# felixendres/rgbdslam_v2

Measured on AMD Instinct MI355X. Metric: frame-pairs matched+RANSAC/sec, 640x480 ORB-1000, higher is better.
Workload: dtype fp4 MFMA, exact (match) + f32/f64 (RANSAC); 1 GPU; configs[1]: synthetic 640x480 RGB-D, ORB 1000 kp, 20 candidate pairs/frame, 200 frames; max_matches=300, parallelism=pair-sharded x1, graph_capture=True

## Files before the change

### include/rgbdfe.h

```cpp
#ifndef RGBDFE_H
#define RGBDFE_H

#include <stddef.h>
#include <stdint.h>

#ifdef __cplusplus
extern "C" {
#endif

#define RGBDFE_MAX_MATCHES 320
#define RGBDFE_MASK_WORDS 5
#define RGBDFE_MAX_KEYPOINTS 65535

typedef enum {
  RGBDFE_OK = 0,
  RGBDFE_ERR_INVALID_ARG = -1,
  RGBDFE_ERR_NO_DEVICE = -2,
  RGBDFE_ERR_HIP = -3,
  RGBDFE_ERR_UNKNOWN_NODE = -4,
  RGBDFE_ERR_CAPACITY = -5,
  RGBDFE_ERR_OUT_OF_MEMORY = -6,
  RGBDFE_ERR_INTERNAL = -7
} rgbdfe_status;

// ... 71 lines not shown
int  rgbdfe_match_pair_list_allgather_inliers(rgbdfe_ctx* ctx, const int32_t* query_ids, const int32_t* train_ids,
                                              int32_t n_pairs, void* const* d_out, int32_t* records_per_device,
                                              int32_t* list_entries, int64_t* stride_bytes);
int  rgbdfe_pack_compact(rgbdfe_ctx* ctx, const void* d_records, int32_t n, void* d_compact, void* stream);
int  rgbdfe_sizeof_compact_result(void);
int  rgbdfe_pack_inliers(rgbdfe_ctx* ctx, const void* d_records, int32_t n, int32_t n_headers, void* d_stream,
                         int32_t* d_total, void* stream);
int  rgbdfe_sizeof_inlier_header(void);
int  rgbdfe_set_params(rgbdfe_ctx* ctx, const rgbdfe_params* p);
const char* rgbdfe_status_string(int status);
const char* rgbdfe_last_error(rgbdfe_ctx* ctx);

int rgbdfe_upload_node(rgbdfe_ctx* ctx, int32_t node_id, const uint8_t* desc,
                       const float* xyz1, int32_t n);
int rgbdfe_upload_nodes(rgbdfe_ctx* ctx, int32_t n_nodes, const int32_t* node_ids, const uint8_t* const* desc,
                        const float* const* xyz1, const int32_t* counts);
int rgbdfe_upload_node_device(rgbdfe_ctx* ctx, int32_t node_id, const void* d_desc,
                              const void* d_xyz1, int32_t n, void* stream);
int rgbdfe_upload_node_keypoints(rgbdfe_ctx* ctx, int32_t node_id, const float* kp_xy, int32_t n);
int rgbdfe_release_node(rgbdfe_ctx* ctx, int32_t node_id);
int rgbdfe_node_count(rgbdfe_ctx* ctx, int32_t node_id);

int rgbdfe_match_node_pairs(rgbdfe_ctx* ctx, int32_t new_node_id, const int32_t* candidate_ids,
                            int32_t n_pairs, rgbdfe_match_result* out);
int rgbdfe_match_pair_list(rgbdfe_ctx* ctx, const int32_t* query_ids, const int32_t* train_ids,
                           int32_t n_pairs, rgbdfe_match_result* out);
int rgbdfe_match_pair_list_device(rgbdfe_ctx* ctx, const int32_t* query_ids,
                                  const int32_t* train_ids, int32_t n_pairs, void* d_out,
                                  void* stream);
int rgbdfe_submit_pair_list(rgbdfe_ctx* ctx, const int32_t* query_ids, const int32_t* train_ids,
                            int32_t n_pairs, void* d_out, int64_t* ticket);
int rgbdfe_wait_ticket(rgbdfe_ctx* ctx, int64_t ticket, void* stream);
#define RGBDFE_HOST_RECORDS 0
#define RGBDFE_HOST_INLIERS 1
int rgbdfe_submit_pair_list_host(rgbdfe_ctx* ctx, const int32_t* query_ids, const int32_t* train_ids, int32_t n_pairs,
                                 void* out, size_t out_bytes, int payload, int64_t* ticket);
int rgbdfe_wait_host(rgbdfe_ctx* ctx, int64_t ticket, int64_t* bytes_written);
int rgbdfe_wait_host_into(rgbdfe_ctx* ctx, int64_t ticket, void* out, size_t out_bytes, int64_t* bytes_written);
int rgbdfe_synchronize(rgbdfe_ctx* ctx);

int rgbdfe_upload_sift_node(rgbdfe_ctx* ctx, int32_t node_id, const float* desc128,
                            const float* xyz1, int32_t n);
int rgbdfe_match_sift_pair_list(rgbdfe_ctx* ctx, const int32_t* query_ids, const int32_t* train_ids,
                                int32_t n_pairs, rgbdfe_match_result* out, float* out_dist);
int rgbdfe_submit_sift_pair_list(rgbdfe_ctx* ctx, const int32_t* query_ids, const int32_t* train_ids,
                                 int32_t n_pairs, void* d_out, void* d_out_dist, int64_t* ticket);
int rgbdfe_sift_match_nodes(rgbdfe_ctx* ctx, int32_t query_id, int32_t train_id, int32_t* match_q,
                            int32_t* match_t, float* match_dist, int32_t* n_matches);

int rgbdfe_upload_float_node(rgbdfe_ctx* ctx, int32_t node_id, const float* desc, int32_t dim, const float* xyz1,
                             int32_t n);
int rgbdfe_match_flann_pair_list(rgbdfe_ctx* ctx, const int32_t* query_ids, const int32_t* train_ids, int32_t n_pairs,
                                 double nn_distance_ratio, rgbdfe_match_result* out, float* out_dist);

int rgbdfe_hamming_nn_nodes(rgbdfe_ctx* ctx, int32_t query_id, int32_t train_id,
                            int32_t* out_hd, int32_t* out_idx);
int rgbdfe_hamming_nn_host(rgbdfe_ctx* ctx, const uint8_t* qdesc, int32_t nq,
                           const uint8_t* tdesc, int32_t nt, int32_t* out_hd, int32_t* out_idx);

int rgbdfe_project_to_3d(rgbdfe_ctx* ctx, const float* kp_xy, int32_t n_kp, const float* depth,
                         int32_t rows, int32_t cols, double fx, double fy, double cx, double cy,
                         double depth_scaling, int32_t max_keypoints, int32_t* kept_idx,
                         float* xyz1, int32_t* n_out);

int rgbdfe_project_to_3d_cloud(rgbdfe_ctx* ctx, const float* kp_xy, int32_t n_kp, const float* cloud, int32_t rows,
                               int32_t cols, double maximum_depth, int32_t max_keypoints, int32_t* kept_idx, float* xyz1,
                               int32_t* n_out);

int rgbdfe_sift_node_features(rgbdfe_ctx* ctx, const float* kp_xy, int32_t n_kp, const float* desc_in,
                              const float* depth, int32_t rows, int32_t cols, double fx, double fy,
                              double cx, double cy, double depth_scaling, int32_t max_keypoints,
                              int32_t use_root_sift, int32_t* kept_idx, float* xyz1,
                              float* siftgpu_descriptors, float* feature_descriptors, int32_t* n_out);
int rgbdfe_sift_node_features_min_depth(rgbdfe_ctx* ctx, const float* kp_xy, const float* kp_size, int32_t n_kp,
                                        const float* desc_in, const float* depth, int32_t rows, int32_t cols, double fx,
                                        double fy, double cx, double cy, double depth_scaling, int32_t max_keypoints,
                                        int32_t use_root_sift, int32_t* kept_idx, float* xyz1, float* siftgpu_descriptors,
                                        float* feature_descriptors, int32_t* n_out);

int rgbdfe_set_latency_mode(rgbdfe_ctx* ctx, int32_t max_pairs, int32_t chunk_iterations);

#define RGBDFE_HAMMING_MODE_DEFAULT 3
int rgbdfe_set_hamming_mode(rgbdfe_ctx* ctx, int32_t mode);

typedef struct rgbdfe_emm_counts {
  uint32_t inliers, outliers, occluded, all;
} rgbdfe_emm_counts;
int rgbdfe_depth_to_mono8(rgbdfe_ctx* ctx, const void* depth, int32_t depth_is_u16, int32_t rows, int32_t cols,
                          uint8_t* mono8, float* depth_m);
int rgbdfe_upload_node_cloud(rgbdfe_ctx* ctx, int32_t node_id, const float* depth, int32_t rows, int32_t cols,
                             const uint8_t* rgb, int32_t rgb_channels, int32_t encoding_bgr, double fx,
                             double fy, double cx, double cy, double depth_scaling, double min_depth,
                             int32_t cloud_skip, float* cloud_out);
int rgbdfe_release_node_cloud(rgbdfe_ctx* ctx, int32_t node_id);
int rgbdfe_observation_likelihood(rgbdfe_ctx* ctx, int32_t n, const int32_t* new_ids, const int32_t* old_ids,
                                  const float* transforms, int32_t emm_skip_step, rgbdfe_emm_counts* out);
int rgbdfe_observation_criterion_met(uint32_t inliers, uint32_t outliers, uint32_t all,
                                     double observability_threshold, double* quality);

int rgbdfe_assemble_map(rgbdfe_ctx* ctx, int32_t n_nodes, const int32_t* node_ids, const float* transforms,
                        double maximum_depth, int32_t preserve_raster, float* out, int64_t capacity, int64_t* n_out,
                        int64_t* node_offsets);
int rgbdfe_assemble_map_device(rgbdfe_ctx* ctx, int32_t n_nodes, const int32_t* node_ids, const float* transforms,
                               double maximum_depth, int32_t preserve_raster, void* d_out, int64_t capacity,
                               int64_t* n_out, int64_t* node_offsets, void* stream);
int rgbdfe_download_node_cloud(rgbdfe_ctx* ctx, int32_t node_id, float* cloud_out, int64_t capacity_points,
                               int32_t* rows, int32_t* cols);

#define RGBDFE_VOXEL_LEAF_TOO_SMALL 1
int rgbdfe_voxel_filter(rgbdfe_ctx* ctx, const float* points, int64_t n_in, double voxelfilter_size, float* out,
                        int64_t capacity, int64_t* n_out, int32_t* flags);
int rgbdfe_voxel_filter_device(rgbdfe_ctx* ctx, const void* d_points, int64_t n_in, double voxelfilter_size,
                               void* d_out, int64_t capacity, int64_t* n_out, int32_t* flags, void* stream);
int rgbdfe_reduce_node_cloud(rgbdfe_ctx* ctx, int32_t node_id, double voxelfilter_size, int64_t* n_out,
                             int32_t* flags);

typedef struct rgbdfe_octomap rgbdfe_octomap;
typedef struct rgbdfe_octomap_params {
  double resolution;
  double prob_hit;
  double prob_miss;
  double clamping_min;
  double clamping_max;
  double occupancy_threshold;
} rgbdfe_octomap_params;
typedef struct rgbdfe_octomap_leaf {
  uint16_t key[3];
  uint16_t zero0;
  float log_odds;
  uint8_t rgb[3];
  uint8_t zero1;
} rgbdfe_octomap_leaf;
void rgbdfe_octomap_default_params(rgbdfe_octomap_params* params);
int rgbdfe_octomap_create(rgbdfe_ctx* ctx, const rgbdfe_octomap_params* params, int64_t capacity_cells,
                          rgbdfe_octomap** map);
void rgbdfe_octomap_destroy(rgbdfe_octomap* map);
int rgbdfe_octomap_reset(rgbdfe_octomap* map);
int rgbdfe_octomap_reserve(rgbdfe_octomap* map, int64_t capacity_cells);
int rgbdfe_octomap_insert_nodes(rgbdfe_octomap* map, int32_t n_nodes, const int32_t* node_ids, const float* transforms,
                                double max_range, int32_t* n_done);
int rgbdfe_octomap_insert_cloud(rgbdfe_octomap* map, const float* points, int64_t n, const float* transform,
                                double max_range);
int rgbdfe_octomap_size(rgbdfe_octomap* map, int64_t* n_leaves);
int rgbdfe_octomap_leaves(rgbdfe_octomap* map, rgbdfe_octomap_leaf* out, int64_t capacity, int64_t* n_out);
int rgbdfe_octomap_stats(rgbdfe_octomap* map, int64_t* out, int32_t n_out);

typedef struct rgbdfe_octomap_node {
  float log_odds;
  uint8_t rgb[3];
  uint8_t children;
} rgbdfe_octomap_node;
int rgbdfe_octomap_tree(rgbdfe_octomap* map, rgbdfe_octomap_node* out, int64_t capacity, int64_t* n_nodes);
int rgbdfe_octomap_tree_device(rgbdfe_octomap* map, void* d_out, int64_t capacity, int64_t* n_nodes, void* stream);
int rgbdfe_octomap_nodes_at_depth(rgbdfe_octomap* map, int32_t depth, float min_log_odds, rgbdfe_octomap_leaf* out,
                                  int64_t capacity, int64_t* n_out);
int rgbdfe_octomap_write(rgbdfe_octomap* map, const char* path);
int rgbdfe_octomap_set_leaves(rgbdfe_octomap* map, const rgbdfe_octomap_leaf* leaves, int64_t n);
int rgbdfe_octomap_read(rgbdfe_octomap* map, const char* path);

typedef struct rgbdfe_pose_graph rgbdfe_pose_graph;
typedef int (*rgbdfe_rand_fn)(void* state);
rgbdfe_pose_graph* rgbdfe_pose_graph_create(void);
void rgbdfe_pose_graph_destroy(rgbdfe_pose_graph* g);
int rgbdfe_pose_graph_add_node(rgbdfe_pose_graph* g, int32_t node_id, int32_t vertex_id, int32_t matchable,
                               int32_t keyframe);
int rgbdfe_pose_graph_add_edge(rgbdfe_pose_graph* g, int32_t node_id1, int32_t node_id2);
// ... 169 lines not shown
```

### rgbdslam_v2_amd/_lib.py

```python
import ctypes as C
import os

import numpy as np

_HERE = os.path.dirname(os.path.abspath(__file__))
LIB_PATH = os.environ.get("RGBDFE_LIB", os.path.join(_HERE, "librgbdfe.so"))

RGBDFE_MAX_MATCHES = 320
RGBDFE_MASK_WORDS = 5

DEFAULT_HAMMING_MODE = 3
KERNEL_HAMMING = 0
KERNEL_RANSAC = 1
KERNEL_SIFT_DOT = 2
KERNEL_SIFT_FINISH = 3
KERNEL_EMM = 4


class RgbdfeParams(C.Structure):
    _fields_ = [
        ("max_matches", C.c_int32),
        ("min_matches", C.c_int32),
        ("ransac_iterations", C.c_int32),
        ("max_dist_for_inliers", C.c_float),
# ... 278 lines not shown
    L.rgbdfe_release_node_cloud.argtypes = [ctx, i32]
    L.rgbdfe_observation_likelihood.restype = C.c_int
    L.rgbdfe_observation_likelihood.argtypes = [ctx, i32, vp, vp, vp, i32, vp]
    L.rgbdfe_assemble_map.restype = C.c_int
    L.rgbdfe_assemble_map.argtypes = [ctx, i32, vp, vp, C.c_double, i32, vp, C.c_int64, C.POINTER(C.c_int64), vp]
    L.rgbdfe_assemble_map_device.restype = C.c_int
    L.rgbdfe_assemble_map_device.argtypes = [ctx, i32, vp, vp, C.c_double, i32, vp, C.c_int64, C.POINTER(C.c_int64), vp, vp]
    L.rgbdfe_download_node_cloud.restype = C.c_int
    L.rgbdfe_download_node_cloud.argtypes = [ctx, i32, vp, C.c_int64, C.POINTER(i32), C.POINTER(i32)]
    L.rgbdfe_voxel_filter.restype = C.c_int
    L.rgbdfe_voxel_filter.argtypes = [ctx, vp, C.c_int64, C.c_double, vp, C.c_int64, C.POINTER(C.c_int64), C.POINTER(i32)]
    L.rgbdfe_voxel_filter_device.restype = C.c_int
    L.rgbdfe_voxel_filter_device.argtypes = [ctx, vp, C.c_int64, C.c_double, vp, C.c_int64, C.POINTER(C.c_int64),
                                             C.POINTER(i32), vp]
    L.rgbdfe_reduce_node_cloud.restype = C.c_int
    L.rgbdfe_reduce_node_cloud.argtypes = [ctx, i32, C.c_double, C.POINTER(C.c_int64), C.POINTER(i32)]
    omap = vp
    L.rgbdfe_octomap_default_params.restype = None
    L.rgbdfe_octomap_default_params.argtypes = [C.POINTER(OctomapParams)]
    L.rgbdfe_octomap_create.restype = C.c_int
    L.rgbdfe_octomap_create.argtypes = [ctx, C.POINTER(OctomapParams), C.c_int64, C.POINTER(vp)]
    L.rgbdfe_octomap_destroy.restype = None
    L.rgbdfe_octomap_destroy.argtypes = [omap]
    L.rgbdfe_octomap_reset.restype = C.c_int
    L.rgbdfe_octomap_reset.argtypes = [omap]
    L.rgbdfe_octomap_reserve.restype = C.c_int
    L.rgbdfe_octomap_reserve.argtypes = [omap, C.c_int64]
    L.rgbdfe_octomap_insert_nodes.restype = C.c_int
    L.rgbdfe_octomap_insert_nodes.argtypes = [omap, i32, vp, vp, C.c_double, C.POINTER(i32)]
    L.rgbdfe_octomap_insert_cloud.restype = C.c_int
    L.rgbdfe_octomap_insert_cloud.argtypes = [omap, vp, C.c_int64, vp, C.c_double]
    L.rgbdfe_octomap_size.restype = C.c_int
    L.rgbdfe_octomap_size.argtypes = [omap, C.POINTER(C.c_int64)]
    L.rgbdfe_octomap_leaves.restype = C.c_int
    L.rgbdfe_octomap_leaves.argtypes = [omap, vp, C.c_int64, C.POINTER(C.c_int64)]
    L.rgbdfe_octomap_stats.restype = C.c_int
    L.rgbdfe_octomap_stats.argtypes = [omap, vp, i32]
    L.rgbdfe_octomap_tree.restype = C.c_int
    L.rgbdfe_octomap_tree.argtypes = [omap, vp, C.c_int64, C.POINTER(C.c_int64)]
    L.rgbdfe_octomap_tree_device.restype = C.c_int
    L.rgbdfe_octomap_tree_device.argtypes = [omap, vp, C.c_int64, C.POINTER(C.c_int64), vp]
    L.rgbdfe_octomap_nodes_at_depth.restype = C.c_int
    L.rgbdfe_octomap_nodes_at_depth.argtypes = [omap, i32, C.c_float, vp, C.c_int64, C.POINTER(C.c_int64)]
    L.rgbdfe_octomap_write.restype = C.c_int
    L.rgbdfe_octomap_write.argtypes = [omap, C.c_char_p]
    L.rgbdfe_octomap_set_leaves.restype = C.c_int
    L.rgbdfe_octomap_set_leaves.argtypes = [omap, vp, C.c_int64]
    L.rgbdfe_octomap_read.restype = C.c_int
    L.rgbdfe_octomap_read.argtypes = [omap, C.c_char_p]
    L.rgbdfe_observation_criterion_met.restype = C.c_int
    L.rgbdfe_observation_criterion_met.argtypes = [C.c_uint32, C.c_uint32, C.c_uint32, C.c_double,
                                                   C.POINTER(C.c_double)]
    L.rgbdfe_set_latency_mode.restype = C.c_int
    L.rgbdfe_set_latency_mode.argtypes = [ctx, i32, i32]
    L.rgbdfe_set_profiling.restype = C.c_int
    L.rgbdfe_set_profiling.argtypes = [ctx, C.c_int]
    L.rgbdfe_get_kernel_time.restype = C.c_int
    L.rgbdfe_get_kernel_time.argtypes = [ctx, C.c_int, C.POINTER(C.c_double),
                                         C.POINTER(C.c_int64), C.POINTER(C.c_int64)]
    L.rgbdfe_reset_kernel_time.restype = C.c_int
    L.rgbdfe_reset_kernel_time.argtypes = [ctx]
    L.rgbdfe_set_graph_capture.restype = C.c_int
    L.rgbdfe_set_graph_capture.argtypes = [ctx, C.c_int]
    L.rgbdfe_graph_stats.restype = C.c_int
    L.rgbdfe_graph_stats.argtypes = [ctx, C.POINTER(C.c_int64), C.c_int32]
    L.rgbdfe_create_multi.restype = C.c_int
    L.rgbdfe_create_multi.argtypes = [C.POINTER(RgbdfeConfig), vp, i32, C.POINTER(vp)]
    L.rgbdfe_device_count.restype = C.c_int
    L.rgbdfe_device_count.argtypes = [ctx]
    L.rgbdfe_device_context.restype = vp
    L.rgbdfe_device_context.argtypes = [ctx, i32]
    L.rgbdfe_match_pair_list_allgather.restype = C.c_int
    L.rgbdfe_match_pair_list_allgather.argtypes = [ctx, vp, vp, i32, vp, C.POINTER(i32)]
    L.rgbdfe_match_pair_list_allgather_edges.restype = C.c_int
    L.rgbdfe_match_pair_list_allgather_edges.argtypes = [ctx, vp, vp, i32, vp, vp, vp, C.POINTER(i32)]
    L.rgbdfe_group_submit_us.restype = C.c_int
    L.rgbdfe_group_submit_us.argtypes = [ctx, C.POINTER(C.c_double)]
    L.rgbdfe_gather_transport.restype = C.c_char_p
    L.rgbdfe_gather_transport.argtypes = [ctx]
    L.rgbdfe_gather_exchanges.restype = C.c_int
    L.rgbdfe_gather_exchanges.argtypes = [ctx]
    L.rgbdfe_set_hamming_mode.restype = C.c_int
    L.rgbdfe_set_hamming_mode.argtypes = [ctx, i32]
    L.rgbdfe_match_pair_list_allgather_compact.restype = C.c_int
    L.rgbdfe_match_pair_list_allgather_compact.argtypes = [ctx, vp, vp, i32, vp, C.POINTER(i32)]
    L.rgbdfe_pack_compact.restype = C.c_int
    L.rgbdfe_pack_compact.argtypes = [ctx, vp, i32, vp, vp]
    L.rgbdfe_sizeof_compact_result.restype = C.c_int
    L.rgbdfe_match_pair_list_allgather_inliers.restype = C.c_int
    L.rgbdfe_match_pair_list_allgather_inliers.argtypes = [ctx, vp, vp, i32, vp, C.POINTER(i32), vp, C.POINTER(C.c_int64)]
    L.rgbdfe_pack_inliers.restype = C.c_int
    L.rgbdfe_pack_inliers.argtypes = [ctx, vp, i32, i32, vp, vp, vp]
    L.rgbdfe_sizeof_inlier_header.restype = C.c_int
    if L.rgbdfe_sizeof_inlier_header() != INLIER_HEADER_DTYPE.itemsize:
        raise RgbdfeError("rgbdfe_inlier_header layout mismatch between librgbdfe.so and the binding")
    if L.rgbdfe_sizeof_compact_result() != COMPACT_DTYPE.itemsize:
        raise RgbdfeError("rgbdfe_compact_result layout mismatch between librgbdfe.so and the binding")
    L.rgbdfe_sift_detect.restype = C.c_int
    L.rgbdfe_sift_detect.argtypes = [ctx, vp, vp, i32, i32, i32, vp, vp, i32, C.POINTER(i32)]
    L.rgbdfe_sift_describe.restype = C.c_int
    L.rgbdfe_sift_describe.argtypes = [ctx, vp, i32, i32, vp, i32, vp]
    L.rgbdfe_sift_detect_batch.restype = C.c_int
    L.rgbdfe_sift_detect_batch.argtypes = [ctx, i32, vp, i32, i32, i32, i32, vp, vp, vp]
    L.rgbdfe_sift_detect_batch_nodes.restype = C.c_int
    L.rgbdfe_sift_detect_batch_nodes.argtypes = [ctx, i32, vp, vp, i32, i32, C.c_double, C.c_double, C.c_double, C.c_double,
                                                 C.c_double, i32, i32, vp, i32, vp, vp, vp, vp]
    L.rgbdfe_detect.restype = C.c_int
    L.rgbdfe_detect.argtypes = [ctx, vp, vp, i32, i32, vp, i32, C.POINTER(i32)]
    L.rgbdfe_detect_sift_describe.restype = C.c_int
    L.rgbdfe_detect_sift_describe.argtypes = [ctx, vp, vp, vp, i32, i32, C.c_double, C.c_double, C.c_double, C.c_double,
                                              C.c_double, i32, vp, vp, vp, vp, C.POINTER(i32)]
    L.rgbdfe_detect_sift_describe_batch_nodes.restype = C.c_int
    L.rgbdfe_detect_sift_describe_batch_nodes.argtypes = [ctx, i32, vp, vp, vp, i32, i32, C.c_double, C.c_double, C.c_double,
                                                          C.c_double, C.c_double, i32, vp, i32, vp, vp, vp, vp]
    L.rgbdfe_sift_detect_orb_describe.restype = C.c_int
    L.rgbdfe_sift_detect_orb_describe.argtypes = [ctx, vp, vp, i32, i32, C.c_double, C.c_double, C.c_double, C.c_double,
                                                  C.c_double, i32, vp, vp, vp, C.POINTER(i32)]
    L.rgbdfe_sift_detect_orb_describe_batch_nodes.restype = C.c_int
    L.rgbdfe_sift_detect_orb_describe_batch_nodes.argtypes = [ctx, i32, vp, vp, i32, i32, C.c_double, C.c_double, C.c_double,
                                                              C.c_double, C.c_double, i32, vp, i32, vp, vp, vp, vp]
    L.rgbdfe_sizeof_sensor_frame.restype = C.c_int
    if L.rgbdfe_sizeof_sensor_frame() != C.sizeof(RgbdfeSensorFrame):
        raise RgbdfeError("rgbdfe_sensor_frame layout mismatch between librgbdfe.so and the binding")
    L.rgbdfe_ingest_frame.restype = C.c_int
    L.rgbdfe_ingest_frame.argtypes = [ctx, C.POINTER(RgbdfeSensorFrame), vp, vp, vp]
    L.rgbdfe_sensor_detect_describe.restype = C.c_int
    L.rgbdfe_sensor_detect_describe.argtypes = [ctx, C.POINTER(RgbdfeSensorFrame), C.c_double, C.c_double, C.c_double, C.c_double,
                                                C.c_double, vp, vp, vp, C.POINTER(i32)]
    L.rgbdfe_sensor_detect_describe_batch_nodes.restype = C.c_int
    L.rgbdfe_sensor_detect_describe_batch_nodes.argtypes = [ctx, i32, C.POINTER(RgbdfeSensorFrame), C.c_double, C.c_double,
                                                            C.c_double, C.c_double, C.c_double, i32, vp, vp, vp, vp, vp,
                                                            C.POINTER(RgbdfeSensorCloud)]
    L.rgbdfe_sift_geometry.restype = C.c_int
    L.rgbdfe_sift_geometry.argtypes = [ctx] + [C.POINTER(i32)] * 4
    L.rgbdfe_sift_debug_plane.restype = C.c_int
    L.rgbdfe_sift_debug_plane.argtypes = [ctx, i32, i32, vp, i32, C.POINTER(i32), C.POINTER(i32)]
    L.rgbdfe_sift_debug_candidates.restype = C.c_int
    L.rgbdfe_sift_debug_candidates.argtypes = [ctx, i32, i32, vp, i32, C.POINTER(i32)]
    L.rgbdfe_sizeof_match_result.restype = C.c_int
    L.rgbdfe_abi_version.restype = C.c_int
    if L.rgbdfe_sizeof_match_result() != C.sizeof(RgbdfeMatchResult) or \
            RESULT_DTYPE.itemsize != C.sizeof(RgbdfeMatchResult):
        raise RgbdfeError("rgbdfe_match_result layout mismatch between librgbdfe.so and the binding")
    RAND_FN = C.CFUNCTYPE(C.c_int, C.c_void_p)
    L.rgbdfe_rand_fn = RAND_FN
    L.rgbdfe_pose_graph_create.restype = vp
    L.rgbdfe_pose_graph_create.argtypes = []
    L.rgbdfe_pose_graph_destroy.restype = None
    L.rgbdfe_pose_graph_destroy.argtypes = [vp]
    L.rgbdfe_pose_graph_add_node.restype = C.c_int
    L.rgbdfe_pose_graph_add_node.argtypes = [vp, i32, i32, i32, i32]
    L.rgbdfe_pose_graph_add_edge.restype = C.c_int
    L.rgbdfe_pose_graph_add_edge.argtypes = [vp, i32, i32]
    L.rgbdfe_pose_graph_set_matchable.restype = C.c_int
    L.rgbdfe_pose_graph_set_matchable.argtypes = [vp, i32, i32]
    L.rgbdfe_pose_graph_set_estimate.restype = C.c_int
    L.rgbdfe_pose_graph_set_estimate.argtypes = [vp, i32, vp]
    L.rgbdfe_pose_graph_get_estimate.restype = C.c_int
    L.rgbdfe_pose_graph_get_estimate.argtypes = [vp, i32, vp]
    L.rgbdfe_pose_graph_set_fixed.restype = C.c_int
    L.rgbdfe_pose_graph_set_fixed.argtypes = [vp, i32, i32]
    L.rgbdfe_pose_graph_add_edge_se3.restype = C.c_int
    L.rgbdfe_pose_graph_add_edge_se3.argtypes = [vp, i32, i32, vp, vp, i32]
    L.rgbdfe_pose_graph_chi2.restype = C.c_int
    L.rgbdfe_pose_graph_chi2.argtypes = [vp, vp, C.POINTER(C.c_double)]
    L.rgbdfe_pose_graph_linearize.restype = C.c_int
    L.rgbdfe_pose_graph_linearize.argtypes = [vp, vp, vp, vp, i32, C.POINTER(i32), vp, vp, vp, i32, C.POINTER(i32), vp, vp, vp,
                                              i32, C.POINTER(i32), C.POINTER(C.c_double)]
    L.rgbdfe_pose_graph_optimize.restype = C.c_int
    L.rgbdfe_pose_graph_optimize.argtypes = [vp, vp, i32, C.POINTER(PoseGraphReport)]
    L.rgbdfe_pose_graph_optimize_graph.restype = C.c_int
    L.rgbdfe_pose_graph_optimize_graph.argtypes = [vp, vp, C.c_double, C.POINTER(PoseGraphReport)]
    L.rgbdfe_pose_graph_transforms.restype = C.c_int
    L.rgbdfe_pose_graph_transforms.argtypes = [vp, i32, vp, vp]
    L.rgbdfe_potential_edge_targets.restype = C.c_int
    L.rgbdfe_potential_edge_targets.argtypes = [vp, i32, i32, i32, i32, i32, i32, RAND_FN, vp, C.c_uint32, vp, i32,
                                                C.POINTER(i32)]
    _lib = L
    return L


EXPORTED_SYMBOLS = [
    "rgbdfe_default_config", "rgbdfe_create", "rgbdfe_destroy", "rgbdfe_set_params",
    "rgbdfe_status_string", "rgbdfe_last_error", "rgbdfe_upload_node", "rgbdfe_upload_nodes",
    "rgbdfe_upload_node_device", "rgbdfe_release_node", "rgbdfe_node_count",
    "rgbdfe_match_node_pairs", "rgbdfe_match_pair_list", "rgbdfe_match_pair_list_device",
    "rgbdfe_detector_configure", "rgbdfe_detector_thresholds", "rgbdfe_detect_describe",
    "rgbdfe_orb_detect", "rgbdfe_orb_compute",
    "rgbdfe_submit_pair_list", "rgbdfe_wait_ticket", "rgbdfe_submit_pair_list_host", "rgbdfe_wait_host", "rgbdfe_wait_host_into", "rgbdfe_upload_sift_node",
    "rgbdfe_match_sift_pair_list", "rgbdfe_submit_sift_pair_list", "rgbdfe_sift_match_nodes",
    "rgbdfe_synchronize", "rgbdfe_hamming_nn_nodes", "rgbdfe_hamming_nn_host",
    "rgbdfe_project_to_3d", "rgbdfe_sift_node_features", "rgbdfe_sift_node_features_min_depth", "rgbdfe_depth_to_mono8",
    "rgbdfe_host_register", "rgbdfe_host_unregister",
    "rgbdfe_upload_node_cloud", "rgbdfe_release_node_cloud", "rgbdfe_observation_likelihood",
    "rgbdfe_assemble_map", "rgbdfe_assemble_map_device", "rgbdfe_download_node_cloud",
    "rgbdfe_voxel_filter", "rgbdfe_voxel_filter_device", "rgbdfe_reduce_node_cloud",
    "rgbdfe_octomap_default_params", "rgbdfe_octomap_create", "rgbdfe_octomap_destroy", "rgbdfe_octomap_reset",
    "rgbdfe_octomap_reserve", "rgbdfe_octomap_insert_nodes", "rgbdfe_octomap_insert_cloud", "rgbdfe_octomap_size",
    "rgbdfe_octomap_leaves", "rgbdfe_octomap_stats",
    "rgbdfe_octomap_tree", "rgbdfe_octomap_tree_device", "rgbdfe_octomap_nodes_at_depth", "rgbdfe_octomap_write",
    "rgbdfe_octomap_set_leaves", "rgbdfe_octomap_read",
    "rgbdfe_observation_criterion_met", "rgbdfe_set_latency_mode", "rgbdfe_set_profiling", "rgbdfe_get_kernel_time",
    "rgbdfe_reset_kernel_time", "rgbdfe_graph_stats", "rgbdfe_set_graph_capture", "rgbdfe_match_pair_list_allgather_inliers", "rgbdfe_pack_inliers", "rgbdfe_sizeof_inlier_header", "rgbdfe_sizeof_match_result", "rgbdfe_abi_version",
    "rgbdfe_pose_graph_create", "rgbdfe_pose_graph_destroy", "rgbdfe_pose_graph_add_node",
    "rgbdfe_pose_graph_add_edge", "rgbdfe_pose_graph_set_matchable", "rgbdfe_potential_edge_targets",
    "rgbdfe_pose_graph_set_estimate", "rgbdfe_pose_graph_get_estimate", "rgbdfe_pose_graph_set_fixed",
    "rgbdfe_pose_graph_add_edge_se3", "rgbdfe_pose_graph_chi2", "rgbdfe_pose_graph_linearize",
    "rgbdfe_pose_graph_optimize", "rgbdfe_pose_graph_optimize_graph", "rgbdfe_pose_graph_transforms",
    "rgbdfe_create_multi", "rgbdfe_device_count", "rgbdfe_device_context", "rgbdfe_match_pair_list_allgather",
    "rgbdfe_gather_transport", "rgbdfe_gather_exchanges", "rgbdfe_set_hamming_mode", "rgbdfe_project_to_3d_cloud", "rgbdfe_detect_describe_cloud",
    "rgbdfe_detect_describe_batch", "rgbdfe_detect_describe_batch_nodes", "rgbdfe_match_pair_list_allgather_edges",
    "rgbdfe_set_feature_min_depth", "rgbdfe_project_to_3d_min_depth",
    "rgbdfe_place_recognition", "rgbdfe_place_recognition_batch", "rgbdfe_upload_float_node",
    "rgbdfe_match_flann_pair_list", "rgbdfe_upload_node_keypoints",
    "rgbdfe_match_pair_list_allgather_compact", "rgbdfe_pack_compact", "rgbdfe_sizeof_compact_result",
    "rgbdfe_group_submit_us", "rgbdfe_sift_detect", "rgbdfe_sift_detect_batch", "rgbdfe_sift_describe", "rgbdfe_sift_geometry", "rgbdfe_sift_debug_plane", "rgbdfe_sift_debug_candidates",
    "rgbdfe_sift_detect_batch_nodes", "rgbdfe_set_detector_type", "rgbdfe_fast_detect",
    "rgbdfe_detect", "rgbdfe_detect_sift_describe", "rgbdfe_detect_sift_describe_batch_nodes",
    "rgbdfe_sift_detect_orb_describe", "rgbdfe_sift_detect_orb_describe_batch_nodes",
    "rgbdfe_sizeof_sensor_frame", "rgbdfe_ingest_frame", "rgbdfe_sensor_detect_describe",
    "rgbdfe_sensor_detect_describe_batch_nodes",
]
```

### rgbdslam_v2_amd/csrc/api_batches.hip

```cpp
#include "rgbdfe_host.h"

namespace rgbdfe_host {


int fail(rgbdfe_ctx* ctx, int code, const std::string& msg) {
  if (ctx) {
    std::lock_guard<std::mutex> g(ctx->err_mu);
    ctx->last_error = msg;
  }
  return code;
}


void fill_ransac_const(rgbdfe_ctx* ctx) {
  const rgbdfe_params& p = ctx->cfg.params;
  RansacConst& rc = ctx->rc;
  rc.max_matches = p.max_matches;
  rc.min_matches = p.min_matches;
  rc.ransac_iterations = p.ransac_iterations;
  rc.max_dist_m = (float)(double)p.max_dist_for_inliers;
  rc.sq_max_dist = (double)(rc.max_dist_m * rc.max_dist_m);
  rc.depth_cov = p.depth_cov;
  const double cam_angle_x = 58.0 / 180.0 * M_PI;
  const double cam_angle_y = 45.0 / 180.0 * M_PI;
// ... 60 lines not shown
      ctx->event_pool.push_back(p.d);
    } else {
      add(RGBDFE_KERNEL_HAMMING, p.a, p.b);
      add(RGBDFE_KERNEL_RANSAC, p.b, p.c);
    }
    ctx->event_pool.push_back(p.a);
    ctx->event_pool.push_back(p.b);
    ctx->event_pool.push_back(p.c);
  }
  ctx->pending.clear();
}

int ensure_ec_pool(rgbdfe_ctx* ctx, rgbdfe_ctx::Lane& lane, size_t regions, hipStream_t stream) {
  if (regions <= lane.ec_regions) return RGBDFE_OK;
  HIP_TRY(ctx, hipStreamSynchronize(stream));
  if (lane.d_ec) (void)hipFree(lane.d_ec);
  lane.d_ec = nullptr;
  lane.ec_regions = 0;
  HIP_TRY(ctx, hipMalloc((void**)&lane.d_ec, regions * select_ransac_ec_region_bytes()));
  lane.ec_regions = regions;
  return RGBDFE_OK;
}
int want_latency_path(rgbdfe_ctx* ctx, rgbdfe_ctx::Lane& lane, int32_t n, hipStream_t stream, bool* use, int* chunk_out,
                      PhasePlan* plan) {
  const size_t need_recs = (size_t)n * (size_t)(ctx->rc.ransac_iterations > 0 ? ctx->rc.ransac_iterations : 0);
  const bool force_phases = ctx->latency_chunk_iters < 0;
  const int chunk_cfg = force_phases ? -ctx->latency_chunk_iters : ctx->latency_chunk_iters;
  int chunk = chunk_cfg > 0 ? chunk_cfg : (n <= 64 ? 4 : (n <= 640 ? 7 : (n <= 1280 ? 14 : 28)));
  const int I_all = ctx->rc.ransac_iterations > 0 ? ctx->rc.ransac_iterations : 0;
  const bool too_many_pairs = (size_t)n > kMaxEcRegions;
  while (!too_many_pairs && chunk < I_all && (size_t)n * (size_t)((I_all + chunk - 1) / chunk) > kMaxEcRegions) ++chunk;
  bool latency = !too_many_pairs && n <= ctx->latency_pairs && ctx->rc.ransac_iterations >= 2 * chunk &&
                 need_recs <= ((size_t)1 << 24);
  *chunk_out = chunk;
  if (latency && need_recs > lane.recs_capacity) {
    HIP_TRY(ctx, hipStreamSynchronize(stream));
    if (lane.d_recs) (void)hipFree(lane.d_recs);
    lane.d_recs = nullptr;
    lane.recs_capacity = 0;
    if (hipMalloc((void**)&lane.d_recs, need_recs * (sizeof(IterRec) + sizeof(IterSum)) +
                                            ransac_split_mask_bytes(need_recs, (size_t)ctx->cfg.max_pairs_per_batch)) == hipSuccess)
      lane.recs_capacity = need_recs;
    else latency = false;
  }
  if (latency && !lane.d_walk &&
      hipMalloc((void**)&lane.d_walk, sizeof(WalkState) * ((size_t)ctx->cfg.max_pairs_per_batch + 1)) != hipSuccess) {
    lane.d_walk = nullptr;
    latency = false;
  }
  const int I = ctx->rc.ransac_iterations;
  static const int env_phases = getenv("RGBDFE_PHASES") ? atoi(getenv("RGBDFE_PHASES")) : 0;
  static const int mid_plan = getenv("RGBDFE_MID_PLAN") ? atoi(getenv("RGBDFE_MID_PLAN")) : 0;
  const bool mid = n > 256 && n <= 1280 && !force_phases && env_phases == 0;
  if ((n <= 256 && !force_phases) || env_phases == 1 || (mid && mid_plan == 1)) { plan->n_phases = 1; plan->ends[0] = I; }
  else if (mid && mid_plan == 2 && I > 14) { plan->n_phases = 2; plan->ends[0] = 14; plan->ends[1] = I; }
  else if (env_phases == 2) { plan->n_phases = 2; plan->ends[0] = ((I * 7 / 20) / 7) * 7 > 0 ? ((I * 7 / 20) / 7) * 7 : I; plan->ends[1] = I; if (plan->ends[0] >= I) plan->n_phases = 1; }
  else {
    const int cand[4] = {14, ((I * 7 / 20) / 7) * 7, ((I * 14 / 20) / 7) * 7, I};
    int k = 0, last = 0;
    for (int c : cand) { const int e = c > I ? I : c; if (e > last) { plan->ends[k++] = e; last = e; } }
    if (k == 0) plan->ends[k++] = I;
    plan->n_phases = k;
  }
  *use = latency;
  size_t regions = (size_t)n;
  if (latency) {
    int begin = 0;
    for (int p = 0; p < plan->n_phases; ++p) {
      size_t chunks = (size_t)((plan->ends[p] - begin + chunk - 1) / chunk);
      if (plan->n_phases > 2 && p == 1)
        chunks += (size_t)((I - begin + 63) / 64);
      if ((size_t)n * chunks > regions) regions = (size_t)n * chunks;
      begin = plan->ends[p];
    }
  }
  regions = regions / (size_t)(n > 0 ? n : 1) * (((size_t)n + 7) / 8 * 8);
  return ensure_ec_pool(ctx, lane, regions + 8, stream);
}

bool hamming_on_mfma(const rgbdfe_ctx* ctx) { return ctx->hamming_mode != 0 && (uint32_t)ctx->cfg.max_keypoints <= 32768u; }

HammingGeometry hamming_geometry(const rgbdfe_ctx* ctx, uint32_t n, uint32_t max_nq, uint32_t max_nt) {
  const uint32_t cap = (uint32_t)ctx->cfg.max_pairs_per_batch;
  return hamming_on_mfma(ctx) ? hamming_mfma_geometry(n, max_nq, max_nt, cap) : hamming_nn_geometry(n, max_nq, max_nt, cap);
}

uint32_t launch_hamming(rgbdfe_ctx* ctx, const PairWork* d_work, uint32_t* d_keys, uint32_t n, HammingGeometry geom,
                        hipStream_t stream) {
  const uint32_t mk = (uint32_t)ctx->cfg.max_keypoints;
  if (hamming_on_mfma(ctx))
    return launch_hamming_mfma(ctx->d_desc4, d_work, d_keys, mk, n, geom, ctx->hamming_mode, stream);
  return launch_hamming_nn(ctx->d_desc, d_work, d_keys, mk, n, geom, stream);
}

uint32_t launch_hamming(rgbdfe_ctx* ctx, const PairWork* d_work, uint32_t* d_keys, uint32_t n, uint32_t max_nq,
                        uint32_t max_nt, hipStream_t stream) {
  return launch_hamming(ctx, d_work, d_keys, n, hamming_geometry(ctx, n, max_nq, max_nt), stream);
}

bool capture_stream_ready(rgbdfe_ctx* ctx) {
  if (ctx->capture_stream) return true;
  if (hipStreamCreateWithFlags(&ctx->capture_stream, hipStreamNonBlocking) != hipSuccess) { (void)hipGetLastError(); ctx->capture_stream = nullptr; }
  return ctx->capture_stream != nullptr;
}

int enqueue_pairs(rgbdfe_ctx* ctx, const int32_t* qids, const int32_t* tids, int32_t n, rgbdfe_match_result* d_out, hipEvent_t wait_for, int64_t* ticket_out, int* lane_out, int matcher, float* d_out_dist, double flann_ratio) {


  const bool sift = matcher != 0;
  if (n > ctx->cfg.max_pairs_per_batch)
    return fail(ctx, RGBDFE_ERR_CAPACITY, "n_pairs exceeds max_pairs_per_batch");
  const int64_t ticket = ctx->next_ticket;
  rgbdfe_ctx::Slot& slot = ctx->ring[ticket % rgbdfe_ctx::kRing];
  const int li = (int)(ticket % rgbdfe_ctx::kLanes);
  rgbdfe_ctx::Lane& lane = ctx->lanes[li];
  hipStream_t stream = lane.stream;
  if (slot.pending) {
    HIP_TRY(ctx, hipEventSynchronize(slot.done));
    slot.pending = false;
  }
  uint32_t max_nq = 0, max_nt = 0, sift_kinds = 0;
  for (int32_t i = 0; i < n; ++i) {
    auto q = ctx->nodes.find(qids[i]);
    auto t = ctx->nodes.find(tids[i]);
    if (q == ctx->nodes.end() || t == ctx->nodes.end())
      return fail(ctx, RGBDFE_ERR_UNKNOWN_NODE, "pair references a node that is not resident");
    if (q->second.kind != (uint32_t)matcher || t->second.kind != (uint32_t)matcher)
      return fail(ctx, RGBDFE_ERR_INVALID_ARG, "node descriptor kind does not fit this matcher");
    PairWork& w = slot.h_work[i];
    w.q_slot = q->second.slot;
    w.t_slot = t->second.slot;
    w.nq = q->second.n;
    w.nt = t->second.n;
    w.uid = pair_uid(qids[i], tids[i]);
    w.qid = qids[i];
    w.tid = tids[i];
    w.pad = matcher == 1 ? sift_fast_keys(ctx, q->second, t->second) : 0u;
    sift_kinds |= w.pad ? 1u : 2u;
    if (ctx->rc.g2o_iterations > 0 && !(q->second.flags & t->second.flags & kNodeHasKeypoints))
      return fail(ctx, RGBDFE_ERR_INVALID_ARG,
                  "g2o_iterations > 0: a node of the batch has no keypoints (rgbdfe_upload_node_keypoints after every upload of it)");
    if (w.nq > max_nq) max_nq = w.nq;
    if (w.nt > max_nt) max_nt = w.nt;
  }
  if (ctx->rc.g2o_iterations > 0 && !ctx->d_kp2d)
    return fail(ctx, RGBDFE_ERR_INVALID_ARG, "g2o_iterations > 0 needs the nodes' keypoints (rgbdfe_upload_node_keypoints)");
  int32_t piece = n;
  if (n > 0 && ctx->latency_pairs != 0) {
    const size_t I = (size_t)(ctx->rc.ransac_iterations > 0 ? ctx->rc.ransac_iterations : 1);
    size_t fit = (((size_t)1 << 24) / I) < kMaxEcRegions ? (((size_t)1 << 24) / I) : kMaxEcRegions;
    if (fit > 65535) fit = 65535;
    if (fit < 1) fit = 1;
    if ((size_t)n > fit && (size_t)n <= (size_t)ctx->latency_pairs) piece = (int32_t)fit;
  }
  if (sift && piece > 65535) return fail(ctx, RGBDFE_ERR_CAPACITY, "a one-wave SIFT batch holds at most 65535 pairs");
  bool latency = false;
  int chunk = 7;
  PhasePlan pp{};
  if (n > 0) {
    int rcl = want_latency_path(ctx, lane, piece, stream, &latency, &chunk, &pp);
    if (rcl != RGBDFE_OK) return rcl;
  }
  if (wait_for) HIP_TRY(ctx, hipStreamWaitEvent(stream, wait_for, 0));
  if (ctx->nodes_ready) HIP_TRY(ctx, hipStreamWaitEvent(stream, ctx->nodes_ready, 0));
  hipError_t launch_err = hipSuccess;
  if (n > 0) {
    if (!d_out) d_out = lane.d_results;
    const bool graphable = ctx->use_graphs && !sift && !ctx->profiling && piece >= n && ctx->rc.g2o_iterations == 0;
    const HammingGeometry geom = sift ? HammingGeometry{0, 1}
                                      : hamming_geometry(ctx, (uint32_t)(piece < n ? piece : n), max_nq, max_nt);
    rgbdfe_ctx::GraphEntry* ge = nullptr;
    bool capturing = false;
    if (graphable) {
      rgbdfe_ctx::GraphKey key;
      memset(&key, 0, sizeof(key));
      key.n = n; key.qblocks = geom.qblocks; key.tsplit = geom.tsplit; key.slot = (int32_t)(ticket % rgbdfe_ctx::kRing);
      key.latency = latency ? 1 : 0; key.chunk = chunk; key.hamming_mode = ctx->hamming_mode; key.n_phases = pp.n_phases;
      for (int i = 0; i < 4; ++i) key.ends[i] = i < pp.n_phases ? pp.ends[i] : 0;
      memcpy(&key.rc, &ctx->rc, sizeof(RansacConst));
      key.d_out = d_out; key.d_recs = lane.d_recs; key.d_ec = lane.d_ec; key.d_walk = lane.d_walk; key.d_keys = lane.d_keys;
      size_t gi = 0;
      for (; gi < ctx->graphs.size(); ++gi)
        if (memcmp(&ctx->graphs[gi].key, &key, sizeof(key)) == 0) { ge = &ctx->graphs[gi]; break; }
      if (ge) {
        ge->used = ++ctx->graph_clock;
        const hipError_t le = hipGraphLaunch(ge->exec, stream);
        if (le == hipSuccess) {
          ctx->graph_launches++;
          ctx->graph_miss_run = 0;
        } else {
          (void)hipGetLastError();
          (void)hipGraphExecDestroy(ge->exec); (void)hipGraphDestroy(ge->graph);
          ctx->graphs.erase(ctx->graphs.begin() + (long)gi);
          ctx->graph_launch_failures++;
          ge = nullptr;
        }
      } else {
        ctx->graph_misses++;
        const bool try_capture = ctx->graph_miss_run < rgbdfe_ctx::kGraphMissRun ||
                                 ctx->graph_miss_run % rgbdfe_ctx::kGraphRetry == 0;
        ctx->graph_miss_run++;
        if (try_capture && capture_stream_ready(ctx) &&
            hipStreamBeginCapture(ctx->capture_stream, hipStreamCaptureModeRelaxed) == hipSuccess) {
          capturing = true;
          if (ctx->graphs.size() >= 48) {
            size_t lru = 0;
            for (size_t i = 1; i < ctx->graphs.size(); ++i) if (ctx->graphs[i].used < ctx->graphs[lru].used) lru = i;
            (void)hipGraphExecDestroy(ctx->graphs[lru].exec); (void)hipGraphDestroy(ctx->graphs[lru].graph);
            ctx->graphs.erase(ctx->graphs.begin() + (long)lru);
          }
          ctx->graphs.push_back(rgbdfe_ctx::GraphEntry{key, nullptr, nullptr, ++ctx->graph_clock});
        } else {
          (void)hipGetLastError();
          ctx->graph_plain_batches++;
        }
      }
    }
    rgbdfe_ctx::Pending pend{};
    pend.sift = sift;
    for (int attempt = 0; attempt < 2; ++attempt) {
      hipStream_t const ls = capturing ? ctx->capture_stream : stream;
      if (!ge) {
        const hipError_t me = hipMemcpyAsync(slot.d_work, slot.h_work, sizeof(PairWork) * (size_t)n, hipMemcpyHostToDevice, ls);
        if (me != hipSuccess && launch_err == hipSuccess) launch_err = me;
      }
      if (ctx->profiling) {
        pend.a = get_event(ctx);
        pend.b = get_event(ctx);
        pend.c = get_event(ctx);
        if (sift) pend.d = get_event(ctx);
        pend.pairs = n;
        (void)hipEventRecord(pend.a, ls);
      }
      const uint32_t mk = (uint32_t)ctx->cfg.max_keypoints;
      for (int32_t off = 0; off < n && !ge; off += piece) {
        const int32_t m = (n - off) < piece ? (n - off) : piece;
        const bool first = off == 0, last = off + m >= n;
        if (!first) {
          int rcl = want_latency_path(ctx, lane, m, ls, &latency, &chunk, &pp);
          if (rcl != RGBDFE_OK) { launch_err = hipErrorOutOfMemory; break; }
        }
        const PairWork* d_work = slot.d_work + off;
        rgbdfe_match_result* d_res = d_out + off;
        if (!sift) {
          const uint32_t planes = launch_hamming(ctx, d_work, lane.d_keys, (uint32_t)m, first ? geom : hamming_geometry(ctx, (uint32_t)m, max_nq, max_nt), ls);
          if (ctx->profiling && first) (void)hipEventRecord(pend.b, ls);
          if (latency)
            launch_select_ransac_latency(ctx->d_xyz, d_work, lane.d_keys, planes, d_res, mk, (uint32_t)m, ctx->rc,
                                         lane.d_prep, lane.d_recs, lane.d_walk, lane.d_ec, chunk, pp.ends, pp.n_phases, ls);
          else
            launch_select_ransac(ctx->d_xyz, d_work, lane.d_keys, planes, d_res, mk, (uint32_t)m, ctx->rc, lane.d_prep,
                                 lane.d_ec, ls);
          if (ctx->rc.g2o_iterations > 0)
            launch_g2o_refine(d_work, d_res, (uint32_t)m, ctx->rc, lane.d_prep, ctx->d_kp2d, mk, lane.d_ec, ls);
          if (ctx->profiling && last) (void)hipEventRecord(pend.c, ls);
        } else {
          float* d_dist = (d_out_dist ? d_out_dist : lane.d_all_dist) + (size_t)off * RGBDFE_MAX_MATCHES;
          if (matcher == 2) {
            launch_l2_knn2(ctx->d_sift_f32, d_work, mk, (uint32_t)m, max_nq, lane.d_row_part, ls);
            if (ctx->profiling && first) (void)hipEventRecord(pend.b, ls);
// ... 83 lines not shown
```

### rgbdslam_v2_amd/csrc/api_context.hip

```cpp
#include "rgbdfe_host.h"

namespace impl {


void rgbdfe_default_config(rgbdfe_config* cfg) {
  if (!cfg) return;
  memset(cfg, 0, sizeof(*cfg));
  cfg->device_id = 0;
  cfg->max_nodes = 256;
  cfg->max_keypoints = 1024;
  cfg->max_pairs_per_batch = 4096;
  cfg->params.max_matches = 300;
  cfg->params.min_matches = 20;
  cfg->params.ransac_iterations = 200;
  cfg->params.max_dist_for_inliers = 3.0f;
  cfg->params.depth_cov = 1e-4;
  cfg->params.seed = 20260923u;
}

int rgbdfe_create(const rgbdfe_config* cfg, rgbdfe_ctx** out) {
  if (!cfg || !out) return RGBDFE_ERR_INVALID_ARG;
  *out = nullptr;
  if (cfg->max_nodes < 1 || cfg->max_keypoints < 1 || cfg->max_keypoints > RGBDFE_MAX_KEYPOINTS ||
      cfg->max_pairs_per_batch < 1)
    return RGBDFE_ERR_INVALID_ARG;
  int ndev = 0;
  if (hipGetDeviceCount(&ndev) != hipSuccess || ndev <= 0) return RGBDFE_ERR_NO_DEVICE;
  if (cfg->device_id < 0 || cfg->device_id >= ndev) return RGBDFE_ERR_NO_DEVICE;
  rgbdfe_ctx* ctx = new rgbdfe_ctx();
  ctx->cfg = *cfg;
  int rc = validate_params(ctx, cfg->params);
  if (rc != RGBDFE_OK) { delete ctx; return rc; }
  fill_ransac_const(ctx);
  if (const char* sf = getenv("RGBDFE_SIFT_FAST_KEYS")) ctx->sift_fast = atoi(sf) != 0;
  if (const char* hm = getenv("RGBDFE_HAMMING_MODE")) ctx->hamming_mode = atoi(hm) < 0 || atoi(hm) > 3 ? RGBDFE_HAMMING_MODE_DEFAULT : atoi(hm);
  if (const char* gr = getenv("RGBDFE_GRAPHS")) ctx->use_graphs = atoi(gr) != 0;
  auto bail = [&](int code) { ::rgbdfe_destroy(ctx); return code; };
  if (hipSetDevice(cfg->device_id) != hipSuccess) return bail(RGBDFE_ERR_NO_DEVICE);
  (void)ransac_split_init();
  if (hipStreamCreateWithFlags(&ctx->stream, hipStreamNonBlocking) != hipSuccess)
    return bail(RGBDFE_ERR_HIP);
  if (hipEventCreateWithFlags(&ctx->ev_in, hipEventDisableTiming) != hipSuccess) return bail(RGBDFE_ERR_HIP);
  const size_t rows = (size_t)cfg->max_nodes * (size_t)cfg->max_keypoints + 16;
  if (hipMalloc((void**)&ctx->d_desc, rows * 32) != hipSuccess) return bail(RGBDFE_ERR_OUT_OF_MEMORY);
  if (hipMalloc((void**)&ctx->d_xyz, rows * 16) != hipSuccess) return bail(RGBDFE_ERR_OUT_OF_MEMORY);
  if (hipMalloc((void**)&ctx->d_desc4, hamming_mfma_slab_bytes((uint32_t)cfg->max_nodes, (uint32_t)cfg->max_keypoints)) != hipSuccess)
    return bail(RGBDFE_ERR_OUT_OF_MEMORY);
  if (hipMemsetAsync(ctx->d_desc, 0, rows * 32, ctx->stream) != hipSuccess) return bail(RGBDFE_ERR_HIP);
  if (hipMemsetAsync(ctx->d_xyz, 0, rows * 16, ctx->stream) != hipSuccess) return bail(RGBDFE_ERR_HIP);
  if (hipMemsetAsync(ctx->d_desc4, 0, hamming_mfma_slab_bytes((uint32_t)cfg->max_nodes, (uint32_t)cfg->max_keypoints), ctx->stream) != hipSuccess)
    return bail(RGBDFE_ERR_HIP);
  if (hipStreamSynchronize(ctx->stream) != hipSuccess) return bail(RGBDFE_ERR_HIP);
  const size_t np = (size_t)cfg->max_pairs_per_batch;
  for (auto& sl : ctx->ring) {
    if (hipMalloc((void**)&sl.d_work, np * sizeof(PairWork)) != hipSuccess) return bail(RGBDFE_ERR_OUT_OF_MEMORY);
    if (hipHostMalloc((void**)&sl.h_work, np * sizeof(PairWork), hipHostMallocDefault) != hipSuccess)
      return bail(RGBDFE_ERR_OUT_OF_MEMORY);
    if (hipEventCreateWithFlags(&sl.done, hipEventDisableTiming) != hipSuccess) return bail(RGBDFE_ERR_HIP);
  }
  for (auto& ln : ctx->lanes) {
    if (hipStreamCreateWithFlags(&ln.stream, hipStreamNonBlocking) != hipSuccess) return bail(RGBDFE_ERR_HIP);
    if (hipMalloc((void**)&ln.d_keys, np * (size_t)cfg->max_keypoints * 4) != hipSuccess)
      return bail(RGBDFE_ERR_OUT_OF_MEMORY);
    if (hipMalloc((void**)&ln.d_results, np * sizeof(rgbdfe_match_result)) != hipSuccess)
      return bail(RGBDFE_ERR_OUT_OF_MEMORY);
    if (hipMalloc((void**)&ln.d_prep, np * sizeof(PairPrep)) != hipSuccess) return bail(RGBDFE_ERR_OUT_OF_MEMORY);
  }
  ctx->emm_q_lo = erf_boundary(0.001);
  ctx->emm_q_hi = erf_boundary(0.999);
  ctx->free_slots.reserve(cfg->max_nodes);
  for (int32_t s = cfg->max_nodes - 1; s >= 0; --s) ctx->free_slots.push_back((uint32_t)s);
  *out = ctx;
  return RGBDFE_OK;
}

void rgbdfe_destroy(rgbdfe_ctx* ctx) {
  if (!ctx) return;
  if (ctx->stream) (void)hipStreamSynchronize(ctx->stream);
  for (auto& ln : ctx->lanes) if (ln.stream) (void)hipStreamSynchronize(ln.stream);
  for (hipStream_t st : {ctx->orb_upload_stream, ctx->orb_compute_stream, ctx->sift_stream1, ctx->sift_stream2, ctx->sift_stream3,
                        ctx->sn.depth_stream, ctx->fast.st, ctx->fast.up})
    if (st) (void)hipStreamSynchronize(st);
  sift_nodes_release(ctx);
  sift_behind_release(ctx);
  sift_orb_release(ctx);
  sensor_release(ctx);
  drain_pending(ctx);
  for (hipEvent_t e : ctx->event_pool) (void)hipEventDestroy(e);
  for (auto& ge : ctx->graphs) { (void)hipGraphExecDestroy(ge.exec); (void)hipGraphDestroy(ge.graph); }
  if (ctx->capture_stream) (void)hipStreamDestroy(ctx->capture_stream);
  if (ctx->upload_stage) (void)hipHostFree(ctx->upload_stage);
  if (ctx->sift_stream1) (void)hipStreamDestroy(ctx->sift_stream1);
  if (ctx->sift_stream2) (void)hipStreamDestroy(ctx->sift_stream2);
  if (ctx->sift_stream3) (void)hipStreamDestroy(ctx->sift_stream3);
  ctx->graphs.clear();
  if (ctx->d_desc) (void)hipFree(ctx->d_desc);
  if (ctx->d_xyz) (void)hipFree(ctx->d_xyz);
  for (auto& sl : ctx->ring) {
    if (sl.d_work) (void)hipFree(sl.d_work);
    if (sl.h_work) (void)hipHostFree(sl.h_work);
    if (sl.done) (void)hipEventDestroy(sl.done);
  }
  for (auto& kv : ctx->clouds) {
    if (kv.second.d) (void)hipFree(kv.second.d);
    if (kv.second.d_samples) (void)hipFree(kv.second.d_samples);
  }
  if (ctx->d_sift_bf16) (void)hipFree(ctx->d_sift_bf16);
  if (ctx->d_sift_f32) (void)hipFree(ctx->d_sift_f32);
  for (auto& ln : ctx->lanes) {
    if (ln.d_row_part) (void)hipFree(ln.d_row_part);
    if (ln.d_col_part) (void)hipFree(ln.d_col_part);
    if (ln.d_col_blocks) (void)hipFree(ln.d_col_blocks);
    if (ln.d_sm_q) (void)hipFree(ln.d_sm_q);
    if (ln.d_sm_t) (void)hipFree(ln.d_sm_t);
    if (ln.d_sm_d) (void)hipFree(ln.d_sm_d);
    if (ln.d_sm_n) (void)hipFree(ln.d_sm_n);
    if (ln.d_all_dist) (void)hipFree(ln.d_all_dist);
    if (ln.d_recs) (void)hipFree(ln.d_recs);
// ... 264 lines not shown
```

### rgbdslam_v2_amd/csrc/api_frame.hip

```cpp
#include "rgbdfe_host.h"

namespace impl {

static int hamming_keys_to_host(rgbdfe_ctx* ctx, uint32_t nq, uint32_t planes, int32_t* out_hd, int32_t* out_idx) {
  const size_t mk = (size_t)ctx->cfg.max_keypoints;
  std::vector<uint32_t> all((size_t)planes * mk), keys(nq);
  hipStream_t st = ctx->lanes[0].stream;
  HIP_TRY(ctx, hipMemcpyAsync(all.data(), ctx->lanes[0].d_keys, all.size() * 4, hipMemcpyDeviceToHost, st));
  HIP_TRY(ctx, hipStreamSynchronize(st));
  for (uint32_t i = 0; i < nq; ++i) {
    uint32_t k = all[i];
    for (uint32_t pl = 1; pl < planes; ++pl) k = std::min(k, all[(size_t)pl * mk + i]);
    keys[i] = k;
  }
  for (uint32_t i = 0; i < nq; ++i) {
    const uint32_t hd = keys[i] >> 16;
    if (hd > 256u) {
      out_hd[i] = 257;
      out_idx[i] = -1;
    } else {
      out_hd[i] = (int32_t)hd;
      out_idx[i] = (int32_t)(keys[i] & 0xFFFFu);
    }
  }
// ... 509 lines not shown
    const CloudEntry& co = b->second;
    const bool flat = co.ch <= 1 || co.cw <= 1;
    if (i == 0) { ch = co.ch; cw = co.cw; cloud_skip = co.cloud_skip; }
    if (ch <= 1 || cw <= 1) {
      if (!flat) return fail(ctx, RGBDFE_ERR_INVALID_ARG, "clouds of one batch must share their dimensions");
      continue;
    }
    if (cn.ch != ch || cn.cw != cw || co.ch != ch || co.cw != cw || co.cloud_skip != cloud_skip)
      return fail(ctx, RGBDFE_ERR_INVALID_ARG, "clouds of one batch must share their dimensions");
    if (cn.samples_skip != emm_skip_step) {
      CloudEntry& w = a->second;
      if (w.d_samples) { (void)hipFree(w.d_samples); w.d_samples = nullptr; }
      const size_t ns = (size_t)((ch + emm_skip_step - 1) / emm_skip_step) * (size_t)((cw + emm_skip_step - 1) / emm_skip_step);
      if (hipMalloc((void**)&w.d_samples, ns * sizeof(float4)) != hipSuccess)
        return fail(ctx, RGBDFE_ERR_OUT_OF_MEMORY, "sample array allocation failed");
      launch_decimate_cloud(w.d, ch, cw, emm_skip_step, w.d_samples, ctx->stream);
      w.samples_skip = emm_skip_step;
    }
    EmmJob& jb = jobs[(size_t)i];
    jb.new_samples = cn.d_samples;
    jb.old_z = reinterpret_cast<const float*>(co.d + (size_t)co.ch * co.cw);
    const float* T = transforms + (size_t)i * 16;
    for (int r = 0; r < 3; ++r)
      for (int c = 0; c < 4; ++c) jb.T[r * 4 + c] = T[c * 4 + r];
    jb.fx = co.fx / cloud_skip; jb.fy = co.fy / cloud_skip;
    jb.cx = co.cx / cloud_skip; jb.cy = co.cy / cloud_skip;
  }
  if (ch <= 1 || cw <= 1) {
    for (int32_t i = 0; i < n; ++i) { out[i].inliers = out[i].all = 1; out[i].outliers = out[i].occluded = 0; }
    return RGBDFE_OK;
  }
  const size_t b_jobs = (sizeof(EmmJob) * (size_t)n + 255) & ~(size_t)255;
  int rc = ensure_scratch(ctx, b_jobs + (size_t)n * 16 + 256);
  if (rc != RGBDFE_OK) return rc;
  EmmJob* d_jobs = (EmmJob*)ctx->d_scratch;
  uint32_t* d_counts = (uint32_t*)((char*)ctx->d_scratch + b_jobs);
  HIP_TRY(ctx, hipMemcpyAsync(d_jobs, jobs.data(), sizeof(EmmJob) * (size_t)n, hipMemcpyHostToDevice, ctx->stream));
  const double s1 = cloud_skip * ctx->cfg.params.depth_cov;
  const double denom = std::sqrt(s1 + s1) * 1.41421;
  hipEvent_t e0 = nullptr, e1 = nullptr;
  if (ctx->profiling) {
    e0 = get_event(ctx); e1 = get_event(ctx);
    (void)hipEventRecord(e0, ctx->stream);
  }
  if (!(denom > 0.0) || !std::isfinite(denom))
    return fail(ctx, RGBDFE_ERR_INVALID_ARG, "depth_cov must be positive and finite for the measurement model");
  const double d_lo = division_boundary(ctx->emm_q_lo, denom), d_hi = division_boundary(ctx->emm_q_hi, denom);
  launch_emm(d_jobs, n, ch, cw, emm_skip_step, d_lo, d_hi, d_counts, ctx->stream);
  if (ctx->profiling) (void)hipEventRecord(e1, ctx->stream);
  HIP_TRY(ctx, hipGetLastError());
  HIP_TRY(ctx, hipMemcpyAsync(out, d_counts, (size_t)n * 16, hipMemcpyDeviceToHost, ctx->stream));
  HIP_TRY(ctx, hipStreamSynchronize(ctx->stream));
  if (ctx->profiling) {
    float ms = 0.f;
    if (hipEventElapsedTime(&ms, e0, e1) == hipSuccess) {
      ctx->k_ms[RGBDFE_KERNEL_EMM] += ms;
      ctx->k_launches[RGBDFE_KERNEL_EMM]++;
      ctx->k_pairs[RGBDFE_KERNEL_EMM] += n;
    }
    ctx->event_pool.push_back(e0);
    ctx->event_pool.push_back(e1);
  }
  return RGBDFE_OK;
}

int rgbdfe_observation_criterion_met(uint32_t inliers, uint32_t outliers, uint32_t all, double observability_threshold,
                                     double* quality) {
  if (observability_threshold < 0) return 1;
  const double q = inliers / static_cast<double>(inliers + outliers);
  if (quality) *quality = q;
  const double certainty = inliers / static_cast<double>(all);
  return (q > observability_threshold) && (certainty > 0.25) ? 1 : 0;
}

int rgbdfe_set_latency_mode(rgbdfe_ctx* ctx, int32_t max_pairs, int32_t chunk_iterations) {
  if (!ctx || max_pairs < 0) return fail(ctx, RGBDFE_ERR_INVALID_ARG, "bad arguments");
  std::lock_guard<std::mutex> g(ctx->mu);
  ctx->latency_pairs = max_pairs;
  ctx->latency_chunk_iters = chunk_iterations;
  return RGBDFE_OK;
}

int rgbdfe_set_hamming_mode(rgbdfe_ctx* ctx, int32_t mode) {
  if (!ctx || mode < 0 || mode > 3) return fail(ctx, RGBDFE_ERR_INVALID_ARG, "hamming mode must be 0, 1, 2 or 3");
  std::lock_guard<std::mutex> g(ctx->mu);
  ctx->hamming_mode = mode;
  return RGBDFE_OK;
}

int rgbdfe_set_profiling(rgbdfe_ctx* ctx, int enable) {
  if (!ctx) return RGBDFE_ERR_INVALID_ARG;
  std::lock_guard<std::mutex> g(ctx->mu);
  ctx->profiling = enable != 0;
  return RGBDFE_OK;
}

int rgbdfe_get_kernel_time(rgbdfe_ctx* ctx, int which, double* total_ms, int64_t* launches,
                           int64_t* pairs) {
  if (!ctx || which < 0 || which >= RGBDFE_KERNEL_COUNT) return RGBDFE_ERR_INVALID_ARG;
  std::lock_guard<std::mutex> g(ctx->mu);
  drain_pending(ctx);
  if (total_ms) *total_ms = ctx->k_ms[which];
  if (launches) *launches = ctx->k_launches[which];
  if (pairs) *pairs = ctx->k_pairs[which];
  return RGBDFE_OK;
}

int rgbdfe_reset_kernel_time(rgbdfe_ctx* ctx) {
  if (!ctx) return RGBDFE_ERR_INVALID_ARG;
  std::lock_guard<std::mutex> g(ctx->mu);
  for (int i = 0; i < RGBDFE_KERNEL_COUNT; ++i) {
    ctx->k_ms[i] = 0;
    ctx->k_launches[i] = 0;
    ctx->k_pairs[i] = 0;
  }
  return RGBDFE_OK;
}

int rgbdfe_sizeof_match_result(void) { return (int)sizeof(rgbdfe_match_result); }
int rgbdfe_sizeof_compact_result(void) { return (int)sizeof(rgbdfe_compact_result); }
int rgbdfe_pack_compact(rgbdfe_ctx* ctx, const void* d_records, int32_t n, void* d_compact, void* stream) {
  if (!ctx || n < 0 || (n > 0 && (!d_records || !d_compact))) return fail(ctx, RGBDFE_ERR_INVALID_ARG, "bad pack arguments");
  std::lock_guard<std::mutex> g(ctx->mu);
  HIP_TRY(ctx, hipSetDevice(ctx->cfg.device_id));
  launch_compact_pack((const rgbdfe_match_result*)d_records, (uint32_t)n, (rgbdfe_compact_result*)d_compact,
                      stream ? (hipStream_t)stream : ctx->stream);
  HIP_TRY(ctx, hipGetLastError());
  return RGBDFE_OK;
}
int rgbdfe_set_graph_capture(rgbdfe_ctx* ctx, int enable) {
  if (!ctx) return RGBDFE_ERR_INVALID_ARG;
  std::lock_guard<std::mutex> g(ctx->mu);
  ctx->use_graphs = enable != 0;
  return RGBDFE_OK;
}

int rgbdfe_pack_inliers(rgbdfe_ctx* ctx, const void* d_records, int32_t n, int32_t n_headers, void* d_stream, int32_t* d_total,
                        void* stream) {
  if (!ctx || n < 0 || n_headers < n || !d_stream || !d_total || (n > 0 && !d_records))
    return fail(ctx, RGBDFE_ERR_INVALID_ARG, "bad pack arguments");
  std::lock_guard<std::mutex> g(ctx->mu);
  HIP_TRY(ctx, hipSetDevice(ctx->cfg.device_id));
  launch_pack_inliers((const rgbdfe_match_result*)d_records, (uint32_t)n, (uint32_t)n_headers, d_stream, d_total,
                      stream ? (hipStream_t)stream : ctx->stream);
  HIP_TRY(ctx, hipGetLastError());
  return RGBDFE_OK;
}
int rgbdfe_sizeof_inlier_header(void) { return (int)sizeof(rgbdfe_inlier_header); }
int rgbdfe_graph_stats(rgbdfe_ctx* ctx, int64_t* out, int32_t n_out) {
  if (!ctx || !out || n_out < 0) return RGBDFE_ERR_INVALID_ARG;
  std::lock_guard<std::mutex> g(ctx->mu);
  const int64_t v[RGBDFE_GRAPH_STATS] = {ctx->graph_captures, ctx->graph_launches, ctx->graph_misses, ctx->graph_plain_batches,
                                         (int64_t)ctx->graph_capture_failures, ctx->graph_launch_failures,
                                         (int64_t)ctx->graphs.size(), ctx->use_graphs ? 1 : 0};
  for (int32_t i = 0; i < n_out && i < RGBDFE_GRAPH_STATS; ++i) out[i] += v[i];
  return RGBDFE_OK;
}

int rgbdfe_abi_version(void) { return 6; }


}
```

### rgbdslam_v2_amd/csrc/hamming_mfma.hip

```cpp
#include "rgbdfe_internal.h"

namespace rgbdfe {

constexpr uint32_t kHammingPhantomTile = 0x7FFFFFFFu;
struct HammingSlots {
  uint32_t nt_search, n_ttiles, tile0, tile1, n_full, n_stages, last_slot;
  bool has_ragged;
  __host__ __device__ static HammingSlots make(uint32_t nt, uint32_t tsplit, uint32_t split, uint32_t tiles_per_stage) {
    HammingSlots s;
    s.nt_search = nt > 0 ? nt - 1u : 0u;
    s.n_ttiles = (s.nt_search + 31u) >> 5;
    s.tile0 = 0; s.tile1 = s.n_ttiles;
    if (tsplit > 1u) {
      const uint32_t chunk = (s.n_ttiles + tsplit - 1u) / tsplit;
      s.tile0 = split * chunk < s.n_ttiles ? split * chunk : s.n_ttiles;
      s.tile1 = s.tile0 + chunk < s.n_ttiles ? s.tile0 + chunk : s.n_ttiles;
    }
    const uint32_t full_tiles = s.nt_search >> 5;
    const uint32_t fend = s.tile1 < full_tiles ? s.tile1 : full_tiles;
    s.n_full = fend > s.tile0 ? fend - s.tile0 : 0u;
    s.has_ragged = (s.nt_search & 31u) != 0u && s.tile1 == s.n_ttiles && s.tile1 > s.tile0;
    s.n_stages = (s.n_full + (s.has_ragged ? 1u : 0u) + tiles_per_stage - 1u) / tiles_per_stage;
    s.last_slot = s.n_stages * tiles_per_stage - 1u;
    return s;
  }
  __host__ __device__ uint32_t tile(uint32_t slot) const {
    const uint32_t behind = (has_ragged & (slot == last_slot)) ? n_ttiles - 1u : kHammingPhantomTile;
    return slot < n_full ? tile0 + slot : behind;
  }
};

namespace {

typedef int v8i __attribute__((ext_vector_type(8)));
typedef float v16f __attribute__((ext_vector_type(16)));

constexpr int kThreads = 256;
#ifndef RGBDFE_HAMMING_QT
#define RGBDFE_HAMMING_QT 2
#endif
#ifndef RGBDFE_HAMMING_STAGE
#define RGBDFE_HAMMING_STAGE 4
#endif
constexpr int kQT = RGBDFE_HAMMING_QT;
constexpr int kQueriesPerBlock = 4 * kQT * 32;
constexpr int kStage = RGBDFE_HAMMING_STAGE;
constexpr float kNone = 3.0e38f;
constexpr float kRowUnit = 1.0f / 16384.0f;
constexpr float kBias = 256.0f;

__device__ __forceinline__ uint32_t spread8(uint32_t x) {
  uint32_t t = (x | (x << 12)) & 0x000F000Fu;
  t = (t | (t << 6)) & 0x03030303u;
  t = (t | (t << 3)) & 0x11111111u;
  return 0x22222222u | (t << 3);
}

__global__ __launch_bounds__(256) void hamming_expand_kernel(const uint32_t* __restrict__ rows, uint4* __restrict__ tiles,
                                                             uint32_t n) {
  const uint32_t gid = blockIdx.x * 256u + threadIdx.x;
  const uint32_t tile = gid >> 8, s = (gid >> 6) & 3u, half = (gid >> 5) & 1u, r = gid & 31u;
  const uint32_t row = tile * 32u + r;
  if (tile * 32u >= n) return;
  uint4 o = make_uint4(0u, 0u, 0u, 0u);
  if (row < n) {
    const uint32_t w = rows[(size_t)row * 8u + 2u * s + half];
    o.x = spread8(w & 0xFFu);
    o.y = spread8((w >> 8) & 0xFFu);
    o.z = spread8((w >> 16) & 0xFFu);
    o.w = spread8(w >> 24);
  }
  tiles[gid] = o;
}

__device__ __forceinline__ v8i as_operand(uint4 v) {
  v8i o;
  o[0] = (int)v.x; o[1] = (int)v.y; o[2] = (int)v.z; o[3] = (int)v.w;
  o[4] = 0; o[5] = 0; o[6] = 0; o[7] = 0;
  return o;
}

__device__ __forceinline__ uint32_t min16(const v16f& a) {
  uint32_t x[16];
#pragma unroll
  for (int r = 0; r < 16; ++r) x[r] = __float_as_uint(a[r]);
  const uint32_t m0 = min(min(x[0], x[1]), x[2]);
  const uint32_t m1 = min(min(x[3], x[4]), x[5]);
  const uint32_t m2 = min(min(x[6], x[7]), x[8]);
  const uint32_t m3 = min(min(x[9], x[10]), x[11]);
  const uint32_t m4 = min(min(x[12], x[13]), x[14]);
  const uint32_t m5 = min(min(m0, m1), x[15]);
  const uint32_t m6 = min(min(m2, m3), m4);
  return min(m5, m6);
}

template <int MODE, bool SPLIT>
__global__ __launch_bounds__(kThreads) void hamming_mfma_kernel(const uint4* __restrict__ slab,
                                                                const PairWork* __restrict__ work,
                                                                uint32_t* __restrict__ keys, uint32_t max_kp,
                                                                uint32_t tiles_per_slot, uint32_t n_pairs,
                                                                uint32_t qblocks, uint32_t tsplit) {
  __shared__ uint4 lds[2][kStage * 256];
  const uint32_t L = blockIdx.x;
  const uint32_t xcd = L & 7u;
  const uint32_t j = L >> 3;
  const uint32_t subs = qblocks * tsplit;
  const uint32_t pair = (j / subs) * 8u + xcd;
  if (pair >= n_pairs) return;
  const uint32_t sub = j % subs;
  const uint32_t qblock = sub / tsplit;
  const uint32_t split = sub % tsplit;

  const PairWork w = work[pair];
  const uint32_t nq = w.nq;
  if (qblock * kQueriesPerBlock >= nq) return;
  const uint32_t nt_search = w.nt > 0 ? w.nt - 1u : 0u;
  const uint32_t n_ttiles = (nt_search + 31u) >> 5;
  uint32_t tile0 = 0, tile1 = n_ttiles;
  if (SPLIT) {
    const uint32_t chunk = (n_ttiles + tsplit - 1u) / tsplit;
    tile0 = min(split * chunk, n_ttiles);
    tile1 = min(tile0 + chunk, n_ttiles);
  }

  const uint32_t lane = threadIdx.x & 63u;
  const uint32_t wave = threadIdx.x >> 6;
  const uint32_t half = lane >> 5;

  v8i bq[kQT][4];
#pragma unroll
  for (int t = 0; t < kQT; ++t) {
    uint32_t qt = qblock * (kQueriesPerBlock / 32) + wave * kQT + t;
    qt = min(qt, tiles_per_slot - 1u);
    const uint4* __restrict__ qs = slab + ((size_t)w.q_slot * tiles_per_slot + qt) * 256u;
#pragma unroll
    for (int s = 0; s < 4; ++s) {
      uint4 v = qs[s * 64 + lane];
      v.x ^= 0x88888888u; v.y ^= 0x88888888u; v.z ^= 0x88888888u; v.w ^= 0x88888888u;
      bq[t][s] = as_operand(v);
    }
  }

  v16f crow;
#pragma unroll
  for (int r = 0; r < 16; ++r) crow[r] = kBias + (float)((r & 3) + 8 * (r >> 2) + 4 * (int)half) * kRowUnit;
  v16f czero;
#pragma unroll
  for (int r = 0; r < 16; ++r) czero[r] = 0.f;
  v16f crow_ragged;
  {
    const uint32_t rag0 = (nt_search >> 5) << 5;
#pragma unroll
    for (int r = 0; r < 16; ++r) {
      const uint32_t row = rag0 + (uint32_t)((r & 3) + 8 * (r >> 2)) + 4u * half;
      crow_ragged[r] = row < nt_search ? crow[r] : kNone;
    }
  }

  uint32_t best[kQT];
#pragma unroll
// ... 2 lines not shown
  const uint4* __restrict__ ts = slab + (size_t)w.t_slot * tiles_per_slot * 256u;
  const uint32_t n_tiles = tile1 - tile0;
  const uint32_t n_stages = (n_tiles + kStage - 1u) / kStage;
  const uint32_t last_tile = tiles_per_slot - 1u;

  {
#pragma unroll
    for (int i = 0; i < kStage; ++i) {
      const uint32_t tl = min(tile0 + (uint32_t)i, last_tile);
      lds[0][i * 256 + threadIdx.x] = ts[(size_t)tl * 256u + threadIdx.x];
    }
  }
  __syncthreads();

  for (uint32_t st = 0; st < n_stages; ++st) {
    uint4 nxt[kStage];
#pragma unroll
    for (int i = 0; i < kStage; ++i) {
      const uint32_t tl = min(tile0 + (st + 1u) * kStage + (uint32_t)i, last_tile);
      nxt[i] = ts[(size_t)tl * 256u + threadIdx.x];
    }
    const uint4* __restrict__ buf = lds[st & 1u];
    auto do_tile = [&](int i, uint32_t tile, const v16f& CROW) {
      v8i a[4];
#pragma unroll
      for (int s = 0; s < 4; ++s) a[s] = as_operand(buf[i * 256 + s * 64 + lane]);
      const float base = (float)(tile * 32u) * kRowUnit;
      v16f acc[kQT];
#pragma unroll
      for (int t = 0; t < kQT; ++t) {
        acc[t] = __builtin_amdgcn_mfma_scale_f32_32x32x64_f8f6f4(a[0], bq[t][0], MODE == 1 ? CROW : czero, 4, 4, 0, 0, 0, 0);
        acc[t] = __builtin_amdgcn_mfma_scale_f32_32x32x64_f8f6f4(a[1], bq[t][1], acc[t], 4, 4, 0, 0, 0, 0);
        acc[t] = __builtin_amdgcn_mfma_scale_f32_32x32x64_f8f6f4(a[2], bq[t][2], acc[t], 4, 4, 0, 0, 0, 0);
        acc[t] = __builtin_amdgcn_mfma_scale_f32_32x32x64_f8f6f4(a[3], bq[t][3], acc[t], 4, 4, 0, 0, 0, 0);
      }
#pragma unroll
      for (int t = 0; t < kQT; ++t) {
        if (MODE != 1) {
#pragma unroll
          for (int r = 0; r < 16; ++r) acc[t][r] += CROW[r];
        }
        const float m = __uint_as_float(min16(acc[t]));
        best[t] = min(best[t], __float_as_uint(m + base));
      }
    };
    const uint32_t stage_tile0 = tile0 + st * kStage;
    if (stage_tile0 + kStage <= tile1 && (stage_tile0 + kStage) * 32u <= nt_search) {
#pragma unroll
      for (int i = 0; i < kStage; ++i) do_tile(i, stage_tile0 + (uint32_t)i, crow);
    } else {
#pragma unroll
      for (int i = 0; i < kStage; ++i) {
        const uint32_t tile = stage_tile0 + (uint32_t)i;
        if (tile < tile1) {
          if (tile * 32u + 32u > nt_search) do_tile(i, tile, crow_ragged);
          else do_tile(i, tile, crow);
        }
      }
    }
#pragma unroll
    for (int i = 0; i < kStage; ++i) lds[(st + 1u) & 1u][i * 256 + threadIdx.x] = nxt[i];
    __syncthreads();
  }

  uint32_t* kout = keys + ((size_t)pair * tsplit + split) * max_kp;
#pragma unroll
  for (int t = 0; t < kQT; ++t) {
    uint32_t bb = best[t];
    bb = min(bb, (uint32_t)__shfl_xor((int)bb, 32));
    const float b = __uint_as_float(bb);
    const uint32_t qi = qblock * kQueriesPerBlock + (wave * kQT + (uint32_t)t) * 32u + (lane & 31u);
    if (half == 0 && qi < nq) {
      uint32_t key = kNoMatchKey;
      if (b < 1.0e30f) {
        const uint32_t k = (uint32_t)(b * 16384.0f);
        key = ((k >> 15) << 16) | (k & 32767u);
      }
      kout[qi] = key;
    }
  }
}


#ifndef RGBDFE_HAMMING_PIPE_BURST
#define RGBDFE_HAMMING_PIPE_BURST 0
#endif
#ifndef RGBDFE_HAMMING_PIPE_ALT4
#define RGBDFE_HAMMING_PIPE_ALT4 0
#endif
#ifndef RGBDFE_HAMMING_PIPE_WAVES
#define RGBDFE_HAMMING_PIPE_WAVES 3
#endif
#ifndef RGBDFE_HAMMING_PIPE_VALU_GROUPS
#define RGBDFE_HAMMING_PIPE_VALU_GROUPS 334
#endif
#ifndef RGBDFE_HAMMING_PIPE_DIAG
#define RGBDFE_HAMMING_PIPE_DIAG 0
#endif
constexpr int kPipeStage = 4;
constexpr float kRowUnitPerTile = 32.0f / 16384.0f;

#define HP_MFMA(ACC, A, B, C) ACC = __builtin_amdgcn_mfma_scale_f32_32x32x64_f8f6f4(A, B, C, 4, 4, 0, 0, 0, 0);
#define HP_SGB(MASK, N) __builtin_amdgcn_sched_group_barrier(MASK, N, 0);
#define HP_FENCE() __builtin_amdgcn_sched_barrier(0);

template <bool SPLIT>
__global__ __launch_bounds__(kThreads) __attribute__((amdgpu_waves_per_eu(RGBDFE_HAMMING_PIPE_WAVES, RGBDFE_HAMMING_PIPE_WAVES)))
void hamming_mfma_pipe_kernel(const uint4* __restrict__ slab,
                                                                     const PairWork* __restrict__ work,
                                                                     uint32_t* __restrict__ keys, uint32_t max_kp,
                                                                     uint32_t tiles_per_slot, uint32_t n_pairs,
                                                                     uint32_t qblocks, uint32_t tsplit) {
  __shared__ uint4 lds0[kPipeStage][256], lds1[kPipeStage][256], lds2[kPipeStage][256];
  const uint32_t L = blockIdx.x;
  const uint32_t xcd = L & 7u;
  const uint32_t j = L >> 3;
  const uint32_t subs = qblocks * tsplit;
  const uint32_t pair = (j / subs) * 8u + xcd;
  if (pair >= n_pairs) return;
  const uint32_t sub = j % subs;
  const uint32_t qblock = sub / tsplit;
  const uint32_t split = sub % tsplit;

  const PairWork w = work[pair];
  const uint32_t nq = w.nq;
  if (qblock * kQueriesPerBlock >= nq) return;
  const HammingSlots slots = HammingSlots::make(w.nt, SPLIT ? tsplit : 1u, SPLIT ? split : 0u, kPipeStage);
  const uint32_t nt_search = slots.nt_search, n_stages = slots.n_stages;
  const bool has_ragged = slots.has_ragged;
  auto slot_tile = [&](uint32_t s) -> uint32_t { return slots.tile(s); };

  const uint32_t lane = threadIdx.x & 63u;
  const uint32_t wave = __builtin_amdgcn_readfirstlane(threadIdx.x >> 6);
  const uint32_t half = lane >> 5;

  v8i bq[kQT][4];
#pragma unroll
  for (int t = 0; t < kQT; ++t) {
    uint32_t qt = qblock * (kQueriesPerBlock / 32) + wave * kQT + t;
    qt = min(qt, tiles_per_slot - 1u);
    const uint4* __restrict__ qs = slab + ((size_t)w.q_slot * tiles_per_slot + qt) * 256u;
#pragma unroll
    for (int s = 0; s < 4; ++s) {
      uint4 v = qs[s * 64 + lane];
      v.x ^= 0x88888888u; v.y ^= 0x88888888u; v.z ^= 0x88888888u; v.w ^= 0x88888888u;
      bq[t][s] = as_operand(v);
    }
  }

  v16f crow, c3;
#pragma unroll
  for (int r = 0; r < 16; ++r) crow[r] = kBias + (float)((r & 3) + 8 * (r >> 2) + 4 * (int)half) * kRowUnit;
  c3 = crow;
  auto set_c3_ragged = [&]() {
    uint32_t nts = nt_search;
    asm volatile("" : "+v"(nts));
    const uint32_t rag0 = (nts >> 5) << 5;
#pragma unroll
    for (int r = 0; r < 16; ++r) {
      const uint32_t row = rag0 + (uint32_t)((r & 3) + 8 * (r >> 2)) + 4u * half;
      c3[r] = row < nts ? crow[r] : kNone;
    }
  };

  uint32_t best0 = __float_as_uint(kNone), best1 = __float_as_uint(kNone);

  const uint32_t last_tile = tiles_per_slot - 1u;
  const char* __restrict__ ts = reinterpret_cast<const char*>(slab + (size_t)w.t_slot * tiles_per_slot * 256u);
  const uint64_t ts_u = reinterpret_cast<uint64_t>(ts);
  const uint32_t ts_lo = __builtin_amdgcn_readfirstlane((uint32_t)ts_u);
  const uint32_t ts_hi = __builtin_amdgcn_readfirstlane((uint32_t)(ts_u >> 32));
  const uint32_t vo16 = threadIdx.x * 16u;

  auto load_stage = [&](uint32_t st, uint4 (*buf)[256]) {
#pragma unroll
    for (int i = 0; i < kPipeStage; ++i) {
      const uint32_t tl = min(slot_tile(st * kPipeStage + (uint32_t)i), last_tile);
      const char* tb = reinterpret_cast<const char*>((((uint64_t)ts_hi << 32) | ts_lo) + (uint64_t)tl * 4096u);
      uint32_t vo = vo16;
      asm volatile("" : "+v"(vo));
      __builtin_amdgcn_global_load_lds((const __attribute__((address_space(1))) void*)(tb + vo),
                                       (__attribute__((address_space(3))) void*)&buf[i][wave * 64],
                                       16, 0, 0);
    }
  };

  if (n_stages > 0) {
    static_assert(kQT == 2 && kPipeStage == 4, "the unrolled stream is written for two query tiles and four-tile stages");
    load_stage(0, lds0);
    if (n_stages > 1) load_stage(1, lds1);
    __builtin_amdgcn_s_waitcnt(0x0F70);
    __syncthreads();

    v8i aA[4], aB[4];
#if RGBDFE_HAMMING_PIPE_DIAG & 2
#define HP_READ(DST, BUF, SLOT, S) asm volatile("" : "+v"(DST[S]));
#else
#define HP_READ(DST, BUF, SLOT, S) DST[S] = as_operand(lds##BUF[SLOT][(S) * 64 + lane]);
#endif
#define HP_BASE(SLOT) ((float)slot_tile(st * kPipeStage + (SLOT)) * kRowUnitPerTile)
#if RGBDFE_HAMMING_PIPE_DIAG & 1
#define HP_EPI(ACC, BEST, BASE) asm volatile("" : : "v"(ACC));
#else
#define HP_EPI(ACC, BEST, BASE)                                                 \
    BEST = min(BEST, __float_as_uint(__uint_as_float(min16(ACC)) + (BASE))); \
    asm volatile("" : "+v"(BEST));
#endif
#if RGBDFE_HAMMING_PIPE_BURST
#define HP_UNIT_SCHED() HP_SGB(0x008, 4) HP_SGB(0x100, 2) HP_SGB(0x002, 12)
#else
#define HP_UNIT_SCHED()                                                                             \
    HP_SGB(0x008, 1) HP_SGB(0x100, 2)                                                               \
    HP_SGB(0x008, 1) HP_SGB(0x002, RGBDFE_HAMMING_PIPE_VALU_GROUPS / 100)                            \
    HP_SGB(0x008, 1) HP_SGB(0x002, RGBDFE_HAMMING_PIPE_VALU_GROUPS / 10 % 10)                        \
    HP_SGB(0x008, 1) HP_SGB(0x002, RGBDFE_HAMMING_PIPE_VALU_GROUPS % 10)
#endif
#define HP_UNIT(ACC, A, Q, C, PACC, PBEST, PBASE, R0, R1)                                           \
    HP_MFMA(ACC, A[0], bq[Q][0], C)                                                                 \
    R0 R1                                                                                           \
    HP_MFMA(ACC, A[1], bq[Q][1], ACC)                                                               \
    HP_EPI(PACC, PBEST, PBASE)                                                                      \
    HP_MFMA(ACC, A[2], bq[Q][2], ACC)                                                               \
    HP_MFMA(ACC, A[3], bq[Q][3], ACC)                                                               \
    HP_UNIT_SCHED()                                                                                 \
    HP_FENCE()
#if RGBDFE_HAMMING_PIPE_DIAG & 4
#define HP_TURN()
#define HP_LOADS false
#else
#define HP_TURN() __builtin_amdgcn_s_waitcnt(0x0F70); __syncthreads();
#define HP_LOADS true
#endif
#if RGBDFE_HAMMING_PIPE_ALT4
#define HP_TILE(X0, X1, A, C, P0, P1, PBASE, R0, R1, R2, R3)                                         \
    HP_MFMA(X0, A[0], bq[0][0], C) HP_MFMA(X1, A[0], bq[1][0], C)                                    \
    R0 R1 R2 R3                                                                                      \
    HP_MFMA(X0, A[1], bq[0][1], X0) HP_MFMA(X1, A[1], bq[1][1], X1)                                  \
    HP_EPI(P0, best0, PBASE)                                                                         \
    HP_MFMA(X0, A[2], bq[0][2], X0) HP_MFMA(X1, A[2], bq[1][2], X1)                                  \
    HP_EPI(P1, best1, PBASE)                                                                         \
    HP_MFMA(X0, A[3], bq[0][3], X0) HP_MFMA(X1, A[3], bq[1][3], X1)                                  \
    HP_SGB(0x008, 1) HP_SGB(0x100, 1) HP_SGB(0x008, 1) HP_SGB(0x100, 1)                              \
    HP_SGB(0x008, 1) HP_SGB(0x100, 1) HP_SGB(0x002, 2) HP_SGB(0x008, 1) HP_SGB(0x100, 1) HP_SGB(0x002, 3) \
    HP_SGB(0x008, 1) HP_SGB(0x002, 4) HP_SGB(0x008, 1) HP_SGB(0x002, 4)                              \
    HP_SGB(0x008, 1) HP_SGB(0x002, 4) HP_SGB(0x008, 1) HP_SGB(0x002, 4)                              \
    HP_FENCE()
#define HP_HALF_A(CUR)                                                                                               \
    {                                                                                                                \
      b0 = HP_BASE(0); b1 = HP_BASE(1);                                                                              \
      HP_FENCE()                                                                                                     \
      HP_TILE(acc0, acc1, aA, crow, acc2, acc3, pend, HP_READ(aB, CUR, 1, 0), HP_READ(aB, CUR, 1, 1),                \
              HP_READ(aB, CUR, 1, 2), HP_READ(aB, CUR, 1, 3))                                                        \
      HP_TILE(acc2, acc3, aB, crow, acc0, acc1, b0, HP_READ(aA, CUR, 2, 0), HP_READ(aA, CUR, 2, 1),                  \
              HP_READ(aA, CUR, 2, 2), HP_READ(aA, CUR, 2, 3))                                                        \
      HP_TURN()                                                                                                      \
    }
#define HP_HALF_B(CUR, NXT, NN)                                                                                      \
    {                                                                                                                \
      if (HP_LOADS && st + 2u < n_stages) load_stage(st + 2u, lds##NN);                                              \
      const float b2 = HP_BASE(2), b3 = HP_BASE(3);                                                                  \
      if (has_ragged && st + 1u == n_stages) {                                                                       \
        set_c3_ragged();                                                                                             \
        asm volatile("" : "+v"(c3));                                                                                 \
      }                                                                                                              \
      HP_FENCE()                                                                                                     \
      HP_TILE(acc0, acc1, aA, crow, acc2, acc3, b1, HP_READ(aB, CUR, 3, 0), HP_READ(aB, CUR, 3, 1),                  \
              HP_READ(aB, CUR, 3, 2), HP_READ(aB, CUR, 3, 3))                                                        \
      HP_TILE(acc2, acc3, aB, c3, acc0, acc1, b2, HP_READ(aA, NXT, 0, 0), HP_READ(aA, NXT, 0, 1),                    \
              HP_READ(aA, NXT, 0, 2), HP_READ(aA, NXT, 0, 3))                                                        \
      pend = b3;                                                                                                     \
    }
#else
#define HP_HALF_A(CUR)                                                                                               \
    {                                                                                                                \
      b0 = HP_BASE(0); b1 = HP_BASE(1);                                                                              \
      HP_FENCE()                                                                                                     \
      HP_UNIT(acc0, aA, 0, crow, acc1, best1, pend, HP_READ(aB, CUR, 1, 0), HP_READ(aB, CUR, 1, 1))                  \
      HP_UNIT(acc1, aA, 1, crow, acc0, best0, b0, HP_READ(aB, CUR, 1, 2), HP_READ(aB, CUR, 1, 3))                    \
      HP_UNIT(acc0, aB, 0, crow, acc1, best1, b0, HP_READ(aA, CUR, 2, 0), HP_READ(aA, CUR, 2, 1))                    \
      HP_UNIT(acc1, aB, 1, crow, acc0, best0, b1, HP_READ(aA, CUR, 2, 2), HP_READ(aA, CUR, 2, 3))                    \
      HP_TURN()                                                                                                      \
    }
#define HP_HALF_B(CUR, NXT, NN)                                                                                      \
    {                                                                                                                \
      if (HP_LOADS && st + 2u < n_stages) load_stage(st + 2u, lds##NN);    \
      const float b2 = HP_BASE(2), b3 = HP_BASE(3);                                                                  \
      if (has_ragged && st + 1u == n_stages) {                                                                       \
        set_c3_ragged();                                                                                             \
        asm volatile("" : "+v"(c3));         \
      }                                                                                                              \
      HP_FENCE()                                                                                                     \
      HP_UNIT(acc0, aA, 0, crow, acc1, best1, b1, HP_READ(aB, CUR, 3, 0), HP_READ(aB, CUR, 3, 1))                    \
      HP_UNIT(acc1, aA, 1, crow, acc0, best0, b2, HP_READ(aB, CUR, 3, 2), HP_READ(aB, CUR, 3, 3))                    \
      HP_UNIT(acc0, aB, 0, c3, acc1, best1, b2, HP_READ(aA, NXT, 0, 0), HP_READ(aA, NXT, 0, 1))                      \
      HP_UNIT(acc1, aB, 1, c3, acc0, best0, b3, HP_READ(aA, NXT, 0, 2), HP_READ(aA, NXT, 0, 3))                      \
      pend = b3;                                                                                                     \
    }

#endif
    HP_READ(aA, 0, 0, 0) HP_READ(aA, 0, 0, 1) HP_READ(aA, 0, 0, 2) HP_READ(aA, 0, 0, 3)
#if RGBDFE_HAMMING_PIPE_ALT4
    v16f acc0, acc1, acc2 = crow, acc3 = crow;
#else
    v16f acc0, acc1 = crow;
#endif
    float pend = 4.0e6f;
    float b0, b1;
    uint32_t st = 0;
    HP_HALF_A(0)
    for (;;) {
      HP_HALF_B(0, 1, 2)
      if (++st == n_stages) break;
      HP_HALF_A(1)
      HP_HALF_B(1, 2, 0)
      if (++st == n_stages) break;
      HP_HALF_A(2)
      HP_HALF_B(2, 0, 1)
      if (++st == n_stages) break;
      HP_HALF_A(0)
    }
#if RGBDFE_HAMMING_PIPE_ALT4
    HP_EPI(acc2, best0, pend)
    HP_EPI(acc3, best1, pend)
#else
    HP_EPI(acc1, best1, pend)
#endif
#undef HP_HALF_A
#undef HP_HALF_B
#undef HP_TURN
#undef HP_LOADS
#undef HP_UNIT
#undef HP_EPI
#undef HP_BASE
#undef HP_READ
  }

  uint32_t* kout = keys + ((size_t)pair * tsplit + split) * max_kp;
  const uint32_t bests[2] = {best0, best1};
#pragma unroll
  for (int t = 0; t < kQT; ++t) {
    uint32_t bb = bests[t];
    bb = min(bb, (uint32_t)__shfl_xor((int)bb, 32));
    const float b = __uint_as_float(bb);
    const uint32_t qi = qblock * kQueriesPerBlock + (wave * kQT + (uint32_t)t) * 32u + (lane & 31u);
    if (half == 0 && qi < nq) {
      uint32_t key = kNoMatchKey;
      if (RGBDFE_HAMMING_PIPE_DIAG ? b < -1.0f : b < 1024.0f) {
        const uint32_t k = (uint32_t)(b * 16384.0f);
        key = ((k >> 15) << 16) | (k & 32767u);
      }
      kout[qi] = key;
    }
  }
}
#undef HP_MFMA
#undef HP_SGB
#undef HP_FENCE

}

}

extern "C" int rgbdfe_debug_hamming_slots(uint32_t nt, uint32_t tsplit, uint32_t split, uint32_t* tiles_out, int capacity,
                                          int* has_ragged, uint32_t* n_ttiles) {
  const rgbdfe::HammingSlots s = rgbdfe::HammingSlots::make(nt, tsplit, split, 4u);
  if (has_ragged) *has_ragged = s.has_ragged ? 1 : 0;
  if (n_ttiles) *n_ttiles = s.n_ttiles;
  const int n = (int)(s.n_stages * 4u);
  if (n > capacity) return -1;
  for (int i = 0; i < n; ++i) tiles_out[i] = s.tile((uint32_t)i);
  return n;
}

namespace rgbdfe {

uint32_t hamming_mfma_tiles_per_slot(uint32_t max_kp) { return (max_kp + 31u) / 32u; }

size_t hamming_mfma_slab_bytes(uint32_t max_nodes, uint32_t max_kp) {
  return ((size_t)max_nodes * hamming_mfma_tiles_per_slot(max_kp) + 1u) * 4096u;
}

void launch_hamming_expand(const uint32_t* node_rows, uint32_t* slab, uint32_t slot, uint32_t max_kp, uint32_t n,
                           hipStream_t stream) {
  if (n == 0) return;
  const uint32_t tiles = (n + 31u) / 32u;
  uint4* dst = reinterpret_cast<uint4*>(slab) + (size_t)slot * hamming_mfma_tiles_per_slot(max_kp) * 256u;
  hipLaunchKernelGGL(hamming_expand_kernel, dim3(tiles), dim3(256), 0, stream, node_rows, dst, n);
}

HammingGeometry hamming_mfma_geometry(uint32_t n_pairs, uint32_t max_nq, uint32_t max_nt, uint32_t key_planes_capacity) {
  HammingGeometry g{0, 1};
  if (n_pairs == 0 || max_nq == 0) return g;
  g.qblocks = (max_nq + kQueriesPerBlock - 1) / kQueriesPerBlock;
  const uint32_t blocks1 = n_pairs * g.qblocks;
  const uint32_t ttiles = (max_nt + 31u) / 32u;
  if (blocks1 < 1024 && ttiles > kStage) {
    uint32_t tsplit = (1024 + blocks1 - 1) / blocks1;
    const uint32_t max_split = (ttiles + kStage - 1) / kStage;
    if (tsplit > max_split) tsplit = max_split;
    if (tsplit > 32) tsplit = 32;
    const uint32_t fit = key_planes_capacity / n_pairs;
    if (tsplit > fit) tsplit = fit;
    if (tsplit < 1) tsplit = 1;
    g.tsplit = tsplit;
  }
  return g;
}

uint32_t launch_hamming_mfma(const uint32_t* slab, const PairWork* work, uint32_t* keys, uint32_t max_kp,
                             uint32_t n_pairs, HammingGeometry geom, int mode, hipStream_t stream) {
  if (n_pairs == 0 || geom.qblocks == 0) return 1;
  const uint32_t qblocks = geom.qblocks, tsplit = geom.tsplit;
  const uint32_t tiles_per_slot = hamming_mfma_tiles_per_slot(max_kp);
  const uint32_t pairs8 = (n_pairs + 7u) / 8u * 8u;
  const uint32_t grid = pairs8 * qblocks * tsplit;
  const uint4* s4 = reinterpret_cast<const uint4*>(slab);
#define RGBDFE_LAUNCH_HM(M, S)                                                                                   \
  hipLaunchKernelGGL((hamming_mfma_kernel<M, S>), dim3(grid), dim3(kThreads), 0, stream, s4, work, keys, max_kp, \
                     tiles_per_slot, n_pairs, qblocks, tsplit)
  if (mode == 3) {
    if (tsplit > 1)
      hipLaunchKernelGGL((hamming_mfma_pipe_kernel<true>), dim3(grid), dim3(kThreads), 0, stream, s4, work, keys, max_kp,
                         tiles_per_slot, n_pairs, qblocks, tsplit);
    else
      hipLaunchKernelGGL((hamming_mfma_pipe_kernel<false>), dim3(grid), dim3(kThreads), 0, stream, s4, work, keys, max_kp,
                         tiles_per_slot, n_pairs, qblocks, tsplit);
  } else if (mode == 2) {
    if (tsplit > 1) RGBDFE_LAUNCH_HM(2, true); else RGBDFE_LAUNCH_HM(2, false);
  } else {
    if (tsplit > 1) RGBDFE_LAUNCH_HM(1, true); else RGBDFE_LAUNCH_HM(1, false);
  }
#undef RGBDFE_LAUNCH_HM
  return tsplit;
}

}
```

### rgbdslam_v2_amd/csrc/hamming_nn.hip

```cpp
#include "rgbdfe_internal.h"

namespace rgbdfe {

constexpr int kHamThreads = 256;
constexpr int kQPL = 2;
constexpr int kQueriesPerBlock = kHamThreads * kQPL;

template <bool SPLIT>
__global__ __launch_bounds__(kHamThreads) void hamming_nn_kernel(
    const uint32_t* __restrict__ desc_pool, const PairWork* __restrict__ work,
    uint32_t* __restrict__ keys, uint32_t max_kp, uint32_t n_pairs, uint32_t tiles,
    uint32_t tsplit) {
  const uint32_t L = blockIdx.x;
  const uint32_t xcd = L & 7u;
  const uint32_t j = L >> 3;
  const uint32_t subs = tiles * tsplit;
  const uint32_t pair = (j / subs) * 8u + xcd;
  if (pair >= n_pairs) return;
  const uint32_t sub = j % subs;
  const uint32_t tile = sub / tsplit;
  const uint32_t split = sub % tsplit;

  const PairWork w = work[pair];
  const uint32_t nq = w.nq;
  const uint32_t nt_search = w.nt > 0 ? w.nt - 1u : 0u;

  uint32_t t0 = 0, t1 = nt_search;
  if (SPLIT) {
    uint32_t chunk = (nt_search + tsplit - 1u) / tsplit;
    t0 = min(split * chunk, nt_search);
    t1 = min(t0 + chunk, nt_search);
  }

  const uint32_t qbase = tile * kQueriesPerBlock + threadIdx.x;
  if (tile * kQueriesPerBlock >= nq) return;

  uint32_t q[kQPL][8];
  const uint4* qpool = reinterpret_cast<const uint4*>(desc_pool + (size_t)w.q_slot * max_kp * 8u);
#pragma unroll
  for (int k = 0; k < kQPL; ++k) {
    uint32_t qi = qbase + k * kHamThreads;
    qi = qi < nq ? qi : nq - 1u;
    uint4 a = qpool[2u * qi], b = qpool[2u * qi + 1u];
    q[k][0] = a.x; q[k][1] = a.y; q[k][2] = a.z; q[k][3] = a.w;
    q[k][4] = b.x; q[k][5] = b.y; q[k][6] = b.z; q[k][7] = b.w;
  }

  uint32_t best[kQPL];
#pragma unroll
  for (int k = 0; k < kQPL; ++k) best[k] = 0xFFFFFFFFu;

  const uint32_t* __restrict__ tpool = desc_pool + (size_t)w.t_slot * max_kp * 8u;
  uint32_t t = t0;
  uint32_t cur[32];
  {
    const uint32_t* __restrict__ row = tpool + (size_t)t * 8u;
#pragma unroll
    for (int i = 0; i < 32; ++i) cur[i] = row[i];
  }
#pragma unroll 2
  for (; t + 4u <= t1; t += 4u) {
    uint32_t nxt[32];
    const uint32_t* __restrict__ row = tpool + (size_t)(t + 4u) * 8u;
#pragma unroll
    for (int i = 0; i < 32; ++i) nxt[i] = row[i];
#pragma unroll
    for (int g = 0; g < 4; ++g) {
#pragma unroll
      for (int k = 0; k < kQPL; ++k) {
        uint32_t hd = 0;
#pragma unroll
        for (int i = 0; i < 8; ++i) hd += __builtin_popcount(q[k][i] ^ cur[g * 8 + i]);
        uint32_t key = (hd << 16) | (t + g);
        best[k] = min(best[k], key);
      }
    }
#pragma unroll
    for (int i = 0; i < 32; ++i) cur[i] = nxt[i];
  }
#pragma unroll
  for (int g = 0; g < 3; ++g) {
    if (t + g < t1) {
#pragma unroll
      for (int k = 0; k < kQPL; ++k) {
        uint32_t hd = 0;
#pragma unroll
        for (int i = 0; i < 8; ++i) hd += __builtin_popcount(q[k][i] ^ cur[g * 8 + i]);
        uint32_t key = (hd << 16) | (t + g);
        best[k] = min(best[k], key);
      }
    }
  }

  uint32_t* kout = keys + ((size_t)pair * tsplit + split) * max_kp;
#pragma unroll
  for (int k = 0; k < kQPL; ++k) {
    uint32_t qi = qbase + k * kHamThreads;
    if (qi < nq) kout[qi] = best[k] == 0xFFFFFFFFu ? kNoMatchKey : best[k];
  }
}

HammingGeometry hamming_nn_geometry(uint32_t n_pairs, uint32_t max_nq, uint32_t max_nt, uint32_t key_planes_capacity) {
  HammingGeometry g{0, 1};
  if (n_pairs == 0 || max_nq == 0) return g;
  g.qblocks = (max_nq + kQueriesPerBlock - 1) / kQueriesPerBlock;
  const uint32_t blocks1 = n_pairs * g.qblocks;
  if (blocks1 < 2048 && max_nt > 64) {
    uint32_t tsplit = (2048 + blocks1 - 1) / blocks1;
    const uint32_t max_split = (max_nt + 63) / 64;
    if (tsplit > max_split) tsplit = max_split;
    if (tsplit > 32) tsplit = 32;
    const uint32_t fit = key_planes_capacity / n_pairs;
    if (tsplit > fit) tsplit = fit;
    if (tsplit < 1) tsplit = 1;
    g.tsplit = tsplit;
  }
  return g;
}

uint32_t launch_hamming_nn(const uint32_t* desc_pool, const PairWork* work, uint32_t* keys,
                           uint32_t max_kp, uint32_t n_pairs, HammingGeometry geom, hipStream_t stream) {
  if (n_pairs == 0 || geom.qblocks == 0) return 1;
  const uint32_t tiles = geom.qblocks, tsplit = geom.tsplit;
  const uint32_t pairs8 = (n_pairs + 7u) / 8u * 8u;
  const uint32_t grid = pairs8 * tiles * tsplit;
  if (tsplit > 1)
    hipLaunchKernelGGL(hamming_nn_kernel<true>, dim3(grid), dim3(kHamThreads), 0, stream,
                       desc_pool, work, keys, max_kp, n_pairs, tiles, tsplit);
  else
    hipLaunchKernelGGL(hamming_nn_kernel<false>, dim3(grid), dim3(kHamThreads), 0, stream,
                       desc_pool, work, keys, max_kp, n_pairs, tiles, tsplit);
  return tsplit;
}

}
```

### rgbdslam_v2_amd/csrc/rgbdfe_api.hip

```cpp
#include "rgbdfe_host.h"

extern "C" {

void rgbdfe_default_config(rgbdfe_config* cfg) { impl::rgbdfe_default_config(cfg); }

int rgbdfe_create(const rgbdfe_config* cfg, rgbdfe_ctx** out) {
  return guarded(nullptr, [&]() -> int { return impl::rgbdfe_create(cfg, out); });
}

int rgbdfe_create_multi(const rgbdfe_config* cfg, const int32_t* device_ids, int32_t n_devices, rgbdfe_ctx** out) {
  return guarded(nullptr, [&]() -> int { return group_create(cfg, device_ids, n_devices, out); });
}

void rgbdfe_destroy(rgbdfe_ctx* ctx) {
  if (!ctx) return;
  try {
    if (ctx->group) group_destroy(ctx);
    else impl::rgbdfe_destroy(ctx);
  } catch (...) {
  }
}

int rgbdfe_device_count(rgbdfe_ctx* ctx) {
  if (!ctx) return RGBDFE_ERR_INVALID_ARG;
// ... 884 lines not shown
int rgbdfe_octomap_nodes_at_depth(rgbdfe_octomap* map, int32_t depth, float min_log_odds, rgbdfe_octomap_leaf* out,
                                  int64_t capacity, int64_t* n_out) {
  RGBDFE_ON_MAP(map, impl::rgbdfe_octomap_nodes_at_depth(map, depth, min_log_odds, out, capacity, n_out));
}

int rgbdfe_octomap_write(rgbdfe_octomap* map, const char* path) { RGBDFE_ON_MAP(map, impl::rgbdfe_octomap_write(map, path)); }

int rgbdfe_octomap_set_leaves(rgbdfe_octomap* map, const rgbdfe_octomap_leaf* leaves, int64_t n) {
  RGBDFE_ON_MAP(map, impl::rgbdfe_octomap_set_leaves(map, leaves, n));
}

int rgbdfe_octomap_read(rgbdfe_octomap* map, const char* path) { RGBDFE_ON_MAP(map, impl::rgbdfe_octomap_read(map, path)); }
#undef RGBDFE_ON_MAP

int rgbdfe_pose_graph_chi2(rgbdfe_ctx* ctx, rgbdfe_pose_graph* g, double* chi2) {
  if (!ctx) return RGBDFE_ERR_INVALID_ARG;
  return RGBDFE_FIRST(ctx, impl::rgbdfe_pose_graph_chi2(c, g, chi2));
}

int rgbdfe_pose_graph_linearize(rgbdfe_ctx* ctx, rgbdfe_pose_graph* g, double* errors, double* weights, int32_t edge_capacity,
                                int32_t* n_edges, int32_t* free_ids, double* h_diag, double* b, int32_t vertex_capacity,
                                int32_t* n_free, int32_t* off_rows, int32_t* off_cols, double* h_off, int32_t block_capacity,
                                int32_t* n_blocks, double* chi2) {
  if (!ctx) return RGBDFE_ERR_INVALID_ARG;
  return RGBDFE_FIRST(ctx, impl::rgbdfe_pose_graph_linearize(c, g, errors, weights, edge_capacity, n_edges, free_ids, h_diag, b,
                                                             vertex_capacity, n_free, off_rows, off_cols, h_off, block_capacity,
                                                             n_blocks, chi2));
}

int rgbdfe_pose_graph_optimize(rgbdfe_ctx* ctx, rgbdfe_pose_graph* g, int32_t iterations, rgbdfe_pose_graph_report* report) {
  if (!ctx) return RGBDFE_ERR_INVALID_ARG;
  return RGBDFE_FIRST(ctx, impl::rgbdfe_pose_graph_optimize(c, g, iterations, report));
}

int rgbdfe_pose_graph_optimize_graph(rgbdfe_ctx* ctx, rgbdfe_pose_graph* g, double break_criterion,
                                     rgbdfe_pose_graph_report* report) {
  if (!ctx) return RGBDFE_ERR_INVALID_ARG;
  return RGBDFE_FIRST(ctx, impl::rgbdfe_pose_graph_optimize_graph(c, g, break_criterion, report));
}

int rgbdfe_observation_likelihood(rgbdfe_ctx* ctx, int32_t n, const int32_t* new_ids, const int32_t* old_ids,
                                  const float* transforms, int32_t emm_skip_step, rgbdfe_emm_counts* out) {
  if (!ctx) return RGBDFE_ERR_INVALID_ARG;
  return guarded(ctx, [&]() -> int {
    if (!RGBDFE_IS_GROUP(ctx))
      return impl::rgbdfe_observation_likelihood(ctx, n, new_ids, old_ids, transforms, emm_skip_step, out);
    if (n < 0 || (n > 0 && (!new_ids || !old_ids || !transforms || !out)))
      return fail(ctx, RGBDFE_ERR_INVALID_ARG, "bad arguments");
    Group& g = *ctx->group;
    const int G = (int)g.children.size();
    return group_run(ctx, [&](int i) -> int {
      std::vector<int32_t> a, b;
      std::vector<float> T;
      for (int32_t k = i; k < n; k += G) {
        a.push_back(new_ids[k]); b.push_back(old_ids[k]);
        T.insert(T.end(), transforms + (size_t)k * 16, transforms + (size_t)k * 16 + 16);
      }
      if (a.empty()) return RGBDFE_OK;
      std::vector<rgbdfe_emm_counts> o(a.size());
      const int rc = impl::rgbdfe_observation_likelihood(g.children[(size_t)i], (int32_t)a.size(), a.data(), b.data(),
                                                         T.data(), emm_skip_step, o.data());
      if (rc != RGBDFE_OK) return rc;
      for (size_t m = 0; m < o.size(); ++m) out[(size_t)i + m * (size_t)G] = o[m];
      return RGBDFE_OK;
    });
  });
}

int rgbdfe_observation_criterion_met(uint32_t inliers, uint32_t outliers, uint32_t all, double observability_threshold,
                                     double* quality) {
  return impl::rgbdfe_observation_criterion_met(inliers, outliers, all, observability_threshold, quality);
}

int rgbdfe_set_latency_mode(rgbdfe_ctx* ctx, int32_t max_pairs, int32_t chunk_iterations) {
  if (!ctx) return RGBDFE_ERR_INVALID_ARG;
  return RGBDFE_ALL(ctx, impl::rgbdfe_set_latency_mode(c, max_pairs, chunk_iterations));
}

int rgbdfe_set_hamming_mode(rgbdfe_ctx* ctx, int32_t mode) {
  if (!ctx) return RGBDFE_ERR_INVALID_ARG;
  return RGBDFE_ALL(ctx, impl::rgbdfe_set_hamming_mode(c, mode));
}

int rgbdfe_set_profiling(rgbdfe_ctx* ctx, int enable) {
  if (!ctx) return RGBDFE_ERR_INVALID_ARG;
  return RGBDFE_ALL(ctx, impl::rgbdfe_set_profiling(c, enable));
}

int rgbdfe_get_kernel_time(rgbdfe_ctx* ctx, int which, double* total_ms, int64_t* launches, int64_t* pairs) {
  if (!ctx) return RGBDFE_ERR_INVALID_ARG;
  return guarded(ctx, [&]() -> int {
    if (!RGBDFE_IS_GROUP(ctx)) return impl::rgbdfe_get_kernel_time(ctx, which, total_ms, launches, pairs);
    double ms = 0; int64_t nl = 0, np = 0;
    for (rgbdfe_ctx* c : ctx->group->children) {
      double a = 0; int64_t b = 0, d = 0;
      const int rc = impl::rgbdfe_get_kernel_time(c, which, &a, &b, &d);
      if (rc != RGBDFE_OK) return rc;
      ms += a; nl += b; np += d;
    }
    if (total_ms) *total_ms = ms;
    if (launches) *launches = nl;
    if (pairs) *pairs = np;
    return RGBDFE_OK;
  });
}

int rgbdfe_reset_kernel_time(rgbdfe_ctx* ctx) {
  if (!ctx) return RGBDFE_ERR_INVALID_ARG;
  return RGBDFE_ALL(ctx, impl::rgbdfe_reset_kernel_time(c));
}

int rgbdfe_graph_stats(rgbdfe_ctx* ctx, int64_t* out, int32_t n_out) {
  if (!ctx || !out || n_out < 0) return RGBDFE_ERR_INVALID_ARG;
  return guarded(ctx, [&]() -> int {
    for (int32_t i = 0; i < n_out; ++i) out[i] = 0;
    if (!RGBDFE_IS_GROUP(ctx)) return impl::rgbdfe_graph_stats(ctx, out, n_out);
    for (rgbdfe_ctx* c : ctx->group->children) {
      const int rc = impl::rgbdfe_graph_stats(c, out, n_out);
      if (rc != RGBDFE_OK) return rc;
    }
    return RGBDFE_OK;
  });
}

int rgbdfe_sizeof_match_result(void) { return impl::rgbdfe_sizeof_match_result(); }
int rgbdfe_sizeof_compact_result(void) { return impl::rgbdfe_sizeof_compact_result(); }
int rgbdfe_abi_version(void) { return impl::rgbdfe_abi_version(); }

}
```

### rgbdslam_v2_amd/csrc/rgbdfe_host.h

```cpp
#pragma once
#include <hip/hip_runtime.h>

#include <algorithm>
#include <atomic>
#include <climits>
#include <cmath>
#include <cstdint>
#include <cstdio>
#include <cstdlib>
#include <cstring>
#include <condition_variable>
#include <functional>
#include <memory>
#include <mutex>
#include <thread>
#include <string>
#include <unordered_map>
#include <unordered_set>
#include <vector>

#include "fast_host.h"
#include "orb_host.h"
#include "sift_extract.h"
#include "rgbdfe_internal.h"
// ... 52 lines not shown

namespace rgbdfe_host {

class TaskPool {
 public:
  explicit TaskPool(int n) {
    for (int i = 0; i < n; ++i) th_.emplace_back([this] { run(); });
  }
  ~TaskPool() {
    { std::lock_guard<std::mutex> l(m_); stop_ = true; }
    cv_.notify_all();
    for (auto& t : th_) if (t.joinable()) t.join();
  }
  void submit(std::function<void()> f) {
    { std::lock_guard<std::mutex> l(m_); q_.push_back(std::move(f)); ++pending_; }
    cv_.notify_one();
  }
  void wait_all() {
    std::unique_lock<std::mutex> l(m_);
    done_.wait(l, [&] { return pending_ == 0; });
  }
  int size() const { return (int)th_.size(); }
  void parallel_for(int n, const std::function<void(int)>& fn) {
    std::atomic<int> next{0};
    auto body = [&next, &fn, n] { for (;;) { const int i = next.fetch_add(1); if (i >= n) break; fn(i); } };
    const int helpers = std::min(n - 1, size());
    for (int h = 0; h < helpers; ++h) submit(body);
    body();
    wait_all();
  }
 private:
  void run() {
    for (;;) {
      std::function<void()> f;
      {
        std::unique_lock<std::mutex> l(m_);
        cv_.wait(l, [&] { return stop_ || !q_.empty(); });
        if (stop_ && q_.empty()) return;
        f = std::move(q_.front());
        q_.erase(q_.begin());
      }
      try { f(); } catch (...) { failed_ = true; }
      { std::lock_guard<std::mutex> l(m_); --pending_; }
      done_.notify_all();
    }
  }
  std::vector<std::thread> th_;
  std::vector<std::function<void()>> q_;
  std::mutex m_;
  std::condition_variable cv_, done_;
  int pending_ = 0;
  bool stop_ = false;
 public:
  bool failed_ = false;
};

}
using namespace rgbdfe_host;

inline hipError_t create_side_stream(hipStream_t* s, int which) {
  int lo = 0, hi = 0;
  if (hipDeviceGetStreamPriorityRange(&lo, &hi) != hipSuccess || lo == hi) { (void)hipGetLastError(); return hipStreamCreateWithFlags(s, hipStreamNonBlocking); }
  return hipStreamCreateWithPriority(s, hipStreamNonBlocking, which > 0 ? hi : lo);
}

struct rgbdfe_ctx {
  rgbdfe_config cfg{};
  std::mutex mu;
  std::mutex err_mu;
  std::string last_error;
  struct Group* group = nullptr;
  hipStream_t stream = nullptr;
  uint32_t* d_desc = nullptr;
  float4* d_xyz = nullptr;
  uint32_t* d_desc4 = nullptr;
  float* d_kp2d = nullptr;
  hipStream_t orb_upload_stream = nullptr;
  hipStream_t orb_compute_stream = nullptr;
  hipEvent_t orb_upload_done[OrbWorkspace::kSets] = {};
  hipEvent_t orb_describe_done[OrbWorkspace::kSets] = {};
  bool feature_min_depth = false;
  bool sift_fast = true;
  int hamming_mode = RGBDFE_HAMMING_MODE_DEFAULT;
#ifndef RGBDFE_LANES
#define RGBDFE_LANES 2
#endif
  static constexpr int kLanes = RGBDFE_LANES;
  static constexpr int kRing = 2 * RGBDFE_LANES;
  struct Lane {
    hipStream_t stream = nullptr;
    IterRec* d_recs = nullptr;
    size_t recs_capacity = 0;
    WalkState* d_walk = nullptr;
    PairPrep* d_prep = nullptr;
    double* d_ec = nullptr;
    size_t ec_regions = 0;
    uint32_t* d_keys = nullptr;
    rgbdfe_match_result* d_results = nullptr;
    uint32_t* d_row_part = nullptr;
    uint32_t* d_col_part = nullptr;
    uint2* d_col_blocks = nullptr;
    uint16_t* d_sm_q = nullptr;
    uint16_t* d_sm_t = nullptr;
    float* d_sm_d = nullptr;
    int32_t* d_sm_n = nullptr;
    float* d_all_dist = nullptr;
  };
  uint16_t* d_sift_bf16 = nullptr;
  float* d_sift_f32 = nullptr;
  bool sift_ready = false;
  struct Slot {
    PairWork* h_work = nullptr;
    PairWork* d_work = nullptr;
    hipEvent_t done = nullptr;
    bool pending = false;
    bool failed = false;
    int64_t ticket = 0;
  };
  Lane lanes[kLanes];
  Slot ring[kRing];
  int32_t latency_pairs = INT32_MAX;
  int32_t latency_chunk_iters = 0;
  int64_t next_ticket = 1;
  struct GraphKey {
    int32_t n; uint32_t qblocks, tsplit; int32_t slot, latency, chunk, hamming_mode, n_phases; int32_t ends[4];
    RansacConst rc;
    void* d_out; void* d_recs; void* d_ec; void* d_walk; void* d_keys;
  };
  struct GraphEntry { GraphKey key; hipGraph_t graph; hipGraphExec_t exec; uint64_t used; };
  std::vector<GraphEntry> graphs;
  uint64_t graph_clock = 0;
  int64_t graph_launches = 0, graph_captures = 0;
  int64_t graph_misses = 0;
  int64_t graph_plain_batches = 0;
  int64_t graph_launch_failures = 0;
  int32_t graph_miss_run = 0;
  static constexpr int32_t kGraphMissRun = 8, kGraphRetry = 16;
  bool use_graphs = false;
  hipStream_t capture_stream = nullptr;
  long graph_capture_failures = 0;
  uint8_t* upload_stage = nullptr; size_t upload_stage_bytes = 0;
  hipEvent_t ev_in = nullptr;
  hipEvent_t nodes_ready = nullptr;
  hipEvent_t nodes_ready_ev = nullptr;
  rgbdfe_match_result* h_results = nullptr;
  struct HostJob {
    bool pending = false;
    bool waiting = false;
    bool direct = false;
    int payload = 0;
    int64_t ticket = 0;
    int32_t n = 0;
    void* out = nullptr;
    size_t out_bytes = 0;
    hipEvent_t copied = nullptr;
  };
  HostJob host_jobs[kLanes];
  uint8_t* h_stage[kLanes] = {};
  uint8_t* d_inl_stream[kLanes] = {};
  int32_t* d_inl_total[kLanes] = {};
  int32_t* h_inl_total[kLanes] = {};
  void* d_scratch = nullptr;
  size_t scratch_bytes = 0;
  OrbWorkspace orb;
  OrbWorkspace orb_super;
  std::unique_ptr<TaskPool> detect_pool, stage_pool;
// ... 182 lines not shown
int rgbdfe_upload_nodes(rgbdfe_ctx* ctx, int32_t n_nodes, const int32_t* node_ids, const uint8_t* const* desc, const float* const* xyz1, const int32_t* counts);
int rgbdfe_upload_node_device(rgbdfe_ctx* ctx, int32_t node_id, const void* d_desc, const void* d_xyz1, int32_t n, void* stream);
int rgbdfe_upload_node_keypoints(rgbdfe_ctx* ctx, int32_t node_id, const float* kp_xy, int32_t n);
int rgbdfe_release_node(rgbdfe_ctx* ctx, int32_t node_id);
int rgbdfe_node_count(rgbdfe_ctx* ctx, int32_t node_id);
int rgbdfe_match_pair_list(rgbdfe_ctx* ctx, const int32_t* query_ids, const int32_t* train_ids, int32_t n_pairs, rgbdfe_match_result* out, int64_t out_stride = 1);
int rgbdfe_match_node_pairs(rgbdfe_ctx* ctx, int32_t new_node_id, const int32_t* candidate_ids, int32_t n_pairs, rgbdfe_match_result* out);
int rgbdfe_match_pair_list_device(rgbdfe_ctx* ctx, const int32_t* query_ids, const int32_t* train_ids, int32_t n_pairs, void* d_out, void* stream);
int rgbdfe_submit_pair_list(rgbdfe_ctx* ctx, const int32_t* query_ids, const int32_t* train_ids, int32_t n_pairs, void* d_out, int64_t* ticket);
int rgbdfe_wait_ticket(rgbdfe_ctx* ctx, int64_t ticket, void* stream);
int rgbdfe_submit_pair_list_host(rgbdfe_ctx* ctx, const int32_t* query_ids, const int32_t* train_ids, int32_t n_pairs, void* out, size_t out_bytes, int payload, int64_t* ticket);
int rgbdfe_wait_host(rgbdfe_ctx* ctx, int64_t ticket, int64_t* bytes_written);
int rgbdfe_wait_host_into(rgbdfe_ctx* ctx, int64_t ticket, void* out, size_t out_bytes, int64_t* bytes_written);
int rgbdfe_synchronize(rgbdfe_ctx* ctx);
int rgbdfe_upload_sift_node(rgbdfe_ctx* ctx, int32_t node_id, const float* desc128, const float* xyz1, int32_t n);
int rgbdfe_upload_float_node(rgbdfe_ctx* ctx, int32_t node_id, const float* desc, int32_t dim, const float* xyz1, int32_t n);
int rgbdfe_match_sift_pair_list(rgbdfe_ctx* ctx, const int32_t* query_ids, const int32_t* train_ids, int32_t n_pairs, rgbdfe_match_result* out, float* out_dist, int64_t out_stride = 1, int matcher = 1, double flann_ratio = 0.95);
int rgbdfe_submit_sift_pair_list(rgbdfe_ctx* ctx, const int32_t* query_ids, const int32_t* train_ids, int32_t n_pairs, void* d_out, void* d_out_dist, int64_t* ticket);
int rgbdfe_sift_match_nodes(rgbdfe_ctx* ctx, int32_t query_id, int32_t train_id, int32_t* match_q, int32_t* match_t, float* match_dist, int32_t* n_matches);
int rgbdfe_detector_configure(rgbdfe_ctx* ctx, int32_t max_keypoints, int32_t grid_resolution, int32_t adjuster_max_iterations);
int rgbdfe_set_detector_type(rgbdfe_ctx* ctx, int32_t type);
int rgbdfe_fast_detect(rgbdfe_ctx* ctx, const uint8_t* gray, const uint8_t* mask, int32_t rows, int32_t cols, int32_t threshold, rgbdfe_keypoint* keypoints, int32_t capacity, int32_t* n_out);
int rgbdfe_detector_thresholds(rgbdfe_ctx* ctx, double* thresholds, int32_t* n_cells);
int rgbdfe_orb_detect(rgbdfe_ctx* ctx, const uint8_t* gray, const uint8_t* mask, int32_t rows, int32_t cols, int32_t fast_threshold, rgbdfe_keypoint* keypoints, int32_t capacity, int32_t* n_out);
int rgbdfe_orb_compute(rgbdfe_ctx* ctx, const uint8_t* gray, int32_t rows, int32_t cols, rgbdfe_keypoint* keypoints, int32_t n, uint8_t* descriptors, int32_t* n_out);
int rgbdfe_sift_detect(rgbdfe_ctx* ctx, const uint8_t* gray, const uint8_t* , int32_t rows, int32_t cols, int32_t max_keypoints, rgbdfe_keypoint* keypoints, float* desc128, int32_t capacity, int32_t* n_out);
int rgbdfe_sift_describe(rgbdfe_ctx* ctx, const uint8_t* gray, int32_t rows, int32_t cols, rgbdfe_keypoint* keypoints, int32_t n, float* desc128);
int rgbdfe_sift_detect_batch(rgbdfe_ctx* ctx, int32_t n_frames, const uint8_t* const* gray, int32_t rows, int32_t cols, int32_t max_keypoints, int32_t out_stride, rgbdfe_keypoint* keypoints, float* desc128, int32_t* n_out);
int rgbdfe_sift_detect_batch_nodes(rgbdfe_ctx* ctx, int32_t n_frames, const uint8_t* const* gray, const float* const* depth, int32_t rows, int32_t cols, double fx, double fy, double cx, double cy, double depth_scaling, int32_t max_keypoints, int32_t use_root_sift, const int32_t* node_ids, int32_t out_stride, rgbdfe_keypoint* keypoints, float* xyz1, float* feature_descriptors, int32_t* n_out);
int rgbdfe_sift_debug_plane(rgbdfe_ctx* ctx, int32_t octave, int32_t level, float* out, int32_t capacity_floats, int32_t* w, int32_t* h);
int rgbdfe_sift_debug_candidates(rgbdfe_ctx* ctx, int32_t octave, int32_t dog_level, float* out, int32_t capacity_rows, int32_t* n);
int rgbdfe_sift_geometry(rgbdfe_ctx* ctx, int32_t* octave_min, int32_t* octave_num, int32_t* levels, int32_t* dog_levels);
int rgbdfe_detect_describe(rgbdfe_ctx* ctx, const uint8_t* gray, const uint8_t* mask, const float* depth, int32_t rows, int32_t cols, double fx, double fy, double cx, double cy, double depth_scaling, rgbdfe_keypoint* keypoints, uint8_t* descriptors, float* xyz1, int32_t* n_out);
int rgbdfe_detect_describe_batch(rgbdfe_ctx* ctx, int32_t n_frames, const uint8_t* const* gray, const uint8_t* const* mask, const float* const* depth, int32_t rows, int32_t cols, double fx, double fy, double cx, double cy, double depth_scaling, int32_t out_stride, rgbdfe_keypoint* keypoints, uint8_t* descriptors, float* xyz1, int32_t* n_out, const int32_t* node_ids = nullptr, const SensorRun* sensor = nullptr);
int rgbdfe_hamming_nn_nodes(rgbdfe_ctx* ctx, int32_t query_id, int32_t train_id, int32_t* out_hd, int32_t* out_idx);
int rgbdfe_place_recognition_batch(rgbdfe_ctx* ctx, const int32_t* query_ids, int32_t n_queries, const int32_t* candidate_offsets, const int32_t* candidate_ids, int32_t k_neighbours, int32_t max_hd, int32_t max_out, int32_t* out_ids, float* out_scores, int32_t* out_counts);
int rgbdfe_place_recognition(rgbdfe_ctx* ctx, int32_t query_id, const int32_t* candidate_ids, int32_t n_candidates, int32_t k_neighbours, int32_t max_hd, int32_t max_out, int32_t* out_ids, float* out_scores, int32_t* n_out);
int rgbdfe_hamming_nn_host(rgbdfe_ctx* ctx, const uint8_t* qdesc, int32_t nq, const uint8_t* tdesc, int32_t nt, int32_t* out_hd, int32_t* out_idx);
int rgbdfe_project_to_3d(rgbdfe_ctx* ctx, const float* kp_xy, int32_t n_kp, const float* depth, int32_t rows, int32_t cols, double fx, double fy, double cx, double cy, double depth_scaling, int32_t max_keypoints, int32_t* kept_idx, float* xyz1, int32_t* n_out);
int rgbdfe_set_feature_min_depth(rgbdfe_ctx* ctx, int32_t on);
int rgbdfe_project_to_3d_min_depth(rgbdfe_ctx* ctx, const float* kp_xy, const float* kp_size, int32_t n_kp, const float* depth, int32_t rows, int32_t cols, double fx, double fy, double cx, double cy, double depth_scaling, int32_t max_keypoints, int32_t* kept_idx, float* xyz1, int32_t* n_out);
int rgbdfe_project_to_3d_cloud(rgbdfe_ctx* ctx, const float* kp_xy, int32_t n_kp, const float* cloud, int32_t rows, int32_t cols, double maximum_depth, int32_t max_keypoints, int32_t* kept_idx, float* xyz1, int32_t* n_out);
int rgbdfe_detect_describe_cloud(rgbdfe_ctx* ctx, const uint8_t* gray, const uint8_t* mask, const float* cloud, int32_t rows, int32_t cols, double maximum_depth, rgbdfe_keypoint* keypoints, uint8_t* descriptors, float* xyz1, int32_t* n_out);
int rgbdfe_detect(rgbdfe_ctx* ctx, const uint8_t* gray, const uint8_t* mask, int32_t rows, int32_t cols, rgbdfe_keypoint* keypoints, int32_t capacity, int32_t* n_out);
int rgbdfe_detect_sift_describe(rgbdfe_ctx* ctx, const uint8_t* gray, const uint8_t* mask, const float* depth, int32_t rows, int32_t cols, double fx, double fy, double cx, double cy, double depth_scaling, int32_t use_root_sift, rgbdfe_keypoint* keypoints, float* xyz1, float* siftgpu_descriptors, float* feature_descriptors, int32_t* n_out);
int rgbdfe_detect_sift_describe_batch_nodes(rgbdfe_ctx* ctx, int32_t n_frames, const uint8_t* const* gray, const uint8_t* const* mask, const float* const* depth, int32_t rows, int32_t cols, double fx, double fy, double cx, double cy, double depth_scaling, int32_t use_root_sift, const int32_t* node_ids, int32_t out_stride, rgbdfe_keypoint* keypoints, float* xyz1, float* feature_descriptors, int32_t* n_out);
int rgbdfe_sift_detect_orb_describe(rgbdfe_ctx* ctx, const uint8_t* gray, const float* depth, int32_t rows, int32_t cols, double fx, double fy, double cx, double cy, double depth_scaling, int32_t max_keypoints, rgbdfe_keypoint* keypoints, uint8_t* descriptors, float* xyz1, int32_t* n_out);
int rgbdfe_sift_detect_orb_describe_batch_nodes(rgbdfe_ctx* ctx, int32_t n_frames, const uint8_t* const* gray, const float* const* depth, int32_t rows, int32_t cols, double fx, double fy, double cx, double cy, double depth_scaling, int32_t max_keypoints, const int32_t* node_ids, int32_t out_stride, rgbdfe_keypoint* keypoints, uint8_t* descriptors, float* xyz1, int32_t* n_out);
int rgbdfe_sift_node_features(rgbdfe_ctx* ctx, const float* kp_xy, const float* kp_size, int32_t n_kp, const float* desc_in, const float* depth, int32_t rows, int32_t cols, double fx, double fy, double cx, double cy, double depth_scaling, int32_t max_keypoints, int32_t use_root_sift, int32_t* kept_idx, float* xyz1, float* siftgpu_descriptors, float* feature_descriptors, int32_t* n_out);
int rgbdfe_depth_to_mono8(rgbdfe_ctx* ctx, const void* depth, int32_t depth_is_u16, int32_t rows, int32_t cols, uint8_t* mono8, float* depth_m);
int rgbdfe_upload_node_cloud(rgbdfe_ctx* ctx, int32_t node_id, const float* depth, int32_t rows, int32_t cols, const uint8_t* rgb, int32_t rgb_channels, int32_t encoding_bgr, double fx, double fy, double cx, double cy, double depth_scaling, double min_depth, int32_t cloud_skip, float* cloud_out);
int rgbdfe_release_node_cloud(rgbdfe_ctx* ctx, int32_t node_id);
int rgbdfe_assemble_map(rgbdfe_ctx* ctx, int32_t n_nodes, const int32_t* node_ids, const float* transforms, double maximum_depth, int32_t preserve_raster, float* out, int64_t capacity, int64_t* n_out, int64_t* node_offsets);
int rgbdfe_assemble_map_device(rgbdfe_ctx* ctx, int32_t n_nodes, const int32_t* node_ids, const float* transforms, double maximum_depth, int32_t preserve_raster, void* d_out, int64_t capacity, int64_t* n_out, int64_t* node_offsets, void* stream);
int rgbdfe_download_node_cloud(rgbdfe_ctx* ctx, int32_t node_id, float* cloud_out, int64_t capacity_points, int32_t* rows, int32_t* cols);
int rgbdfe_voxel_filter(rgbdfe_ctx* ctx, const float* points, int64_t n_in, double voxelfilter_size, float* out, int64_t capacity, int64_t* n_out, int32_t* flags);
int rgbdfe_voxel_filter_device(rgbdfe_ctx* ctx, const void* d_points, int64_t n_in, double voxelfilter_size, void* d_out, int64_t capacity, int64_t* n_out, int32_t* flags, void* stream);
int rgbdfe_reduce_node_cloud(rgbdfe_ctx* ctx, int32_t node_id, double voxelfilter_size, int64_t* n_out, int32_t* flags);
int rgbdfe_pose_graph_chi2(rgbdfe_ctx* ctx, rgbdfe_pose_graph* g, double* chi2);
int rgbdfe_pose_graph_linearize(rgbdfe_ctx* ctx, rgbdfe_pose_graph* g, double* errors, double* weights, int32_t edge_capacity, int32_t* n_edges, int32_t* free_ids, double* h_diag, double* b, int32_t vertex_capacity, int32_t* n_free, int32_t* off_rows, int32_t* off_cols, double* h_off, int32_t block_capacity, int32_t* n_blocks, double* chi2);
int rgbdfe_pose_graph_optimize(rgbdfe_ctx* ctx, rgbdfe_pose_graph* g, int32_t iterations, rgbdfe_pose_graph_report* report);
int rgbdfe_pose_graph_optimize_graph(rgbdfe_ctx* ctx, rgbdfe_pose_graph* g, double break_criterion, rgbdfe_pose_graph_report* report);
void rgbdfe_octomap_default_params(rgbdfe_octomap_params* p);
rgbdfe_ctx* octomap_owner(rgbdfe_octomap* map);
int rgbdfe_octomap_create(rgbdfe_ctx* ctx, rgbdfe_ctx* owner, const rgbdfe_octomap_params* params, int64_t capacity_cells, rgbdfe_octomap** out);
void rgbdfe_octomap_destroy(rgbdfe_octomap* map);
int rgbdfe_octomap_reset(rgbdfe_octomap* map);
int rgbdfe_octomap_reserve(rgbdfe_octomap* map, int64_t capacity_cells);
int rgbdfe_octomap_insert_nodes(rgbdfe_octomap* map, int32_t n_nodes, const int32_t* node_ids, const float* transforms, double max_range, int32_t* n_done);
int rgbdfe_octomap_insert_cloud(rgbdfe_octomap* map, const float* points, int64_t n, const float* transform, double max_range);
int rgbdfe_octomap_size(rgbdfe_octomap* map, int64_t* n_leaves);
int rgbdfe_octomap_leaves(rgbdfe_octomap* map, rgbdfe_octomap_leaf* out, int64_t capacity, int64_t* n_out);
int rgbdfe_octomap_stats(rgbdfe_octomap* map, int64_t* out, int32_t n_out);
int rgbdfe_octomap_tree(rgbdfe_octomap* map, rgbdfe_octomap_node* out, int64_t capacity, int64_t* n_nodes);
int rgbdfe_octomap_tree_device(rgbdfe_octomap* map, void* d_out, int64_t capacity, int64_t* n_nodes, void* stream);
int rgbdfe_octomap_nodes_at_depth(rgbdfe_octomap* map, int32_t depth, float min_log_odds, rgbdfe_octomap_leaf* out, int64_t capacity, int64_t* n_out);
int rgbdfe_octomap_write(rgbdfe_octomap* map, const char* path);
int rgbdfe_octomap_set_leaves(rgbdfe_octomap* map, const rgbdfe_octomap_leaf* leaves, int64_t n);
int rgbdfe_octomap_read(rgbdfe_octomap* map, const char* path);
int rgbdfe_observation_likelihood(rgbdfe_ctx* ctx, int32_t n, const int32_t* new_ids, const int32_t* old_ids, const float* transforms, int32_t emm_skip_step, rgbdfe_emm_counts* out);
int rgbdfe_observation_criterion_met(uint32_t inliers, uint32_t outliers, uint32_t all, double observability_threshold, double* quality);
int rgbdfe_set_latency_mode(rgbdfe_ctx* ctx, int32_t max_pairs, int32_t chunk_iterations);
int rgbdfe_set_hamming_mode(rgbdfe_ctx* ctx, int32_t mode);
int rgbdfe_set_profiling(rgbdfe_ctx* ctx, int enable);
int rgbdfe_get_kernel_time(rgbdfe_ctx* ctx, int which, double* total_ms, int64_t* launches, int64_t* pairs);
int rgbdfe_reset_kernel_time(rgbdfe_ctx* ctx);
int rgbdfe_sizeof_match_result(void);
int rgbdfe_sizeof_compact_result(void);
int rgbdfe_pack_compact(rgbdfe_ctx* ctx, const void* d_records, int32_t n, void* d_compact, void* stream);
int rgbdfe_set_graph_capture(rgbdfe_ctx* ctx, int enable);
int rgbdfe_pack_inliers(rgbdfe_ctx* ctx, const void* d_records, int32_t n, int32_t n_headers, void* d_stream, int32_t* d_total, void* stream);
int rgbdfe_sizeof_inlier_header(void);
int rgbdfe_graph_stats(rgbdfe_ctx* ctx, int64_t* out, int32_t n_out);
int rgbdfe_abi_version(void);
}

#include <dlfcn.h>
namespace rgbdfe_host {

struct Rccl {
  void* handle = nullptr;
  int (*CommInitAll)(void**, int, const int*) = nullptr;
  int (*CommDestroy)(void*) = nullptr;
  int (*AllGather)(const void*, void*, size_t, int, void*, hipStream_t) = nullptr;
  int (*GroupStart)() = nullptr;
  int (*GroupEnd)() = nullptr;
  const char* (*GetErrorString)(int) = nullptr;
  bool load() {
    if (handle) return true;
    for (const char* name : {"librccl.so.1", "librccl.so", "/opt/rocm/lib/librccl.so.1"}) {
      handle = dlopen(name, RTLD_NOW | RTLD_GLOBAL);
      if (handle) break;
    }
    if (!handle) return false;
    CommInitAll = (decltype(CommInitAll))dlsym(handle, "ncclCommInitAll");
    CommDestroy = (decltype(CommDestroy))dlsym(handle, "ncclCommDestroy");
    AllGather = (decltype(AllGather))dlsym(handle, "ncclAllGather");
    GroupStart = (decltype(GroupStart))dlsym(handle, "ncclGroupStart");
    GroupEnd = (decltype(GroupEnd))dlsym(handle, "ncclGroupEnd");
    GetErrorString = (decltype(GetErrorString))dlsym(handle, "ncclGetErrorString");
    return CommInitAll && CommDestroy && AllGather && GroupStart && GroupEnd;
  }
};
constexpr int kNcclChar = 0;

struct Worker {
  std::thread th;
  std::mutex m;
  std::condition_variable cv;
  std::function<int()> job;
  bool has_job = false, quit = false;
  int rc = RGBDFE_OK;
};

}

struct Group {
  std::vector<rgbdfe_ctx*> children;
  std::vector<int> device_ids;
  std::vector<std::unique_ptr<Worker>> workers;
  Rccl rccl;
  std::vector<void*> comms;
  bool rccl_tried = false, rccl_ok = false;
  std::vector<hipStream_t> gather_streams;
  std::vector<hipEvent_t> gather_events;
  std::string transport = "none";
  std::vector<rgbdfe_match_result*> edge_recs;
  std::vector<int32_t*> edge_idx, edge_dst, edge_cnt;
  std::vector<int32_t*> edge_cnt_host;
  std::vector<char*> inl_stream;
  int32_t edge_cap = 0;
  size_t inl_cap_entries = 0;
  int inl_exchanges = 0;
  double last_submit_us = 0.0;
  std::recursive_mutex mu;
};
namespace rgbdfe_host {
void worker_main(Worker* w);
int group_run(rgbdfe_ctx* gctx, const std::function<int(int)>& fn);
void group_destroy(rgbdfe_ctx* gctx);
int group_create(const rgbdfe_config* cfg, const int32_t* device_ids, int32_t n, rgbdfe_ctx** out);
int group_match(rgbdfe_ctx* gctx, const int32_t* q, const int32_t* t, int32_t n, rgbdfe_match_result* out, bool sift, float* out_dist);
int group_each(rgbdfe_ctx* gctx, const std::function<int(int)>& fn);
int group_submit(rgbdfe_ctx* gctx, const std::function<int(int)>& fn);
bool group_setup_rccl(rgbdfe_ctx* gctx);
int group_ensure_edge_scratch(rgbdfe_ctx* gctx, int32_t per);
// ... 37 lines not shown
```

### rgbdslam_v2_amd/csrc/rgbdfe_internal.h

```cpp
#pragma once
#include <hip/hip_runtime.h>
#include <stdint.h>

#include "rgbdfe.h"

namespace rgbdfe {

struct PairWork {
  uint32_t q_slot, t_slot;
  uint32_t nq, nt;
  uint32_t uid;
  int32_t qid, tid;
  uint32_t pad;
};
static_assert(sizeof(PairWork) == 32, "PairWork layout");

constexpr uint32_t kNoMatchKey = (257u << 16) | 0xFFFFu;

struct RansacConst {
  int32_t max_matches, min_matches, ransac_iterations;
  float max_dist_m;
  double sq_max_dist;
  double depth_cov;
  double raster_cov_x;
  double raster_cov_y;
  uint32_t seed;
  int32_t g2o_iterations;
};

struct HammingGeometry { uint32_t qblocks, tsplit; };
HammingGeometry hamming_nn_geometry(uint32_t n_pairs, uint32_t max_nq, uint32_t max_nt, uint32_t key_planes_capacity);
uint32_t launch_hamming_nn(const uint32_t* desc_pool, const PairWork* work, uint32_t* keys,
                           uint32_t max_kp, uint32_t n_pairs, HammingGeometry geom, hipStream_t stream);
uint32_t hamming_mfma_tiles_per_slot(uint32_t max_kp);
size_t hamming_mfma_slab_bytes(uint32_t max_nodes, uint32_t max_kp);
void launch_hamming_expand(const uint32_t* node_rows, uint32_t* slab, uint32_t slot, uint32_t max_kp, uint32_t n,
                           hipStream_t stream);
HammingGeometry hamming_mfma_geometry(uint32_t n_pairs, uint32_t max_nq, uint32_t max_nt, uint32_t key_planes_capacity);
uint32_t launch_hamming_mfma(const uint32_t* slab, const PairWork* work, uint32_t* keys, uint32_t max_kp,
                             uint32_t n_pairs, HammingGeometry geom, int mode, hipStream_t stream);
void launch_place_votes(const uint32_t* keys, uint32_t planes, uint32_t max_kp, const PairWork* work, const uint32_t* seg,
                        uint32_t n_queries, uint32_t max_nq, uint32_t k_neighbours, uint32_t max_hd, uint32_t* votes,
                        hipStream_t stream);
void launch_select_ransac(const float4* xyz_pool, const PairWork* work, const uint32_t* keys,
                          uint32_t key_planes, rgbdfe_match_result* results, uint32_t max_kp,
                          uint32_t n_pairs, const RansacConst& rc, struct PairPrep* prep, double* ec_pool,
                          hipStream_t stream);
struct IterRec {
  float rR[9], rt[3];
  uint64_t rmask[5];
  double rerr;
  int32_t rn;
  int32_t pad;
};
struct IterSum {
  double rerr;
  int32_t rn;
  int32_t pad;
};
struct alignas(16) PairPrep {
  float M[RGBDFE_MAX_MATCHES * 7];
  uint64_t w_nonzero[RGBDFE_MASK_WORDS];
  int32_t n_all;
  float pmax;
  uint32_t fast_alpha;
  uint32_t pad;
};
struct WalkState {
  int32_t state;
  int32_t it, real_iterations, valid_iterations;
  int32_t best_idx;
  int32_t best_n;
  float rmse;
  int32_t speculate;
};
struct RecordPlan {
  IterRec* recs = nullptr;
  IterSum* sums = nullptr;
  WalkState* walk = nullptr;
  uint32_t n_chunks = 1;
  int chunk_iters = 0;
  int phase_begin = 0, phase_end = 0;
  int spec_end = 0;
  uint32_t n_chunks_b = 0;
  int chunk_iters_b = 0;
  int n_phases_total = 0;
  const PairPrep* prep = nullptr;
  double* ec_pool = nullptr;
  int final_walk = 0;
  const uint64_t* vmask = nullptr;
  int vmask_words = 0;
};
size_t select_ransac_ec_region_bytes();
struct SplitPlan {
  IterRec* recs = nullptr;
  IterSum* sums = nullptr;
  uint64_t* vmask = nullptr;
  WalkState* walk = nullptr;
  const PairPrep* prep = nullptr;
  int vmask_words = 0;
  int phased = 0;
  int n_phases = 1;
  int phase_ends[4] = {0, 0, 0, 0};
  int n_shares = 1;
  int share_iters = 0;
  uint8_t* preclass = nullptr;
  int preclass_iters = 0;
  uint32_t* unit_counter = nullptr;
  uint32_t* order_cnt = nullptr;
  uint32_t* order = nullptr;
};
constexpr int kOrderBuckets = 64;
__host__ __device__ inline int order_bucket(int n) { return n < 32 ? n : (32 + (n - 32) / 8 < kOrderBuckets ? 32 + (n - 32) / 8 : kOrderBuckets - 1); }
void launch_ransac_hyp(const PairWork* work, uint32_t n_pairs, const RansacConst& rc, const SplitPlan& plan, hipStream_t stream);
void launch_ransac_refine(uint32_t n_pairs, const RansacConst& rc, const SplitPlan& plan, hipStream_t stream);
int ransac_split_words_per_pair(int ransac_iterations);
int ransac_split_max_share();
int ransac_split_wgs();
int ransac_split_init();
inline size_t ransac_split_mask_bytes(size_t rec_capacity, size_t max_pairs) { return (rec_capacity / 64 + (5 + 32) * max_pairs + 64 + 64) * 8; }
inline uint32_t* ransac_split_order_cnt(IterRec* recs, size_t n_pairs, int ransac_iterations) {
// ... 193 lines not shown
```

### rgbdslam_v2_amd/frontend.py

```python
import ctypes as C
import os
import threading
import warnings
import weakref
from dataclasses import dataclass, field
from typing import List, Optional, Sequence

import numpy as np

from . import _lib
from ._lib import DEFAULT_HAMMING_MODE, RESULT_DTYPE, RgbdfeConfig, RgbdfeError, RgbdfeParams


@dataclass
class DMatch:
    queryIdx: int
    trainIdx: int
    distance: float


@dataclass
class LoadedEdge3D:
    id1: int = -1
    id2: int = -1
    transform: np.ndarray = field(default_factory=lambda: np.eye(4))
    informationMatrix: np.ndarray = field(default_factory=lambda: np.zeros((6, 6)))


@dataclass
class MatchingResult:
    inlier_matches: List[DMatch] = field(default_factory=list)
    all_matches: List[DMatch] = field(default_factory=list)
    edge: LoadedEdge3D = field(default_factory=LoadedEdge3D)
    rmse: float = 0.0
    ransac_trafo: np.ndarray = field(default_factory=lambda: np.eye(4, dtype=np.float32))
    final_trafo: np.ndarray = field(default_factory=lambda: np.eye(4, dtype=np.float32))
    valid_iterations: int = 0
    real_iterations: int = 0


def inlier_indices(rec) -> np.ndarray:
    bits = np.unpackbits(np.asarray(rec["inlier_mask"]).view(np.uint8), bitorder="little")
    return np.flatnonzero(bits[: int(rec["n_all"])]).astype(np.int32)


def record_to_matching_result(rec) -> MatchingResult:
    n_all = int(rec["n_all"])
    q = rec["all_q"][:n_all].astype(np.int32)
    t = rec["all_t"][:n_all].astype(np.int32)
    d = rec["all_hd"][:n_all].astype(np.float32) / np.float32(256.0)
    all_matches = [DMatch(int(a), int(b), float(c)) for a, b, c in zip(q, t, d)]
    inl = inlier_indices(rec)
    T = np.array(rec["trafo"], np.float32).reshape(4, 4).T.copy()
    mr = MatchingResult(all_matches=all_matches, inlier_matches=[all_matches[i] for i in inl],
                        rmse=float(rec["rmse"]), ransac_trafo=T, final_trafo=T.copy(),
                        valid_iterations=int(rec["valid_iterations"]),
                        real_iterations=int(rec["real_iterations"]))
    mr.edge.id1, mr.edge.id2 = int(rec["id1"]), int(rec["id2"])
    if mr.edge.id1 >= 0:
        mr.edge.transform = T.astype(np.float64)
        mr.edge.informationMatrix = np.eye(6) * float(rec["info_scale"])
    return mr


class FrontEnd:

    def __init__(self, device_id: int = 0, max_nodes: int = 256, max_keypoints: int = 1024,
                 max_pairs_per_batch: int = 4096, device_ids: Optional[Sequence[int]] = None, **params):
        self._L = _lib.load()
        self._batch_lock = threading.Lock()
        cfg = RgbdfeConfig()
        self._L.rgbdfe_default_config(C.byref(cfg))
        cfg.device_id = device_id
        cfg.max_nodes = max_nodes
        cfg.max_keypoints = max_keypoints
        cfg.max_pairs_per_batch = max_pairs_per_batch
        for k, v in params.items():
            if not hasattr(cfg.params, k):
                raise TypeError(f"unknown front-end parameter {k!r}")
            setattr(cfg.params, k, v)
        self.cfg = cfg
        self._ctx = C.c_void_p()
        if device_ids is not None:
            ids = np.ascontiguousarray(device_ids, np.int32)
            st = self._L.rgbdfe_create_multi(C.byref(cfg), ids.ctypes.data, len(ids), C.byref(self._ctx))
        else:
            st = self._L.rgbdfe_create(C.byref(cfg), C.byref(self._ctx))
        if st != 0:
            self._ctx = C.c_void_p()
            raise RgbdfeError(f"rgbdfe_create failed: {self._L.rgbdfe_status_string(st).decode()}")

    @property
    def device_count(self) -> int:
        return int(self._L.rgbdfe_device_count(self._ctx))

    def set_hamming_mode(self, mode: int):
        self._check(self._L.rgbdfe_set_hamming_mode(self._ctx, mode))
        self._hamming_mode = int(mode)

    @property
    def hamming_mode(self) -> int:
        import os
        m = getattr(self, "_hamming_mode", None)
        if m is None:
            try:
                m = int(os.environ.get("RGBDFE_HAMMING_MODE", str(DEFAULT_HAMMING_MODE)))
            except ValueError:
                m = DEFAULT_HAMMING_MODE
            m = m if 0 <= m <= 3 else DEFAULT_HAMMING_MODE
        return 0 if self.cfg.max_keypoints > 32768 else m

    def group_submit_us(self) -> float:
        v = C.c_double(0.0)
        self._check(self._L.rgbdfe_group_submit_us(self._ctx, C.byref(v)))
        return float(v.value)

    def gather_transport(self) -> str:
        return self._L.rgbdfe_gather_transport(self._ctx).decode()

    def gather_exchanges(self) -> int:
        return int(self._L.rgbdfe_gather_exchanges(self._ctx))

    def match_pair_list_allgather(self, query_ids, train_ids, d_out_ptrs: Sequence[int]) -> int:
        q = np.ascontiguousarray(query_ids, np.int32)
        t = np.ascontiguousarray(train_ids, np.int32)
        ptrs = (C.c_void_p * len(d_out_ptrs))(*[C.c_void_p(int(p)) for p in d_out_ptrs])
        per = C.c_int32(0)
        self._check(self._L.rgbdfe_match_pair_list_allgather(self._ctx, q.ctypes.data, t.ctypes.data, len(q),
                                                             C.cast(ptrs, C.c_void_p), C.byref(per)))
        return int(per.value)

    def match_pair_list_allgather_compact(self, query_ids, train_ids, d_out_ptrs: Sequence[int]) -> int:
        q = np.ascontiguousarray(query_ids, np.int32)
        t = np.ascontiguousarray(train_ids, np.int32)
        ptrs = (C.c_void_p * len(d_out_ptrs))(*[C.c_void_p(int(p)) for p in d_out_ptrs])
        per = C.c_int32(0)
        self._check(self._L.rgbdfe_match_pair_list_allgather_compact(self._ctx, q.ctypes.data, t.ctypes.data, len(q),
                                                                     C.cast(ptrs, C.c_void_p), C.byref(per)))
        return int(per.value)

    def match_pair_list_allgather_inliers(self, query_ids, train_ids, d_out_ptrs: Sequence[int]):
        q = np.ascontiguousarray(query_ids, np.int32)
        t = np.ascontiguousarray(train_ids, np.int32)
        g = len(d_out_ptrs)
        ptrs = (C.c_void_p * g)(*[C.c_void_p(int(p)) for p in d_out_ptrs])
        per, stride = C.c_int32(0), C.c_int64(0)
        totals = np.zeros(g, np.int32)
        self._check(self._L.rgbdfe_match_pair_list_allgather_inliers(self._ctx, q.ctypes.data, t.ctypes.data, len(q),
                                                                     C.cast(ptrs, C.c_void_p), C.byref(per), totals.ctypes.data,
                                                                     C.byref(stride)))
        return int(per.value), totals, int(stride.value)

    def pack_compact(self, d_records_ptr: int, n: int, d_compact_ptr: int, stream: Optional[int] = None):
        self._check(self._L.rgbdfe_pack_compact(self._ctx, C.c_void_p(int(d_records_ptr)), int(n),
                                                C.c_void_p(int(d_compact_ptr)), C.c_void_p(stream or 0)))

    def pack_inliers(self, d_records_ptr: int, n: int, n_headers: int, d_stream_ptr: int, d_total_ptr: int,
                     stream: Optional[int] = None):
        self._check(self._L.rgbdfe_pack_inliers(self._ctx, C.c_void_p(int(d_records_ptr)), int(n), int(n_headers),
                                                C.c_void_p(int(d_stream_ptr)), C.c_void_p(int(d_total_ptr)),
                                                C.c_void_p(stream or 0)))

    def match_pair_list_allgather_edges(self, query_ids, train_ids, d_out_ptrs: Sequence[int], d_index_ptrs=None):
        q = np.ascontiguousarray(query_ids, np.int32)
        t = np.ascontiguousarray(train_ids, np.int32)
        g = len(d_out_ptrs)
        ptrs = (C.c_void_p * g)(*[C.c_void_p(int(p)) for p in d_out_ptrs])
        iptrs = None if d_index_ptrs is None else (C.c_void_p * g)(*[C.c_void_p(int(p)) for p in d_index_ptrs])
        counts = np.zeros(g, np.int32)
        stride = C.c_int32(0)
        self._check(self._L.rgbdfe_match_pair_list_allgather_edges(
            self._ctx, q.ctypes.data, t.ctypes.data, len(q), C.cast(ptrs, C.c_void_p),
            None if iptrs is None else C.cast(iptrs, C.c_void_p), counts.ctypes.data, C.byref(stride)))
        return counts, int(stride.value)

    def _check(self, st):
        if st != 0:
            msg = self._L.rgbdfe_last_error(self._ctx).decode()
            raise RgbdfeError(f"{self._L.rgbdfe_status_string(st).decode()}: {msg}")

    def close(self):
        if getattr(self, "_ctx", None) and self._ctx.value:
            for ref in getattr(self, "_octomaps", []):
                m = ref()
                if m is not None:
                    m.close()
            self._L.rgbdfe_destroy(self._ctx)
            self._ctx = C.c_void_p()

    def __del__(self):
        try:
            self.close()
# ... 1084 lines not shown
```

Before: 3.990 million frame-pairs/s.

## Add four-query-tile wide variant of pipelined MFMA Hamming kernel with auto selection

```diff
diff --git a/include/rgbdfe.h b/include/rgbdfe.h
--- a/include/rgbdfe.h
+++ b/include/rgbdfe.h
@@ -177,6 +177,7 @@
 
 #define RGBDFE_HAMMING_MODE_DEFAULT 3
 int rgbdfe_set_hamming_mode(rgbdfe_ctx* ctx, int32_t mode);
+int rgbdfe_hamming_wide_last(rgbdfe_ctx* ctx);
 
 typedef struct rgbdfe_emm_counts {
   uint32_t inliers, outliers, occluded, all;
diff --git a/rgbdslam_v2_amd/_lib.py b/rgbdslam_v2_amd/_lib.py
--- a/rgbdslam_v2_amd/_lib.py
+++ b/rgbdslam_v2_amd/_lib.py
@@ -384,6 +384,8 @@
     L.rgbdfe_gather_exchanges.argtypes = [ctx]
     L.rgbdfe_set_hamming_mode.restype = C.c_int
     L.rgbdfe_set_hamming_mode.argtypes = [ctx, i32]
+    L.rgbdfe_hamming_wide_last.restype = C.c_int
+    L.rgbdfe_hamming_wide_last.argtypes = [ctx]
     L.rgbdfe_match_pair_list_allgather_compact.restype = C.c_int
     L.rgbdfe_match_pair_list_allgather_compact.argtypes = [ctx, vp, vp, i32, vp, C.POINTER(i32)]
     L.rgbdfe_pack_compact.restype = C.c_int
@@ -510,7 +512,7 @@
     "rgbdfe_pose_graph_add_edge_se3", "rgbdfe_pose_graph_chi2", "rgbdfe_pose_graph_linearize",
     "rgbdfe_pose_graph_optimize", "rgbdfe_pose_graph_optimize_graph", "rgbdfe_pose_graph_transforms",
     "rgbdfe_create_multi", "rgbdfe_device_count", "rgbdfe_device_context", "rgbdfe_match_pair_list_allgather",
-    "rgbdfe_gather_transport", "rgbdfe_gather_exchanges", "rgbdfe_set_hamming_mode", "rgbdfe_project_to_3d_cloud", "rgbdfe_detect_describe_cloud",
+    "rgbdfe_gather_transport", "rgbdfe_gather_exchanges", "rgbdfe_set_hamming_mode", "rgbdfe_hamming_wide_last", "rgbdfe_project_to_3d_cloud", "rgbdfe_detect_describe_cloud",
     "rgbdfe_detect_describe_batch", "rgbdfe_detect_describe_batch_nodes", "rgbdfe_match_pair_list_allgather_edges",
     "rgbdfe_set_feature_min_depth", "rgbdfe_project_to_3d_min_depth",
     "rgbdfe_place_recognition", "rgbdfe_place_recognition_batch", "rgbdfe_upload_float_node",
diff --git a/rgbdslam_v2_amd/csrc/api_batches.hip b/rgbdslam_v2_amd/csrc/api_batches.hip
--- a/rgbdslam_v2_amd/csrc/api_batches.hip
+++ b/rgbdslam_v2_amd/csrc/api_batches.hip
@@ -166,12 +166,15 @@
 
 HammingGeometry hamming_geometry(const rgbdfe_ctx* ctx, uint32_t n, uint32_t max_nq, uint32_t max_nt) {
   const uint32_t cap = (uint32_t)ctx->cfg.max_pairs_per_batch;
-  return hamming_on_mfma(ctx) ? hamming_mfma_geometry(n, max_nq, max_nt, cap) : hamming_nn_geometry(n, max_nq, max_nt, cap);
+  if (!hamming_on_mfma(ctx)) return hamming_nn_geometry(n, max_nq, max_nt, cap);
+  const int pipe_wide = ctx->hamming_mode == 4 ? 1 : ctx->hamming_mode == 3 ? ctx->hamming_wide : 0;
+  return hamming_mfma_geometry(n, max_nq, max_nt, cap, pipe_wide);
 }
 
 uint32_t launch_hamming(rgbdfe_ctx* ctx, const PairWork* d_work, uint32_t* d_keys, uint32_t n, HammingGeometry geom,
                         hipStream_t stream) {
   const uint32_t mk = (uint32_t)ctx->cfg.max_keypoints;
+  if (n > 0 && geom.qblocks > 0) ctx->hamming_wide_last = (int)geom.wide;
   if (hamming_on_mfma(ctx))
     return launch_hamming_mfma(ctx->d_desc4, d_work, d_keys, mk, n, geom, ctx->hamming_mode, stream);
   return launch_hamming_nn(ctx->d_desc, d_work, d_keys, mk, n, geom, stream);
@@ -251,15 +254,16 @@
   if (n > 0) {
     if (!d_out) d_out = lane.d_results;
     const bool graphable = ctx->use_graphs && !sift && !ctx->profiling && piece >= n && ctx->rc.g2o_iterations == 0;
-    const HammingGeometry geom = sift ? HammingGeometry{0, 1}
+    const HammingGeometry geom = sift ? HammingGeometry{0, 1, 0}
                                       : hamming_geometry(ctx, (uint32_t)(piece < n ? piece : n), max_nq, max_nt);
+    if (!sift && geom.qblocks > 0) ctx->hamming_wide_last = (int)geom.wide;
     rgbdfe_ctx::GraphEntry* ge = nullptr;
     bool capturing = false;
     if (graphable) {
       rgbdfe_ctx::GraphKey key;
       memset(&key, 0, sizeof(key));
       key.n = n; key.qblocks = geom.qblocks; key.tsplit = geom.tsplit; key.slot = (int32_t)(ticket % rgbdfe_ctx::kRing);
-      key.latency = latency ? 1 : 0; key.chunk = chunk; key.hamming_mode = ctx->hamming_mode; key.n_phases = pp.n_phases;
+      key.latency = latency ? 1 : 0; key.chunk = chunk; key.hamming_mode = ctx->hamming_mode | (int32_t)(geom.wide << 8); key.n_phases = pp.n_phases;
       for (int i = 0; i < 4; ++i) key.ends[i] = i < pp.n_phases ? pp.ends[i] : 0;
       memcpy(&key.rc, &ctx->rc, sizeof(RansacConst));
       key.d_out = d_out; key.d_recs = lane.d_recs; key.d_ec = lane.d_ec; key.d_walk = lane.d_walk; key.d_keys = lane.d_keys;
diff --git a/rgbdslam_v2_amd/csrc/api_context.hip b/rgbdslam_v2_amd/csrc/api_context.hip
--- a/rgbdslam_v2_amd/csrc/api_context.hip
+++ b/rgbdslam_v2_amd/csrc/api_context.hip
@@ -33,7 +33,8 @@
   if (rc != RGBDFE_OK) { delete ctx; return rc; }
   fill_ransac_const(ctx);
   if (const char* sf = getenv("RGBDFE_SIFT_FAST_KEYS")) ctx->sift_fast = atoi(sf) != 0;
-  if (const char* hm = getenv("RGBDFE_HAMMING_MODE")) ctx->hamming_mode = atoi(hm) < 0 || atoi(hm) > 3 ? RGBDFE_HAMMING_MODE_DEFAULT : atoi(hm);
+  if (const char* hm = getenv("RGBDFE_HAMMING_MODE")) ctx->hamming_mode = atoi(hm) < 0 || atoi(hm) > 4 ? RGBDFE_HAMMING_MODE_DEFAULT : atoi(hm);
+  if (const char* hw = getenv("RGBDFE_HAMMING_WIDE")) ctx->hamming_wide = atoi(hw) != 0 ? 1 : 0;
   if (const char* gr = getenv("RGBDFE_GRAPHS")) ctx->use_graphs = atoi(gr) != 0;
   auto bail = [&](int code) { ::rgbdfe_destroy(ctx); return code; };
   if (hipSetDevice(cfg->device_id) != hipSuccess) return bail(RGBDFE_ERR_NO_DEVICE);
diff --git a/rgbdslam_v2_amd/csrc/api_frame.hip b/rgbdslam_v2_amd/csrc/api_frame.hip
--- a/rgbdslam_v2_amd/csrc/api_frame.hip
+++ b/rgbdslam_v2_amd/csrc/api_frame.hip
@@ -615,10 +615,17 @@
 }
 
 int rgbdfe_set_hamming_mode(rgbdfe_ctx* ctx, int32_t mode) {
-  if (!ctx || mode < 0 || mode > 3) return fail(ctx, RGBDFE_ERR_INVALID_ARG, "hamming mode must be 0, 1, 2 or 3");
+  if (!ctx || mode < 0 || mode > 4) return fail(ctx, RGBDFE_ERR_INVALID_ARG, "hamming mode must be 0, 1, 2, 3 or 4");
   std::lock_guard<std::mutex> g(ctx->mu);
   ctx->hamming_mode = mode;
-  return RGBDFE_OK;
+  if (mode == 3) ctx->hamming_wide = 0;
+  return RGBDFE_OK;
+}
+
+int rgbdfe_hamming_wide_last(rgbdfe_ctx* ctx) {
+  if (!ctx) return -1;
+  std::lock_guard<std::mutex> g(ctx->mu);
+  return ctx->hamming_wide_last;
 }
 
 int rgbdfe_set_profiling(rgbdfe_ctx* ctx, int enable) {
diff --git a/rgbdslam_v2_amd/csrc/hamming_mfma.hip b/rgbdslam_v2_amd/csrc/hamming_mfma.hip
--- a/rgbdslam_v2_amd/csrc/hamming_mfma.hip
+++ b/rgbdslam_v2_amd/csrc/hamming_mfma.hip
@@ -34,6 +34,7 @@
 
 typedef int v8i __attribute__((ext_vector_type(8)));
 typedef float v16f __attribute__((ext_vector_type(16)));
+typedef int v4i __attribute__((ext_vector_type(4)));
 
 constexpr int kThreads = 256;
 #ifndef RGBDFE_HAMMING_QT
@@ -76,6 +77,13 @@
 __device__ __forceinline__ v8i as_operand(uint4 v) {
   v8i o;
   o[0] = (int)v.x; o[1] = (int)v.y; o[2] = (int)v.z; o[3] = (int)v.w;
+  o[4] = 0; o[5] = 0; o[6] = 0; o[7] = 0;
+  return o;
+}
+
+__device__ __forceinline__ v8i op8(v4i v) {
+  v8i o;
+  o[0] = v[0]; o[1] = v[1]; o[2] = v[2]; o[3] = v[3];
   o[4] = 0; o[5] = 0; o[6] = 0; o[7] = 0;
   return o;
 }
@@ -244,6 +252,9 @@
 }
 
 
+#ifndef RGBDFE_HAMMING_PIPE_QT
+#define RGBDFE_HAMMING_PIPE_QT 0
+#endif
 #ifndef RGBDFE_HAMMING_PIPE_BURST
 #define RGBDFE_HAMMING_PIPE_BURST 0
 #endif
@@ -266,7 +277,7 @@
 #define HP_SGB(MASK, N) __builtin_amdgcn_sched_group_barrier(MASK, N, 0);
 #define HP_FENCE() __builtin_amdgcn_sched_barrier(0);
 
-template <bool SPLIT>
+template <int QT, bool SPLIT>
 __global__ __launch_bounds__(kThreads) __attribute__((amdgpu_waves_per_eu(RGBDFE_HAMMING_PIPE_WAVES, RGBDFE_HAMMING_PIPE_WAVES)))
 void hamming_mfma_pipe_kernel(const uint4* __restrict__ slab,
                                                                      const PairWork* __restrict__ work,
@@ -274,6 +285,8 @@
                                                                      uint32_t tiles_per_slot, uint32_t n_pairs,
                                                                      uint32_t qblocks, uint32_t tsplit) {
   __shared__ uint4 lds0[kPipeStage][256], lds1[kPipeStage][256], lds2[kPipeStage][256];
+  static_assert((QT == 2 || QT == 4) && kPipeStage == 4, "the unrolled streams are written for two or four query tiles and four-tile stages");
+  constexpr uint32_t kQPB = 4u * QT * 32u;
   const uint32_t L = blockIdx.x;
   const uint32_t xcd = L & 7u;
   const uint32_t j = L >> 3;
@@ -286,7 +299,7 @@
 
   const PairWork w = work[pair];
   const uint32_t nq = w.nq;
-  if (qblock * kQueriesPerBlock >= nq) return;
+  if (qblock * kQPB >= nq) return;
   const HammingSlots slots = HammingSlots::make(w.nt, SPLIT ? tsplit : 1u, SPLIT ? split : 0u, kPipeStage);
   const uint32_t nt_search = slots.nt_search, n_stages = slots.n_stages;
   const bool has_ragged = slots.has_ragged;
@@ -296,10 +309,10 @@
   const uint32_t wave = __builtin_amdgcn_readfirstlane(threadIdx.x >> 6);
   const uint32_t half = lane >> 5;
 
-  v8i bq[kQT][4];
-#pragma unroll
-  for (int t = 0; t < kQT; ++t) {
-    uint32_t qt = qblock * (kQueriesPerBlock / 32) + wave * kQT + t;
+  v8i bq[QT][4];
+#pragma unroll
+  for (int t = 0; t < QT; ++t) {
+    uint32_t qt = qblock * (kQPB / 32u) + wave * QT + t;
     qt = min(qt, tiles_per_slot - 1u);
     const uint4* __restrict__ qs = slab + ((size_t)w.q_slot * tiles_per_slot + qt) * 256u;
 #pragma unroll
@@ -324,8 +337,8 @@
       c3[r] = row < nts ? crow[r] : kNone;
     }
   };
-
   uint32_t best0 = __float_as_uint(kNone), best1 = __float_as_uint(kNone);
+  uint32_t best2 = __float_as_uint(kNone), best3 = __float_as_uint(kNone);
 
   const uint32_t last_tile = tiles_per_slot - 1u;
   const char* __restrict__ ts = reinterpret_cast<const char*>(slab + (size_t)w.t_slot * tiles_per_slot * 256u);
@@ -348,7 +361,6 @@
   };
 
   if (n_stages > 0) {
-    static_assert(kQT == 2 && kPipeStage == 4, "the unrolled stream is written for two query tiles and four-tile stages");
     load_stage(0, lds0);
     if (n_stages > 1) load_stage(1, lds1);
     __builtin_amdgcn_s_waitcnt(0x0F70);
@@ -377,15 +389,25 @@
     HP_SGB(0x008, 1) HP_SGB(0x002, RGBDFE_HAMMING_PIPE_VALU_GROUPS / 10 % 10)                        \
     HP_SGB(0x008, 1) HP_SGB(0x002, RGBDFE_HAMMING_PIPE_VALU_GROUPS % 10)
 #endif
-#define HP_UNIT(ACC, A, Q, C, PACC, PBEST, PBASE, R0, R1)                                           \
+#if RGBDFE_HAMMING_PIPE_BURST
+#define HP_UNIT_SCHED0() HP_SGB(0x008, 4) HP_SGB(0x002, 12)
+#else
+#define HP_UNIT_SCHED0()                                                                            \
+    HP_SGB(0x008, 1)                                                                                \
+    HP_SGB(0x008, 1) HP_SGB(0x002, RGBDFE_HAMMING_PIPE_VALU_GROUPS / 100)                            \
+    HP_SGB(0x008, 1) HP_SGB(0x002, RGBDFE_HAMMING_PIPE_VALU_GROUPS / 10 % 10)                        \
+    HP_SGB(0x008, 1) HP_SGB(0x002, RGBDFE_HAMMING_PIPE_VALU_GROUPS % 10)
+#endif
+#define HP_UNIT_X(ACC, A, Q, C, PACC, PBEST, PBASE, READS, SCHED)                                   \
     HP_MFMA(ACC, A[0], bq[Q][0], C)                                                                 \
-    R0 R1                                                                                           \
+    READS                                                                                           \
     HP_MFMA(ACC, A[1], bq[Q][1], ACC)                                                               \
     HP_EPI(PACC, PBEST, PBASE)                                                                      \
     HP_MFMA(ACC, A[2], bq[Q][2], ACC)                                                               \
     HP_MFMA(ACC, A[3], bq[Q][3], ACC)                                                               \
-    HP_UNIT_SCHED()                                                                                 \
+    SCHED()                                                                                         \
     HP_FENCE()
+#define HP_UNIT(ACC, A, Q, C, PACC, PBEST, PBASE, R0, R1) HP_UNIT_X(ACC, A, Q, C, PACC, PBEST, PBASE, R0 R1, HP_UNIT_SCHED)
 #if RGBDFE_HAMMING_PIPE_DIAG & 4
 #define HP_TURN()
 #define HP_LOADS false
@@ -460,51 +482,145 @@
     }
 
 #endif
-    HP_READ(aA, 0, 0, 0) HP_READ(aA, 0, 0, 1) HP_READ(aA, 0, 0, 2) HP_READ(aA, 0, 0, 3)
+#if RGBDFE_HAMMING_PIPE_DIAG & 2
+#define HP4_READ(BUF, SLOT, S) asm volatile("" : "+v"(a4[S]));
+#else
+#define HP4_READ(BUF, SLOT, S)                                                                                       \
+    asm volatile("ds_read_b128 %0, %1 offset:%2" : "+v"(a4[S]) : "v"(rd##BUF), "n"((SLOT) * 4096 + (S) * 1024) : "memory");
+#endif
+#define HP4_WAIT(N) __builtin_amdgcn_s_waitcnt(0xC07F | ((N) << 8)); HP_FENCE()
+#define HP4_A(S) op8(a4[S])
+#define HP4_BASE(SLOT) __uint_as_float(__builtin_amdgcn_readfirstlane(__float_as_uint(HP_BASE(SLOT))))
+#define HP4_UNIT0(ACC, Q, C, PACC, PBEST, PBASE)                                                                     \
+      HP_MFMA(ACC, HP4_A(0), bq[Q][0], C)                                                                            \
+      HP_MFMA(ACC, HP4_A(1), bq[Q][1], ACC)                                                                          \
+      HP_EPI(PACC, PBEST, PBASE)                                                                                     \
+      HP_MFMA(ACC, HP4_A(2), bq[Q][2], ACC)                                                                          \
+      HP_MFMA(ACC, HP4_A(3), bq[Q][3], ACC)                                                                          \
+      HP_UNIT_SCHED0()                                                                                               \
+      HP_FENCE()
+#define HP4_TILE(C, PB, B, RSLOT, RBUF)                                                                              \
+      HP4_WAIT(3) HP_MFMA(acc0, HP4_A(0), bq[0][0], C)                                                               \
+      HP4_WAIT(2) HP_MFMA(acc0, HP4_A(1), bq[0][1], acc0)                                                            \
+      HP_EPI(acc1, best3, PB)                                                                                        \
+      HP4_WAIT(1) HP_MFMA(acc0, HP4_A(2), bq[0][2], acc0)                                                            \
+      HP4_WAIT(0) HP_MFMA(acc0, HP4_A(3), bq[0][3], acc0)                                                            \
+      HP_FENCE()                                                                                                     \
+      HP4_UNIT0(acc1, 1, C, acc0, best0, B)                                                                          \
+      HP4_UNIT0(acc0, 2, C, acc1, best1, B)                                                                          \
+      HP_MFMA(acc1, HP4_A(0), bq[3][0], C)                                                                           \
+      HP_FENCE() HP4_READ(RBUF, RSLOT, 0)                                                                            \
+      HP_MFMA(acc1, HP4_A(1), bq[3][1], acc1)                                                                        \
+      HP_FENCE() HP4_READ(RBUF, RSLOT, 1)                                                                            \
+      HP_EPI(acc0, best2, B)                                                                                         \
+      HP_MFMA(acc1, HP4_A(2), bq[3][2], acc1)                                                                        \
+      HP_FENCE() HP4_READ(RBUF, RSLOT, 2)                                                                            \
+      HP_MFMA(acc1, HP4_A(3), bq[3][3], acc1)                                                                        \
+      HP_FENCE() HP4_READ(RBUF, RSLOT, 3)                                                                            \
+      HP_FENCE()
+#define HP4_HALF_A(CUR, NXT)                                                                                         \
+    {                                                                                                                \
+      b0 = HP4_BASE(0); b1 = HP4_BASE(1);                                                                            \
+      HP_FENCE()                                                                                                     \
+      HP4_TILE(crow, pend, b0, 1, CUR)                                                                               \
+      HP4_TILE(crow, b0, b1, 2, CUR)                                                                                 \
+      HP_TURN()                                                                                                      \
+      if (has_ragged && st + 2u == n_stages) patch_ragged(lds##NXT);              \
+    }
+#define HP4_HALF_B(CUR, NXT, NN)                                                                                     \
+    {                                                                                                                \
+      if (HP_LOADS && st + 2u < n_stages) load_stage(st + 2u, lds##NN);                                              \
+      const float b2 = HP4_BASE(2), b3 = HP4_BASE(3);                                                                \
+      HP_FENCE()                                                                                                     \
+      HP4_TILE(crow, b1, b2, 3, CUR)                                                                                 \
+      HP_FENCE()                                                                                                     \
+      HP4_TILE(crow, b2, b3, 0, NXT)                                                                                 \
+      pend = b3;                                                                                                     \
+    }
+    if constexpr (QT == 2) {
+      HP_READ(aA, 0, 0, 0) HP_READ(aA, 0, 0, 1) HP_READ(aA, 0, 0, 2) HP_READ(aA, 0, 0, 3)
 #if RGBDFE_HAMMING_PIPE_ALT4
-    v16f acc0, acc1, acc2 = crow, acc3 = crow;
-#else
-    v16f acc0, acc1 = crow;
-#endif
-    float pend = 4.0e6f;
-    float b0, b1;
-    uint32_t st = 0;
-    HP_HALF_A(0)
-    for (;;) {
-      HP_HALF_B(0, 1, 2)
-      if (++st == n_stages) break;
-      HP_HALF_A(1)
-      HP_HALF_B(1, 2, 0)
-      if (++st == n_stages) break;
-      HP_HALF_A(2)
-      HP_HALF_B(2, 0, 1)
-      if (++st == n_stages) break;
+      v16f acc0, acc1, acc2 = crow, acc3 = crow;
+#else
+      v16f acc0, acc1 = crow;
+#endif
+      float pend = 4.0e6f;
+      float b0, b1;
+      uint32_t st = 0;
       HP_HALF_A(0)
-    }
+      for (;;) {
+        HP_HALF_B(0, 1, 2)
+        if (++st == n_stages) break;
+        HP_HALF_A(1)
+        HP_HALF_B(1, 2, 0)
+        if (++st == n_stages) break;
+        HP_HALF_A(2)
+        HP_HALF_B(2, 0, 1)
+        if (++st == n_stages) break;
+        HP_HALF_A(0)
+      }
 #if RGBDFE_HAMMING_PIPE_ALT4
-    HP_EPI(acc2, best0, pend)
-    HP_EPI(acc3, best1, pend)
-#else
-    HP_EPI(acc1, best1, pend)
-#endif
+      HP_EPI(acc2, best0, pend)
+      HP_EPI(acc3, best1, pend)
+#else
+      HP_EPI(acc1, best1, pend)
+#endif
+    } else {
+      const uint32_t rd0 = (uint32_t)(size_t)(__attribute__((address_space(3))) char*)&lds0[0][0] + lane * 16u;
+      const uint32_t rd1 = (uint32_t)(size_t)(__attribute__((address_space(3))) char*)&lds1[0][0] + lane * 16u;
+      const uint32_t rd2 = (uint32_t)(size_t)(__attribute__((address_space(3))) char*)&lds2[0][0] + lane * 16u;
+      v4i a4[4] = {{0, 0, 0, 0}, {0, 0, 0, 0}, {0, 0, 0, 0}, {0, 0, 0, 0}};
+      auto patch_ragged = [&](uint4 (*buf)[256]) {
+        const uint32_t t = threadIdx.x;
+        if ((t & 31u) >= (nt_search & 31u)) buf[kPipeStage - 1][t] = buf[kPipeStage - 1][t & ~31u];
+      };
+      if (has_ragged && n_stages <= 2u) patch_ragged(n_stages == 1u ? lds0 : lds1);
+      HP4_READ(0, 0, 0) HP4_READ(0, 0, 1) HP4_READ(0, 0, 2) HP4_READ(0, 0, 3)
+      v16f acc0, acc1 = crow;
+      float pend = 4.0e6f;
+      float b0, b1;
+      uint32_t st = 0;
+      HP4_HALF_A(0, 1)
+      for (;;) {
+        HP4_HALF_B(0, 1, 2)
+        if (++st == n_stages) break;
+        HP4_HALF_A(1, 2)
+        HP4_HALF_B(1, 2, 0)
+        if (++st == n_stages) break;
+        HP4_HALF_A(2, 0)
+        HP4_HALF_B(2, 0, 1)
+        if (++st == n_stages) break;
+        HP4_HALF_A(0, 1)
+      }
+      HP_EPI(acc1, best3, pend)
+    }
+#undef HP4_TILE
+#undef HP4_UNIT0
+#undef HP4_BASE
+#undef HP4_A
+#undef HP4_WAIT
+#undef HP4_READ
+#undef HP4_HALF_A
+#undef HP4_HALF_B
 #undef HP_HALF_A
 #undef HP_HALF_B
 #undef HP_TURN
 #undef HP_LOADS
 #undef HP_UNIT
+#undef HP_UNIT_X
 #undef HP_EPI
 #undef HP_BASE
 #undef HP_READ
   }
 
   uint32_t* kout = keys + ((size_t)pair * tsplit + split) * max_kp;
-  const uint32_t bests[2] = {best0, best1};
-#pragma unroll
-  for (int t = 0; t < kQT; ++t) {
+  const uint32_t bests[4] = {best0, best1, best2, best3};
+#pragma unroll
+  for (int t = 0; t < QT; ++t) {
     uint32_t bb = bests[t];
     bb = min(bb, (uint32_t)__shfl_xor((int)bb, 32));
     const float b = __uint_as_float(bb);
-    const uint32_t qi = qblock * kQueriesPerBlock + (wave * kQT + (uint32_t)t) * 32u + (lane & 31u);
+    const uint32_t qi = qblock * kQPB + (wave * QT + (uint32_t)t) * 32u + (lane & 31u);
     if (half == 0 && qi < nq) {
       uint32_t key = kNoMatchKey;
       if (RGBDFE_HAMMING_PIPE_DIAG ? b < -1.0f : b < 1024.0f) {
@@ -550,21 +666,43 @@
   hipLaunchKernelGGL(hamming_expand_kernel, dim3(tiles), dim3(256), 0, stream, node_rows, dst, n);
 }
 
-HammingGeometry hamming_mfma_geometry(uint32_t n_pairs, uint32_t max_nq, uint32_t max_nt, uint32_t key_planes_capacity) {
-  HammingGeometry g{0, 1};
+constexpr uint32_t kHammingBlockSlots = 256u * 3u;
+constexpr uint32_t kWideMinBlocksPerSlot = 10u;
+
+HammingGeometry hamming_mfma_geometry(uint32_t n_pairs, uint32_t max_nq, uint32_t max_nt, uint32_t key_planes_capacity,
+                                      int pipe_wide) {
+  HammingGeometry g{0, 1, 0};
   if (n_pairs == 0 || max_nq == 0) return g;
-  g.qblocks = (max_nq + kQueriesPerBlock - 1) / kQueriesPerBlock;
-  const uint32_t blocks1 = n_pairs * g.qblocks;
   const uint32_t ttiles = (max_nt + 31u) / 32u;
-  if (blocks1 < 1024 && ttiles > kStage) {
-    uint32_t tsplit = (1024 + blocks1 - 1) / blocks1;
-    const uint32_t max_split = (ttiles + kStage - 1) / kStage;
-    if (tsplit > max_split) tsplit = max_split;
-    if (tsplit > 32) tsplit = 32;
-    const uint32_t fit = key_planes_capacity / n_pairs;
-    if (tsplit > fit) tsplit = fit;
-    if (tsplit < 1) tsplit = 1;
-    g.tsplit = tsplit;
+  auto shape = [&](uint32_t queries_per_block) {
+    HammingGeometry h{(max_nq + queries_per_block - 1u) / queries_per_block, 1, 0};
+    const uint32_t blocks1 = n_pairs * h.qblocks;
+    if (blocks1 < 1024 && ttiles > kStage) {
+      uint32_t tsplit = (1024 + blocks1 - 1) / blocks1;
+      const uint32_t max_split = (ttiles + kStage - 1) / kStage;
+      if (tsplit > max_split) tsplit = max_split;
+      if (tsplit > 32) tsplit = 32;
+      const uint32_t fit = key_planes_capacity / n_pairs;
+      if (tsplit > fit) tsplit = fit;
+      if (tsplit < 1) tsplit = 1;
+      h.tsplit = tsplit;
+    }
+    return h;
+  };
+  g = shape(kQueriesPerBlock);
+  if (pipe_wide < 0) {
+#if RGBDFE_HAMMING_PIPE_QT == 4
+    pipe_wide = 1;
+#elif RGBDFE_HAMMING_PIPE_QT == 2
+    pipe_wide = 0;
+#else
+    const uint64_t wide_blocks = (uint64_t)n_pairs * ((max_nq + 2u * kQueriesPerBlock - 1u) / (2u * kQueriesPerBlock));
+    pipe_wide = g.tsplit == 1u && wide_blocks >= (uint64_t)kHammingBlockSlots * kWideMinBlocksPerSlot ? 1 : 0;
+#endif
+  }
+  if (pipe_wide > 0) {
+    g = shape(2u * kQueriesPerBlock);
+    g.wide = 1;
   }
   return g;
 }
@@ -580,18 +718,21 @@
 #define RGBDFE_LAUNCH_HM(M, S)                                                                                   \
   hipLaunchKernelGGL((hamming_mfma_kernel<M, S>), dim3(grid), dim3(kThreads), 0, stream, s4, work, keys, max_kp, \
                      tiles_per_slot, n_pairs, qblocks, tsplit)
-  if (mode == 3) {
-    if (tsplit > 1)
-      hipLaunchKernelGGL((hamming_mfma_pipe_kernel<true>), dim3(grid), dim3(kThreads), 0, stream, s4, work, keys, max_kp,
-                         tiles_per_slot, n_pairs, qblocks, tsplit);
-    else
-      hipLaunchKernelGGL((hamming_mfma_pipe_kernel<false>), dim3(grid), dim3(kThreads), 0, stream, s4, work, keys, max_kp,
-                         tiles_per_slot, n_pairs, qblocks, tsplit);
+#define RGBDFE_LAUNCH_HP(QT, S)                                                                                        \
+  hipLaunchKernelGGL((hamming_mfma_pipe_kernel<QT, S>), dim3(grid), dim3(kThreads), 0, stream, s4, work, keys, max_kp, \
+                     tiles_per_slot, n_pairs, qblocks, tsplit)
+  if (mode == 3 || mode == 4) {
+    if (geom.wide) {
+      if (tsplit > 1) RGBDFE_LAUNCH_HP(4, true); else RGBDFE_LAUNCH_HP(4, false);
+    } else {
+      if (tsplit > 1) RGBDFE_LAUNCH_HP(2, true); else RGBDFE_LAUNCH_HP(2, false);
+    }
   } else if (mode == 2) {
     if (tsplit > 1) RGBDFE_LAUNCH_HM(2, true); else RGBDFE_LAUNCH_HM(2, false);
   } else {
     if (tsplit > 1) RGBDFE_LAUNCH_HM(1, true); else RGBDFE_LAUNCH_HM(1, false);
   }
+#undef RGBDFE_LAUNCH_HP
 #undef RGBDFE_LAUNCH_HM
   return tsplit;
 }
diff --git a/rgbdslam_v2_amd/csrc/hamming_nn.hip b/rgbdslam_v2_amd/csrc/hamming_nn.hip
--- a/rgbdslam_v2_amd/csrc/hamming_nn.hip
+++ b/rgbdslam_v2_amd/csrc/hamming_nn.hip
@@ -101,7 +101,7 @@
 }
 
 HammingGeometry hamming_nn_geometry(uint32_t n_pairs, uint32_t max_nq, uint32_t max_nt, uint32_t key_planes_capacity) {
-  HammingGeometry g{0, 1};
+  HammingGeometry g{0, 1, 0};
   if (n_pairs == 0 || max_nq == 0) return g;
   g.qblocks = (max_nq + kQueriesPerBlock - 1) / kQueriesPerBlock;
   const uint32_t blocks1 = n_pairs * g.qblocks;
diff --git a/rgbdslam_v2_amd/csrc/rgbdfe_api.hip b/rgbdslam_v2_amd/csrc/rgbdfe_api.hip
--- a/rgbdslam_v2_amd/csrc/rgbdfe_api.hip
+++ b/rgbdslam_v2_amd/csrc/rgbdfe_api.hip
@@ -990,6 +990,11 @@
   return RGBDFE_ALL(ctx, impl::rgbdfe_set_hamming_mode(c, mode));
 }
 
+int rgbdfe_hamming_wide_last(rgbdfe_ctx* ctx) {
+  if (!ctx) return -1;
+  return impl::rgbdfe_hamming_wide_last(RGBDFE_IS_GROUP(ctx) ? ctx->group->children[0] : ctx);
+}
+
 int rgbdfe_set_profiling(rgbdfe_ctx* ctx, int enable) {
   if (!ctx) return RGBDFE_ERR_INVALID_ARG;
   return RGBDFE_ALL(ctx, impl::rgbdfe_set_profiling(c, enable));
diff --git a/rgbdslam_v2_amd/csrc/rgbdfe_host.h b/rgbdslam_v2_amd/csrc/rgbdfe_host.h
--- a/rgbdslam_v2_amd/csrc/rgbdfe_host.h
+++ b/rgbdslam_v2_amd/csrc/rgbdfe_host.h
@@ -158,6 +158,8 @@
   bool feature_min_depth = false;
   bool sift_fast = true;
   int hamming_mode = RGBDFE_HAMMING_MODE_DEFAULT;
+  int hamming_wide = -1;
+  int hamming_wide_last = -1;
 #ifndef RGBDFE_LANES
 #define RGBDFE_LANES 2
 #endif
@@ -506,6 +508,7 @@
 int rgbdfe_observation_criterion_met(uint32_t inliers, uint32_t outliers, uint32_t all, double observability_threshold, double* quality);
 int rgbdfe_set_latency_mode(rgbdfe_ctx* ctx, int32_t max_pairs, int32_t chunk_iterations);
 int rgbdfe_set_hamming_mode(rgbdfe_ctx* ctx, int32_t mode);
+int rgbdfe_hamming_wide_last(rgbdfe_ctx* ctx);
 int rgbdfe_set_profiling(rgbdfe_ctx* ctx, int enable);
 int rgbdfe_get_kernel_time(rgbdfe_ctx* ctx, int which, double* total_ms, int64_t* launches, int64_t* pairs);
 int rgbdfe_reset_kernel_time(rgbdfe_ctx* ctx);
diff --git a/rgbdslam_v2_amd/csrc/rgbdfe_internal.h b/rgbdslam_v2_amd/csrc/rgbdfe_internal.h
--- a/rgbdslam_v2_amd/csrc/rgbdfe_internal.h
+++ b/rgbdslam_v2_amd/csrc/rgbdfe_internal.h
@@ -28,7 +28,7 @@
   int32_t g2o_iterations;
 };
 
-struct HammingGeometry { uint32_t qblocks, tsplit; };
+struct HammingGeometry { uint32_t qblocks, tsplit, wide; };
 HammingGeometry hamming_nn_geometry(uint32_t n_pairs, uint32_t max_nq, uint32_t max_nt, uint32_t key_planes_capacity);
 uint32_t launch_hamming_nn(const uint32_t* desc_pool, const PairWork* work, uint32_t* keys,
                            uint32_t max_kp, uint32_t n_pairs, HammingGeometry geom, hipStream_t stream);
@@ -36,7 +36,8 @@
 size_t hamming_mfma_slab_bytes(uint32_t max_nodes, uint32_t max_kp);
 void launch_hamming_expand(const uint32_t* node_rows, uint32_t* slab, uint32_t slot, uint32_t max_kp, uint32_t n,
                            hipStream_t stream);
-HammingGeometry hamming_mfma_geometry(uint32_t n_pairs, uint32_t max_nq, uint32_t max_nt, uint32_t key_planes_capacity);
+HammingGeometry hamming_mfma_geometry(uint32_t n_pairs, uint32_t max_nq, uint32_t max_nt, uint32_t key_planes_capacity,
+                                      int pipe_wide);
 uint32_t launch_hamming_mfma(const uint32_t* slab, const PairWork* work, uint32_t* keys, uint32_t max_kp,
                              uint32_t n_pairs, HammingGeometry geom, int mode, hipStream_t stream);
 void launch_place_votes(const uint32_t* keys, uint32_t planes, uint32_t max_kp, const PairWork* work, const uint32_t* seg,
diff --git a/rgbdslam_v2_amd/frontend.py b/rgbdslam_v2_amd/frontend.py
--- a/rgbdslam_v2_amd/frontend.py
+++ b/rgbdslam_v2_amd/frontend.py
@@ -99,6 +99,10 @@
         self._hamming_mode = int(mode)
 
     @property
+    def hamming_wide_last(self) -> int:
+        return int(self._L.rgbdfe_hamming_wide_last(self._ctx))
+
+    @property
     def hamming_mode(self) -> int:
         import os
         m = getattr(self, "_hamming_mode", None)
@@ -107,7 +111,7 @@
                 m = int(os.environ.get("RGBDFE_HAMMING_MODE", str(DEFAULT_HAMMING_MODE)))
             except ValueError:
                 m = DEFAULT_HAMMING_MODE
-            m = m if 0 <= m <= 3 else DEFAULT_HAMMING_MODE
+            m = m if 0 <= m <= 4 else DEFAULT_HAMMING_MODE
         return 0 if self.cfg.max_keypoints > 32768 else m
 
     def group_submit_us(self) -> float:
```

Measured after the change: 4.074 million frame-pairs/s (median of 6 runs). 1.02x the previous value.
